# yex33/ReSpaSol

Hardware: AMD Instinct MI355X
Metric: CSR SpMV GFLOP/s + achieved HBM GB/s (fp64 vs fp32), SuiteSparse set, 1/2/4/8 GPU (higher is better)
Workload: dtype f64; 1 GPU; big-set CSR SpMV fp64, 15 matrices per step; matrices=15, nnz_stored_total=268386865, parallelism=1 GPU, launch=rsp_spmv_batch (1 launch(es) of <= 32 matrices per step part): whole step

## Files before the change

include/rsp.h:

```cpp
#ifndef RSP_H
#define RSP_H

#include <stddef.h>
#include <stdint.h>

#ifdef __cplusplus
extern "C" {
#endif

#define RSP_VERSION_MAJOR 0
#define RSP_VERSION_MINOR 1

typedef enum {
    RSP_STATUS_SUCCESS = 0,
    RSP_STATUS_NOT_INITIALIZED = 1,
    RSP_STATUS_ALLOC_FAILED = 2,
    RSP_STATUS_INVALID_VALUE = 3,
    RSP_STATUS_ARCH_MISMATCH = 4,
    RSP_STATUS_EXECUTION_FAILED = 6,
    RSP_STATUS_INTERNAL_ERROR = 7,
    RSP_STATUS_MATRIX_TYPE_NOT_SUPPORTED = 8,
    RSP_STATUS_ZERO_PIVOT = 9,
    RSP_STATUS_NOT_SUPPORTED = 10
} rsp_status_t;

typedef enum { RSP_R_64F = 0, RSP_R_32F = 1 } rsp_datatype_t;

typedef enum { RSP_OPERATION_NON_TRANSPOSE = 0, RSP_OPERATION_TRANSPOSE = 1 } rsp_operation_t;

typedef struct rsp_context *rsp_handle_t;
typedef struct rsp_spmat *rsp_spmat_t;
typedef struct rsp_ilu0_info *rsp_ilu0_info_t;
typedef struct rsp_spmv_batch *rsp_spmv_batch_t;


rsp_status_t rsp_create(rsp_handle_t *handle);
rsp_status_t rsp_destroy(rsp_handle_t handle);
rsp_status_t rsp_set_stream(rsp_handle_t handle, void *stream);
rsp_status_t rsp_get_stream(rsp_handle_t handle, void **stream);
rsp_status_t rsp_set_ftz(rsp_handle_t handle, int enable);
rsp_status_t rsp_get_ftz(rsp_handle_t handle, int *enable);
const char *rsp_get_error_string(rsp_status_t status);
int rsp_get_version(void);


rsp_status_t rsp_create_csr(rsp_spmat_t *mat, int64_t rows, int64_t cols, int64_t nnz,
                            void *d_row_offsets, void *d_col_ind, void *d_values,
                            rsp_datatype_t value_type);
rsp_status_t rsp_csr_set_values(rsp_spmat_t mat, void *d_values, rsp_datatype_t value_type);
rsp_status_t rsp_destroy_spmat(rsp_spmat_t mat);


rsp_status_t rsp_spmv_buffer_size(rsp_handle_t handle, rsp_operation_t op, const void *alpha,
                                  rsp_spmat_t mat, const void *beta, rsp_datatype_t compute_type,
                                  size_t *buffer_size);
rsp_status_t rsp_spmv_preprocess(rsp_handle_t handle, rsp_operation_t op, const void *alpha,
                                 rsp_spmat_t mat, const void *d_x, const void *beta, void *d_y,
                                 rsp_datatype_t compute_type, void *d_buffer);
rsp_status_t rsp_spmv(rsp_handle_t handle, rsp_operation_t op, const void *alpha, rsp_spmat_t mat,
                      const void *d_x, const void *beta, void *d_y, rsp_datatype_t compute_type,
                      void *d_buffer);


rsp_status_t rsp_create_ilu0_info(rsp_ilu0_info_t *info);
rsp_status_t rsp_destroy_ilu0_info(rsp_ilu0_info_t info);

rsp_status_t rsp_ilu0_buffer_size(rsp_handle_t handle, int n, int nnz, rsp_datatype_t value_type,
                                  rsp_ilu0_info_t info, size_t *buffer_size);

rsp_status_t rsp_ilu0_analysis(rsp_handle_t handle, int n, int nnz, const int *d_row_offsets,
                               const int *d_col_ind, rsp_ilu0_info_t info);

rsp_status_t rsp_trsv_analysis(rsp_handle_t handle, rsp_operation_t op, rsp_ilu0_info_t info);

rsp_status_t rsp_ilu0_zero_pivot(rsp_handle_t handle, rsp_ilu0_info_t info, int *position);

#define RSP_TRSV_L 0
#define RSP_TRSV_LT 1
#define RSP_TRSV_U 2
rsp_status_t rsp_trsv_zero_pivot(rsp_handle_t handle, rsp_ilu0_info_t info, int which, int *position);

rsp_status_t rsp_ilu0_factor(rsp_handle_t handle, rsp_ilu0_info_t info, rsp_datatype_t value_type,
                             void *d_values);

rsp_status_t rsp_trsv_lower_unit(rsp_handle_t handle, rsp_operation_t op, const void *alpha,
                                 rsp_ilu0_info_t info, rsp_datatype_t value_type,
                                 const void *d_values, const void *d_x, void *d_y);

rsp_status_t rsp_trsv_upper(rsp_handle_t handle, const void *alpha, rsp_ilu0_info_t info,
                            rsp_datatype_t value_type, const void *d_values, const void *d_x,
                            void *d_y);


typedef struct rsp_bicgstab *rsp_bicgstab_t;
typedef enum { RSP_SOLVE_CONVERGED = 0, RSP_SOLVE_MAX_ITERS = 1, RSP_SOLVE_BREAKDOWN = 2 } rsp_solve_reason_t;

rsp_status_t rsp_bicgstab_create(rsp_handle_t handle, rsp_spmat_t A, rsp_ilu0_info_t info,
                                 rsp_datatype_t precond_type, const void *d_factor, rsp_bicgstab_t *s);
rsp_status_t rsp_bicgstab_solve(rsp_handle_t handle, rsp_bicgstab_t s, const void *d_b, void *d_x,
                                double rtol, int max_iters, int check_every,
                                int *iters, double *relres, rsp_solve_reason_t *reason);
rsp_status_t rsp_bicgstab_history(rsp_bicgstab_t s, int cap, double *relres, int *count);
rsp_status_t rsp_bicgstab_destroy(rsp_bicgstab_t s);
rsp_status_t rsp_dot(rsp_handle_t handle, rsp_datatype_t value_type, int64_t n, const void *d_x,
                     const void *d_y, double *result);

#define RSP_GMRES_MAX_RESTART 64
typedef struct rsp_gmres *rsp_gmres_t;
rsp_status_t rsp_gmres_create(rsp_handle_t handle, rsp_spmat_t A, rsp_ilu0_info_t info,
                              rsp_datatype_t precond_type, const void *d_factor, int restart,
                              rsp_gmres_t *s);
rsp_status_t rsp_gmres_solve(rsp_handle_t handle, rsp_gmres_t s, const void *d_b, void *d_x, double rtol,
                             int max_iters, int check_every, int *iters, double *relres,
                             rsp_solve_reason_t *reason);
rsp_status_t rsp_gmres_history(rsp_gmres_t s, int cap, double *relres, int *count);
rsp_status_t rsp_gmres_destroy(rsp_gmres_t s);
rsp_status_t rsp_orthogonalize(rsp_handle_t handle, rsp_datatype_t value_type, int64_t n, int k,
                               const void *d_V, int64_t ldv, void *d_w, double *h);
rsp_status_t rsp_gmres_lsq_host(int k, int ldh, const double *H, double beta, double *y, double *est);


rsp_status_t rsp_gather(rsp_handle_t handle, rsp_datatype_t value_type, int64_t n,
                        const int64_t *d_idx, const void *d_src, void *d_dst);
rsp_status_t rsp_scatter(rsp_handle_t handle, rsp_datatype_t value_type, int64_t n,
                         const int64_t *d_idx, const void *d_src, void *d_dst);

rsp_status_t rsp_csr2csc(rsp_handle_t handle, int64_t rows, int64_t cols, int64_t nnz,
                         const int *d_row_offsets, const int *d_col_ind, const void *d_values,
                         rsp_datatype_t value_type, int *d_csc_col_offsets, int *d_csc_row_ind,
                         void *d_csc_values);

rsp_status_t rsp_spmv_plan_info(rsp_spmat_t mat, int64_t *tiles, int64_t *entries_16bit);

rsp_status_t rsp_spmat_set_local_cols(rsp_spmat_t mat, int64_t ncols_local);
rsp_status_t rsp_spmv_part(rsp_handle_t handle, const void *alpha, rsp_spmat_t mat,
                           const void *d_x, const void *beta, void *d_y,
                           rsp_datatype_t compute_type, void *d_buffer, int part);

rsp_status_t rsp_spmv_batch_create(rsp_handle_t handle, int count, const rsp_spmat_t *mats,
                                   const void *const *d_x, void *const *d_y,
                                   void *const *d_buffers, rsp_datatype_t compute_type,
                                   int part, rsp_spmv_batch_t *batch);
rsp_status_t rsp_spmv_batch_run(rsp_handle_t handle, rsp_spmv_batch_t batch, const void *alpha,
                                const void *beta);
rsp_status_t rsp_spmv_batch_destroy(rsp_spmv_batch_t batch);
rsp_status_t rsp_spmv_batch_info(rsp_spmv_batch_t batch, int64_t *tiles, int64_t *entries_16bit);

rsp_status_t rsp_ilu0_levels(rsp_ilu0_info_t info, int *levels_lower, int *levels_upper);
rsp_status_t rsp_ilu0_solve_blocks(rsp_ilu0_info_t info, int *blocks_lower, int *blocks_upper);

rsp_status_t rsp_ilu0_analysis_host(int n, const int *row_offsets, const int *col_ind,
                                    int *levels_lower, int *levels_upper, uint64_t *digest,
                                    double *phase_ms);
rsp_status_t rsp_spmv_plan_host(int m, const int *row_offsets, const int *col_ind, int64_t nnz,
                                rsp_datatype_t compute_type, int64_t *tiles, int64_t *entries_16bit,
                                int64_t *entries_staged);
rsp_status_t rsp_spmv_transpose_permute(rsp_handle_t handle, rsp_spmat_t mat);
rsp_status_t rsp_csr_transpose_host(int64_t rows, int64_t cols, const int *row_offsets, const int *col_ind,
                                    int *t_row_offsets, int *t_col_ind, int *perm);
rsp_status_t rsp_spmv_plan_stats(int m, const int *row_offsets, const int *col_ind, int64_t nnz,
                                 rsp_datatype_t compute_type, int64_t stats[8]);
rsp_status_t rsp_ilu0_plan_digest(rsp_ilu0_info_t info, uint64_t *digest);

#ifdef __cplusplus
}
#endif

#endif
```

respasol_amd/_lib.py:

```python
from __future__ import annotations

import ctypes as C
import os

_HERE = os.path.dirname(os.path.abspath(__file__))
LIB_DIR = os.path.join(_HERE, "lib")
BIN_DIR = os.path.join(_HERE, "bin")


class RspError(RuntimeError):

    def __init__(self, status: int, where: str):
        self.status = int(status)
        super().__init__(f"{where}: {STATUS_NAMES.get(self.status, 'RSP_STATUS_UNKNOWN')} ({self.status})")


STATUS_SUCCESS = 0
STATUS_NOT_INITIALIZED = 1
STATUS_ALLOC_FAILED = 2
STATUS_INVALID_VALUE = 3
STATUS_ARCH_MISMATCH = 4
STATUS_EXECUTION_FAILED = 6
STATUS_INTERNAL_ERROR = 7
STATUS_MATRIX_TYPE_NOT_SUPPORTED = 8
STATUS_ZERO_PIVOT = 9
STATUS_NOT_SUPPORTED = 10
STATUS_NAMES = {
    0: "RSP_STATUS_SUCCESS", 1: "RSP_STATUS_NOT_INITIALIZED", 2: "RSP_STATUS_ALLOC_FAILED",
    3: "RSP_STATUS_INVALID_VALUE", 4: "RSP_STATUS_ARCH_MISMATCH", 6: "RSP_STATUS_EXECUTION_FAILED",
    7: "RSP_STATUS_INTERNAL_ERROR", 8: "RSP_STATUS_MATRIX_TYPE_NOT_SUPPORTED",
    9: "RSP_STATUS_ZERO_PIVOT", 10: "RSP_STATUS_NOT_SUPPORTED",
}

R_64F = 0
R_32F = 1
OP_N = 0
OP_T = 1

SOLVE_CONVERGED = 0
SOLVE_MAX_ITERS = 1
SOLVE_BREAKDOWN = 2
KRY_CHUNK = 2048
KRY_MAX_GRID = 1024
GMRES_MAX_RESTART = 64

MM_FULL_SYMMETRIC = 0x1
MM_QUIET = 0x2
MM_SERIAL = 0x4
SURR_FTZ_STRESS = 0x1


class CSRStruct(C.Structure):

    _fields_ = [("isSymmetric", C.c_int), ("m", C.c_int), ("n", C.c_int), ("nnz", C.c_int),
                ("rowptr", C.POINTER(C.c_int)), ("colidx", C.POINTER(C.c_int)),
                ("values", C.POINTER(C.c_double))]


class COOStruct(C.Structure):

    _fields_ = [("isSymmetric", C.c_int), ("m", C.c_int), ("n", C.c_int), ("nnz", C.c_int),
                ("Colidx", C.POINTER(C.c_int)), ("Rowidx", C.POINTER(C.c_int)),
                ("values", C.POINTER(C.c_double))]


vp = C.c_void_p
ip = C.POINTER(C.c_int)
i64 = C.c_int64
i32 = C.c_int

RSP_PROTOS = {
    "rsp_create": (i32, [C.POINTER(vp)]),
    "rsp_destroy": (i32, [vp]),
    "rsp_set_stream": (i32, [vp, vp]),
    "rsp_get_stream": (i32, [vp, C.POINTER(vp)]),
    "rsp_set_ftz": (i32, [vp, i32]),
    "rsp_get_ftz": (i32, [vp, ip]),
    "rsp_get_error_string": (C.c_char_p, [i32]),
    "rsp_get_version": (i32, []),
    "rsp_create_csr": (i32, [C.POINTER(vp), i64, i64, i64, vp, vp, vp, i32]),
    "rsp_csr_set_values": (i32, [vp, vp, i32]),
    "rsp_destroy_spmat": (i32, [vp]),
    "rsp_spmv_buffer_size": (i32, [vp, i32, vp, vp, vp, i32, C.POINTER(C.c_size_t)]),
    "rsp_spmv_preprocess": (i32, [vp, i32, vp, vp, vp, vp, vp, i32, vp]),
    "rsp_spmv": (i32, [vp, i32, vp, vp, vp, vp, vp, i32, vp]),
    "rsp_create_ilu0_info": (i32, [C.POINTER(vp)]),
    "rsp_destroy_ilu0_info": (i32, [vp]),
    "rsp_ilu0_buffer_size": (i32, [vp, i32, i32, i32, vp, C.POINTER(C.c_size_t)]),
    "rsp_ilu0_analysis": (i32, [vp, i32, i32, vp, vp, vp]),
    "rsp_ilu0_zero_pivot": (i32, [vp, vp, ip]),
    "rsp_trsv_zero_pivot": (i32, [vp, vp, i32, ip]),
    "rsp_ilu0_factor": (i32, [vp, vp, i32, vp]),
    "rsp_trsv_lower_unit": (i32, [vp, i32, vp, vp, i32, vp, vp, vp]),
    "rsp_trsv_upper": (i32, [vp, vp, vp, i32, vp, vp, vp]),
    "rsp_ilu0_levels": (i32, [vp, ip, ip]),
    "rsp_ilu0_solve_blocks": (i32, [vp, ip, ip]),
    "rsp_trsv_analysis": (i32, [vp, i32, vp]),
    "rsp_bicgstab_create": (i32, [vp, vp, vp, i32, vp, C.POINTER(vp)]),
    "rsp_bicgstab_solve": (i32, [vp, vp, vp, vp, C.c_double, i32, i32, ip, C.POINTER(C.c_double), ip]),
    "rsp_bicgstab_history": (i32, [vp, i32, C.POINTER(C.c_double), ip]),
    "rsp_bicgstab_destroy": (i32, [vp]),
    "rsp_dot": (i32, [vp, i32, i64, vp, vp, C.POINTER(C.c_double)]),
    "rsp_gmres_create": (i32, [vp, vp, vp, i32, vp, i32, C.POINTER(vp)]),
    "rsp_gmres_solve": (i32, [vp, vp, vp, vp, C.c_double, i32, i32, ip, C.POINTER(C.c_double), ip]),
    "rsp_gmres_history": (i32, [vp, i32, C.POINTER(C.c_double), ip]),
    "rsp_gmres_destroy": (i32, [vp]),
    "rsp_orthogonalize": (i32, [vp, i32, i64, i32, vp, i64, vp, C.POINTER(C.c_double)]),
    "rsp_gmres_lsq_host": (i32, [i32, i32, C.POINTER(C.c_double), C.c_double, C.POINTER(C.c_double),
                                 C.POINTER(C.c_double)]),
    "rsp_gather": (i32, [vp, i32, i64, vp, vp, vp]),
    "rsp_scatter": (i32, [vp, i32, i64, vp, vp, vp]),
    "rsp_spmat_set_local_cols": (i32, [vp, i64]),
    "rsp_spmv_part": (i32, [vp, vp, vp, vp, vp, vp, i32, vp, i32]),
    "rsp_spmv_batch_create": (i32, [vp, i32, vp, vp, vp, vp, i32, i32, vp]),
    "rsp_spmv_batch_run": (i32, [vp, vp, vp, vp]),
    "rsp_spmv_batch_destroy": (i32, [vp]),
    "rsp_spmv_batch_info": (i32, [vp, vp, vp]),
    "rsp_spmv_plan_info": (i32, [vp, vp, vp]),
    "rsp_ilu0_analysis_host": (i32, [i32, vp, vp, vp, vp, vp, vp]),
    "rsp_spmv_plan_host": (i32, [i32, vp, vp, C.c_int64, i32, vp, vp, vp]),
    "rsp_spmv_plan_stats": (i32, [i32, vp, vp, C.c_int64, i32, vp]),
    "rsp_ilu0_plan_digest": (i32, [vp, vp]),
    "rsp_csr2csc": (i32, [vp, i64, i64, i64, vp, vp, vp, i32, vp, vp, vp]),
    "rsp_csr_transpose_host": (i32, [i64, i64, vp, vp, vp, vp, vp]),
    "rsp_spmv_transpose_permute": (i32, [vp, vp]),
}

HOST_PROTOS = {
    "loadMatrixMarket": (i32, [C.c_char_p, C.POINTER(CSRStruct), i32, i32]),
    "loadCooMatrix": (i32, [C.c_char_p, C.POINTER(COOStruct), i32, i32]),
    "rsp_mm_load": (i32, [C.c_char_p, C.POINTER(CSRStruct), i32, i32, i32]),
    "rsp_mm_load_buffer": (i32, [C.c_char_p, C.c_size_t, C.POINTER(CSRStruct), i32, i32, i32]),
    "rsp_row_qsort": (None, [ip, C.POINTER(C.c_double), i32, i32]),
    "rsp_csr_free": (None, [C.POINTER(CSRStruct)]),
    "rsp_coo_free": (None, [C.POINTER(COOStruct)]),
    "rsp_csr_save": (i32, [C.c_char_p, C.POINTER(CSRStruct)]),
    "rsp_csr_load": (i32, [C.c_char_p, C.POINTER(CSRStruct)]),
    "rsp_dlarnv": (i32, [i32, ip, i64, C.POINTER(C.c_double)]),
    "rsp_set_cpu_ftz": (None, [i32]),
    "rsp_surrogate_count": (i32, []),
    "rsp_surrogate_name": (C.c_char_p, [i32]),
    "rsp_surrogate_info": (i32, [C.c_char_p, ip, C.POINTER(i64), ip, ip, ip]),
    "rsp_surrogate_rowlens": (i32, [C.c_char_p, C.c_double, i32, i32, i32, ip]),
    "rsp_surrogate_rows": (i32, [C.c_char_p, C.c_double, ip]),
    "rsp_surrogate_fill": (i32, [C.c_char_p, C.c_double, i32, i32, i32, ip, ip, C.POINTER(C.c_double)]),
    "rsp_surrogate_csr": (i32, [C.c_char_p, C.c_double, i32, C.POINTER(CSRStruct)]),
    "rsp_partition_rows": (i32, [ip, i32, i32, ip]),
    "rsp_padded_chunk": (i32, [ip, i32]),
    "rsp_remap_cols_padded": (i32, [i64, ip, ip, i32, i32, ip]),
    "rsp_host_spmv_f64": (None, [i32, ip, ip, vp, vp, vp]),
    "rsp_host_spmv_f32": (None, [i32, ip, ip, vp, vp, vp]),
}


def _load(name: str, protos: dict, path: str | None = None, probe: bool = False) -> C.CDLL:
    path = path or os.path.join(LIB_DIR, name)
    if not os.path.exists(path):
        raise ImportError(
            f"{path} is missing: build the HIP/C libraries first "
            f"(python -c 'import __graft_entry__ as g; g.build()' or make -C respasol_amd/csrc)")
    lib = C.CDLL(path, mode=C.RTLD_GLOBAL)
    for fname, (res, args) in protos.items():
        if probe and not hasattr(lib, fname):
            continue
        fn = getattr(lib, fname)
        fn.restype = res
        fn.argtypes = args
    return lib


host = _load("librsp_host.so", HOST_PROTOS)
_RSP_PATH = os.environ.get("RSP_PROBE_LIB") or os.path.join(LIB_DIR, "librsp.so")
rsp = (None if os.environ.get("RSP_HOST_ONLY") == "1"
       else _load("librsp.so", RSP_PROTOS, _RSP_PATH, probe=bool(os.environ.get("RSP_PROBE_LIB"))))


def check(status: int, where: str) -> None:
    if status != STATUS_SUCCESS:
        raise RspError(status, where)


def loaded_paths() -> list[str]:
    return [os.path.join(LIB_DIR, "librsp_host.so"), _RSP_PATH]
```

respasol_amd/csrc/rsp_api.cpp:

```cpp

#include "rsp_internal.h"

#include <atomic>

using namespace rsp_api;

using rsp::SpmvBlock;
using rsp::SpmvLongRow;
using rsp_plan::PlanOptions;
using rsp_plan::TilePlan;

namespace {
std::atomic<unsigned long long> g_plan_next{1};
unsigned long long plan_new_gen() { return g_plan_next.fetch_add(1); }
}


static int64_t spmv_resident_tiles(rsp_handle_t h, rsp_datatype_t t) {
    return (int64_t)rsp_k::spmv_tiles_per_cu((int)elem_size(t)) * h->num_cus;
}

static PlanOptions handle_plan_options(rsp_handle_t h, rsp_datatype_t t, int64_t local_cols, int64_t spread) {
    const int e = (int)elem_size(t), v = h->spmv_variant;
    PlanOptions o = rsp_plan::plan_options(t);
    o.spread = spread;
    o.local_cols = local_cols;
    o.row_align = (v & 64) ? 128 / e : (v & 128) ? 64 / e : 1;
    o.use_c16 = !(v & 32);
    o.use_stage = !(v & rsp::kSpmvVariantNoStage);
    return o;
}

static rsp_status_t download_pattern(rsp_handle_t h, rsp_spmat_t mat, rsp_an::hvec<int> &rp,
                                     rsp_an::hvec<int> &ci) {
    const int m = (int)mat->rows;
    rp.assign((size_t)m + 1, 0);
    ci.clear();
    if (m > 0) {
        RSP_CHECK_HIP(hipMemcpyAsync(rp.data(), mat->rowptr, ((size_t)m + 1) * sizeof(int),
                                     hipMemcpyDeviceToHost, h->stream));
        RSP_CHECK_HIP(hipStreamSynchronize(h->stream));
    }
    if (m > 0 && rp[0] != 0) return RSP_STATUS_INVALID_VALUE;
    for (int i = 0; i < m; i++)
        if (rp[i + 1] < rp[i]) return RSP_STATUS_INVALID_VALUE;
    if (m > 0 && (int64_t)rp[(size_t)m] > mat->nnz) return RSP_STATUS_INVALID_VALUE;
    if (m > 0 && rp[(size_t)m] > 0) {
        if (!mat->colidx) return RSP_STATUS_INVALID_VALUE;
        ci.resize((size_t)rp[(size_t)m]);
        RSP_CHECK_HIP(hipMemcpyAsync(ci.data(), mat->colidx, ci.size() * sizeof(int),
                                     hipMemcpyDeviceToHost, h->stream));
        RSP_CHECK_HIP(hipStreamSynchronize(h->stream));
        const int ncols = (int)mat->cols;
        for (int c : ci)
            if ((unsigned)c >= (unsigned)ncols) return RSP_STATUS_INVALID_VALUE;
    }
    return RSP_STATUS_SUCCESS;
}

rsp_status_t rsp_api::spmv_plan(rsp_handle_t h, rsp_spmat_t mat, rsp_datatype_t compute_type) {
    const int m = (int)mat->rows;
    rsp_an::hvec<int> rp, ci;
    rsp_status_t st = download_pattern(h, mat, rp, ci);
    if (st != RSP_STATUS_SUCCESS) return st;
    const bool spread = (h->spmv_variant & 512) != 0;
    TilePlan p;
    rsp_plan::make_tile_plan(rp.data(), ci.data(), m, mat->nnz,
                             handle_plan_options(h, compute_type, mat->local_cols,
                                                 spread ? spmv_resident_tiles(h, compute_type) : 0),
                             p);
    const size_t elem = elem_size(compute_type);
    const rsp_plan::SpmvLayout lay = rsp_plan::spmv_layout({p.blocks.size(), p.longrows.size(), (size_t)p.nslots},
                                                           elem, (int64_t)p.c16.size(), p.runs.size());
    mat->planned = 0;
    if (lay.bytes > mat->plan_cap || !mat->d_plan) {
        if (mat->d_plan) {
            int cur = 0;
            (void)hipGetDevice(&cur);
            (void)hipSetDevice(mat->plan_device);
            (void)hipFree(mat->d_plan);
            (void)hipSetDevice(cur);
            mat->d_plan = nullptr;
            mat->plan_cap = 0;
        }
        RSP_CHECK_HIP(hipMalloc(&mat->d_plan, std::max<size_t>(lay.bytes, 256)));
        mat->plan_cap = std::max<size_t>(lay.bytes, 256);
        RSP_CHECK_HIP(hipGetDevice(&mat->plan_device));
    }
    char *buf = (char *)mat->d_plan;
    auto upload = [&](size_t off, const void *src, size_t bytes) {
        return bytes == 0 ? hipSuccess : hipMemcpyAsync(buf + off, src, bytes, hipMemcpyHostToDevice, h->stream);
    };
    RSP_CHECK_HIP(upload(0, p.blocks.data(), p.blocks.size() * sizeof(SpmvBlock)));
    RSP_CHECK_HIP(upload(lay.off_cbase, p.cbase.data(), p.cbase.size() * sizeof(int)));
    RSP_CHECK_HIP(upload(lay.off_poff, p.poff.data(), p.poff.size() * sizeof(int)));
    RSP_CHECK_HIP(upload(lay.off_cidx, p.c16.data(), p.c16.size() * sizeof(uint16_t)));
    RSP_CHECK_HIP(upload(lay.off_runs, p.runs.data(), p.runs.size() * sizeof(int)));
    RSP_CHECK_HIP(upload(lay.off_long, p.longrows.data(), p.longrows.size() * sizeof(SpmvLongRow)));
    if (p.nslots > 0)
        RSP_CHECK_HIP(hipMemsetAsync(buf + lay.off_part, 0, (size_t)p.nslots * 2 * elem, h->stream));
    RSP_CHECK_HIP(hipStreamSynchronize(h->stream));
    mat->planned = 1;
    mat->plan_type = compute_type;
    mat->nblocks = (int)p.blocks.size();
    mat->nint = p.nint;
    mat->plan_gen = plan_new_gen();
    mat->nlong = (int)p.longrows.size();
    mat->nslots = p.nslots;
    mat->nnz_s = m > 0 ? rp[(size_t)m] : 0;
    mat->lay = lay;
    mat->nnz_c16 = p.nnz_c16;
    mat->nnz_staged = p.nnz_staged;
    return RSP_STATUS_SUCCESS;
}


struct HostTranspose {
    rsp_an::hvec<int> rowptr, colidx, perm;
    int64_t nnz = 0;
};

static rsp_status_t transpose_pattern(rsp_handle_t h, rsp_spmat_t mat, HostTranspose &t) {
    rsp_an::hvec<int> rp, ci;
    RSP_TRY(download_pattern(h, mat, rp, ci));
    t.nnz = mat->rows > 0 ? rp[(size_t)mat->rows] : 0;
    if (mat->cols > INT_MAX - 1) return RSP_STATUS_INVALID_VALUE;
    t.rowptr.assign((size_t)mat->cols + 1, 0);
    t.colidx.assign((size_t)t.nnz, 0);
    t.perm.assign((size_t)t.nnz, 0);
    return rsp_tr::csr_transpose(mat->rows, mat->cols, rp.data(), ci.data(), t.rowptr.data(), t.colidx.data(),
                                 t.perm.data());
}

static hipError_t upload_ints(rsp_handle_t h, void *dst, const rsp_an::hvec<int> &src) {
    return src.empty() ? hipSuccess
                       : hipMemcpyAsync(dst, src.data(), src.size() * sizeof(int), hipMemcpyHostToDevice, h->stream);
}

static rsp_status_t tside_build(rsp_handle_t h, rsp_spmat_t mat) {
    HostTranspose ht;
    RSP_TRY(transpose_pattern(h, mat, ht));
    std::unique_ptr<rsp_spmat_tside> t(new rsp_spmat_tside());
    RSP_CHECK_HIP(hipGetDevice(&t->device));
    const size_t off_ci = align256(ht.rowptr.size() * sizeof(int));
    const size_t off_perm = off_ci + align256(ht.colidx.size() * sizeof(int));
    const size_t bytes = off_perm + std::max<size_t>(align256(ht.perm.size() * sizeof(int)), 256);
    RSP_CHECK_HIP(hipMalloc(&t->pattern.p, bytes));
    RSP_CHECK_HIP(hipMalloc(&t->vt.p, std::max<size_t>((size_t)ht.nnz * elem_size(mat->type), 256)));
    char *buf = (char *)t->pattern.p;
    RSP_CHECK_HIP(upload_ints(h, buf, ht.rowptr));
    RSP_CHECK_HIP(upload_ints(h, buf + off_ci, ht.colidx));
    RSP_CHECK_HIP(upload_ints(h, buf + off_perm, ht.perm));
    RSP_CHECK_HIP(hipStreamSynchronize(h->stream));
    t->perm = (int *)(buf + off_perm);
    rsp_spmat &c = t->child;
    c.rows = mat->cols;
    c.cols = mat->rows;
    c.nnz = ht.nnz;
    c.rowptr = (int *)buf;
    c.colidx = (int *)(buf + off_ci);
    c.vals = t->vt.p;
    c.type = mat->type;
    c.local_cols = -1;
    RSP_TRY(rsp_api::spmv_plan(h, &c, c.type));
    rsp_k::warm_transpose();
    delete mat->tside;
    mat->tside = t.release();
    return RSP_STATUS_SUCCESS;
}

static rsp_status_t tside_ready(rsp_handle_t h, rsp_spmat_t mat) {
    if (!mat->tside) return tside_build(h, mat);
    rsp_spmat_tside *t = mat->tside;
    if (t->child.type != mat->type) {
        DevMem v;
        RSP_CHECK_HIP(hipMalloc(&v.p, std::max<size_t>((size_t)t->child.nnz * elem_size(mat->type), 256)));
        t->vt = std::move(v);
        t->child.vals = t->vt.p;
        t->child.type = mat->type;
        t->child.planned = 0;
    }
    return RSP_STATUS_SUCCESS;
}

static rsp_status_t spmv_run_transposed(rsp_handle_t h, const void *alpha, rsp_spmat_t mat, const void *d_x,
                                        const void *beta, void *d_y, rsp_datatype_t compute_type, void *d_buffer) {
    if (compute_type != mat->type) return RSP_STATUS_INVALID_VALUE;
    if ((mat->rows > 0 && !d_x) || (mat->cols > 0 && !d_y)) return RSP_STATUS_INVALID_VALUE;
    RSP_TRY(tside_ready(h, mat));
    rsp_spmat_tside *t = mat->tside;
    if (t->child.nnz > 0 && !mat->vals) return RSP_STATUS_INVALID_VALUE;
    if (rsp_k::permute_values((int)elem_size(compute_type), t->child.nnz, t->perm, mat->vals, t->vt.p, h->num_cus,
                              h->stream) != hipSuccess)
        return RSP_STATUS_EXECUTION_FAILED;
    return rsp_api::spmv_run(h, RSP_OPERATION_NON_TRANSPOSE, alpha, &t->child, d_x, beta, d_y, compute_type,
                             d_buffer, 0);
}

rsp_status_t rsp_api::spmv_run(rsp_handle_t h, rsp_operation_t op, const void *alpha, rsp_spmat_t mat,
                               const void *d_x, const void *beta, void *d_y,
                               rsp_datatype_t compute_type, void *d_buffer, int part) {
    if (!h) return RSP_STATUS_NOT_INITIALIZED;
    if (!mat || !alpha || !beta) return RSP_STATUS_INVALID_VALUE;
    if (op == RSP_OPERATION_TRANSPOSE && part == 0)
        return spmv_run_transposed(h, alpha, mat, d_x, beta, d_y, compute_type, d_buffer);
    if (op != RSP_OPERATION_NON_TRANSPOSE) return RSP_STATUS_NOT_SUPPORTED;
    if (compute_type != mat->type) return RSP_STATUS_INVALID_VALUE;
    if (mat->rows > 0 && (!d_y || (mat->cols > 0 && !d_x))) return RSP_STATUS_INVALID_VALUE;
    (void)d_buffer;
    if (!mat->planned || mat->plan_type != compute_type) {
        rsp_status_t st = spmv_plan(h, mat, compute_type);
        if (st != RSP_STATUS_SUCCESS) return st;
    }
    char *plan = (char *)mat->d_plan;
    rsp::SpmvArgs a;
    a.m = (int)mat->rows;
    a.rowptr = mat->rowptr;
    a.colidx = mat->colidx;
    a.vals = mat->vals;
    a.x = d_x;
    a.y = d_y;
    a.blocks = (const SpmvBlock *)plan;
    a.nblocks = mat->nblocks;
    a.cbases = (const int *)(plan + mat->lay.off_cbase);
    a.poffs = (const int *)(plan + mat->lay.off_poff);
    a.cidx = (const unsigned short *)(plan + mat->lay.off_cidx);
    a.runs = (const int *)(plan + mat->lay.off_runs);
    a.cmax = mat->cols > 0 ? (int)(mat->cols - 1) : 0;
    a.longrows = (const SpmvLongRow *)(plan + mat->lay.off_long);
    a.nlong = mat->nlong;
    a.partials = plan + mat->lay.off_part;
    if (compute_type == RSP_R_64F) {
        a.alpha = *(const double *)alpha;
        a.beta = *(const double *)beta;
    } else {
        a.alpha = *(const float *)alpha;
        a.beta = *(const float *)beta;
    }
    if (part != 0) {
        if (a.beta != 0.0) return RSP_STATUS_INVALID_VALUE;
        if (part == 1) {
            a.nblocks = mat->nint;
            a.nlong = 0;
        } else {
            a.blocks += mat->nint;
            a.cbases += mat->nint;
            a.poffs += mat->nint;
            a.nblocks = mat->nblocks - mat->nint;
        }
    }
    a.vector_ok = ((((uintptr_t)mat->colidx) | ((uintptr_t)mat->vals)) & 15) == 0;
    a.nnz = mat->nnz_s;
    a.variant = h->spmv_variant;
    hipError_t e;
    if (compute_type == RSP_R_64F)
        e = rsp_k::spmv_f64(a, h->stream);
    else
        e = h->ftz ? rsp_k_ftz::spmv_f32(a, h->stream) : rsp_k::spmv_f32(a, h->stream);
    return e == hipSuccess ? RSP_STATUS_SUCCESS : RSP_STATUS_EXECUTION_FAILED;
}


struct rsp_spmv_batch {
    rsp_datatype_t type;
    int part;
    rsp_an::hvec<rsp_spmat_t> mats;
    rsp_an::hvec<unsigned long long> plan_gen;
    rsp_an::hvec<rsp::SpmvBatchArgs> launches;
    void *d_mem = nullptr;
    int64_t tiles = 0, entries_16bit = 0;
    ~rsp_spmv_batch() {
        if (d_mem) (void)hipFree(d_mem);
    }
};

static rsp_status_t spmv_batch_create(rsp_handle_t h, int count, const rsp_spmat_t *mats,
                                      const void *const *d_x, void *const *d_y,
                                      void *const *d_buffers, rsp_datatype_t compute_type,
                                      int part, rsp_spmv_batch_t *batch) {
    if (!h) return RSP_STATUS_NOT_INITIALIZED;
    (void)d_buffers;
    if (!batch || count < 0 || (count > 0 && (!mats || !d_x || !d_y)))
        return RSP_STATUS_INVALID_VALUE;
    if (part < 0 || part > 2) return RSP_STATUS_INVALID_VALUE;
    if (compute_type != RSP_R_64F && compute_type != RSP_R_32F) return RSP_STATUS_INVALID_VALUE;
    *batch = nullptr;
    for (int j = 0; j < count; j++) {
        rsp_spmat_t A = mats[j];
        if (!A) return RSP_STATUS_INVALID_VALUE;
        if (A->type != compute_type) return RSP_STATUS_INVALID_VALUE;
        if (A->rows > 0 && (!d_y[j] || (A->cols > 0 && !d_x[j]))) return RSP_STATUS_INVALID_VALUE;
        if (!A->planned || A->plan_type != compute_type) {
            rsp_status_t st = spmv_plan(h, A, compute_type);
            if (st != RSP_STATUS_SUCCESS) return st;
        }
    }
    std::unique_ptr<rsp_spmv_batch> b(new rsp_spmv_batch());
    b->type = compute_type;
    b->part = part;
    const int64_t R = spmv_resident_tiles(h, compute_type);
    const bool spread_ok = !(h->spmv_variant & 16);
    rsp_an::hvec<TilePlan> plans((size_t)count);
    struct Region { size_t off, len; };
    struct Span {
        int first, count, nt, nl;
        rsp_an::hvec<Region> reg;
        enum { kEntries, kTiles, kCbases, kPoffs, kLongRows, kC16, kRuns, kPartials };
        const Region &at(int kind, int q) const { return reg[kind < kC16 ? kind : kC16 + (kind - kC16) * count + q]; }
    };
    rsp_an::hvec<Span> spans;
    size_t bytes = 0;
    auto tile_range = [part](const TilePlan &p, int *t0, int *t1) {
        *t0 = part == 2 ? p.nint : 0;
        *t1 = part == 1 ? p.nint : (int)p.blocks.size();
    };
    for (int first = 0; first < count; first += rsp::kSpmvBatchMax) {
        Span sp{first, std::min(rsp::kSpmvBatchMax, count - first), 0, 0, {}};
        rsp_an::hvec<rsp_an::hvec<int>> rps((size_t)sp.count), cis((size_t)sp.count);
        auto plan_members = [&](int64_t spread_all, int64_t nnz_all) {
            sp.nt = 0;
            for (int q = 0; q < sp.count; q++) {
                rsp_spmat_t A = mats[first + q];
                const int64_t nnz_q = A->rows > 0 ? rps[q][(size_t)A->rows] : 0;
                const int64_t share =
                    spread_all > 0 ? std::max<int64_t>(1, spread_all * nnz_q / std::max<int64_t>(1, nnz_all)) : 0;
                TilePlan &p = plans[first + q];
                rsp_plan::make_tile_plan(rps[q].data(), cis[q].data(), (int)A->rows, A->nnz,
                                         handle_plan_options(h, compute_type, A->local_cols, share), p);
                int t0, t1;
                tile_range(p, &t0, &t1);
                sp.nt += t1 - t0;
            }
        };
        int64_t nnz_all = 0;
        for (int q = 0; q < sp.count; q++) {
            rsp_spmat_t A = mats[first + q];
            rsp_status_t st = download_pattern(h, A, rps[q], cis[q]);
            if (st != RSP_STATUS_SUCCESS) return st;
            nnz_all += A->rows > 0 ? rps[q][(size_t)A->rows] : 0;
        }
        plan_members(0, nnz_all);
        if (spread_ok && sp.nt < R) plan_members(R, nnz_all);
        for (int q = 0; q < sp.count; q++) {
            const TilePlan &p = plans[first + q];
            rsp_spmat_t A = mats[first + q];
            if ((int)p.longrows.size() != A->nlong || p.nslots != A->nslots)
                return RSP_STATUS_INTERNAL_ERROR;
            sp.nl += part == 1 ? 0 : (int)p.longrows.size();
        }
        sp.reg = {{0, (size_t)sp.count * sizeof(rsp::SpmvBatchEntry)},
                  {0, (size_t)sp.nt * sizeof(SpmvBlock)},
                  {0, (size_t)sp.nt * sizeof(int)},
                  {0, (size_t)sp.nt * sizeof(int)},
                  {0, (size_t)sp.nl * sizeof(SpmvLongRow)}};
        for (int q = 0; q < sp.count; q++) sp.reg.push_back({0, plans[first + q].c16.size() * sizeof(uint16_t)});
        for (int q = 0; q < sp.count; q++) sp.reg.push_back({0, plans[first + q].runs.size() * sizeof(int)});
        for (int q = 0; q < sp.count; q++)
            sp.reg.push_back({0, (size_t)plans[first + q].nslots * 2 * elem_size(compute_type)});
        for (Region &r : sp.reg) {
            r.off = bytes;
            bytes += (r.len + 15) & ~(size_t)15;
        }
        spans.push_back(sp);
    }
    {
        size_t end = 0;
        for (const Span &sp : spans)
            for (const Region &r : sp.reg) {
                if (r.off < end || r.off + r.len > bytes) return RSP_STATUS_INTERNAL_ERROR;
                end = r.off + r.len;
            }
    }
    if (bytes > 0) RSP_CHECK_HIP(hipMalloc(&b->d_mem, bytes));
    rsp_an::hvec<unsigned char> host(bytes);
    bool fits = true;
    for (const Span &sp : spans) {
        auto dev = [&](int kind, int q = 0) { return (char *)b->d_mem + sp.at(kind, q).off; };
        auto put = [&](int kind, int q, size_t at, const void *src, size_t n) {
            const Region &r = sp.at(kind, q);
            if (at + n > r.len)
                fits = false;
            else if (n > 0)
                memcpy(host.data() + r.off + at, src, n);
        };
        rsp::SpmvBatchArgs a{};
        a.entries = (const rsp::SpmvBatchEntry *)dev(Span::kEntries);
        a.tiles = (const SpmvBlock *)dev(Span::kTiles);
        a.cbases = (const int *)dev(Span::kCbases);
        a.poffs = (const int *)dev(Span::kPoffs);
        a.longrows = (const SpmvLongRow *)dev(Span::kLongRows);
        a.count = sp.count;
        for (int q = 0; q <= rsp::kSpmvBatchMax; q++)
            a.tiles_at.begin[q] = a.longs_at.begin[q] = INT_MAX;
        size_t nt = 0, nl = 0;
        for (int q = 0; q < sp.count; q++) {
            rsp_spmat_t A = mats[sp.first + q];
            const TilePlan &p = plans[sp.first + q];
            int t0, t1;
            tile_range(p, &t0, &t1);
            const size_t ntq = (size_t)(t1 - t0), nlq = part == 1 ? 0 : p.longrows.size();
            rsp::SpmvBatchEntry e{};
            e.rowptr = A->rowptr;
            e.colidx = A->colidx;
            e.vals = A->vals;
            e.x = d_x[sp.first + q];
            e.y = d_y[sp.first + q];
            e.partials = (void *)dev(Span::kPartials, q);
            e.cidx = (const unsigned short *)dev(Span::kC16, q);
            e.runs = (const int *)dev(Span::kRuns, q);
            e.cmax = A->cols > 0 ? (int)(A->cols - 1) : 0;
            e.nnz = A->nnz_s;
            e.vector_ok = ((((uintptr_t)A->colidx) | ((uintptr_t)A->vals)) & 15) == 0;
            put(Span::kEntries, 0, (size_t)q * sizeof(e), &e, sizeof(e));
            a.tiles_at.begin[q] = (int)nt;
            a.longs_at.begin[q] = (int)nl;
            for (int t = t0; t < t1; t++)
                if (p.cbase[(size_t)t] != rsp_plan::kCbaseInt32)
                    b->entries_16bit += p.blocks[(size_t)t].k1 - p.blocks[(size_t)t].k0;
            b->tiles += (int64_t)ntq;
            put(Span::kTiles, 0, nt * sizeof(SpmvBlock), p.blocks.data() + t0, ntq * sizeof(SpmvBlock));
            put(Span::kCbases, 0, nt * sizeof(int), p.cbase.data() + t0, ntq * sizeof(int));
            put(Span::kPoffs, 0, nt * sizeof(int), p.poff.data() + t0, ntq * sizeof(int));
            put(Span::kLongRows, 0, nl * sizeof(SpmvLongRow), p.longrows.data(), nlq * sizeof(SpmvLongRow));
            put(Span::kC16, q, 0, p.c16.data(), p.c16.size() * sizeof(uint16_t));
            put(Span::kRuns, q, 0, p.runs.data(), p.runs.size() * sizeof(int));
            nt += ntq;
            nl += nlq;
        }
        a.tiles_at.begin[sp.count] = (int)nt;
        a.longs_at.begin[sp.count] = (int)nl;
        b->launches.push_back(a);
    }
    if (!fits) return RSP_STATUS_INTERNAL_ERROR;
    if (bytes > 0) {
        RSP_CHECK_HIP(hipMemcpyAsync(b->d_mem, host.data(), bytes, hipMemcpyHostToDevice, h->stream));
        RSP_CHECK_HIP(hipStreamSynchronize(h->stream));
    }
    for (int j = 0; j < count; j++) {
        b->mats.push_back(mats[j]);
        b->plan_gen.push_back(mats[j]->plan_gen);
    }
    *batch = b.release();
    return RSP_STATUS_SUCCESS;
}

extern "C" {

int rsp_get_version(void) { return RSP_VERSION_MAJOR * 1000 + RSP_VERSION_MINOR; }

const char *rsp_get_error_string(rsp_status_t s) {
    switch (s) {
        case RSP_STATUS_SUCCESS: return "RSP_STATUS_SUCCESS";
        case RSP_STATUS_NOT_INITIALIZED: return "RSP_STATUS_NOT_INITIALIZED";
        case RSP_STATUS_ALLOC_FAILED: return "RSP_STATUS_ALLOC_FAILED";
        case RSP_STATUS_INVALID_VALUE: return "RSP_STATUS_INVALID_VALUE";
        case RSP_STATUS_ARCH_MISMATCH: return "RSP_STATUS_ARCH_MISMATCH";
        case RSP_STATUS_EXECUTION_FAILED: return "RSP_STATUS_EXECUTION_FAILED";
        case RSP_STATUS_INTERNAL_ERROR: return "RSP_STATUS_INTERNAL_ERROR";
        case RSP_STATUS_MATRIX_TYPE_NOT_SUPPORTED: return "RSP_STATUS_MATRIX_TYPE_NOT_SUPPORTED";
        case RSP_STATUS_ZERO_PIVOT: return "RSP_STATUS_ZERO_PIVOT";
        case RSP_STATUS_NOT_SUPPORTED: return "RSP_STATUS_NOT_SUPPORTED";
    }
    return "RSP_STATUS_UNKNOWN";
}

rsp_status_t rsp_create(rsp_handle_t *handle) {
    if (!handle) return RSP_STATUS_INVALID_VALUE;
    *handle = nullptr;
    int dev = 0;
    if (hipGetDevice(&dev) != hipSuccess) return RSP_STATUS_NOT_INITIALIZED;
    hipDeviceProp_t prop;
    if (hipGetDeviceProperties(&prop, dev) != hipSuccess) return RSP_STATUS_NOT_INITIALIZED;
    if (strncmp(prop.gcnArchName, "gfx950", 6) != 0) return RSP_STATUS_ARCH_MISMATCH;
    rsp_context *c = new (std::nothrow) rsp_context;
    if (!c) return RSP_STATUS_ALLOC_FAILED;
    c->device = dev;
    c->stream = nullptr;
    c->ftz = 0;
    const char *v = getenv("RSP_SPMV_VARIANT");
    c->spmv_variant = v ? atoi(v) : 0;
    c->num_cus = prop.multiProcessorCount > 0 ? prop.multiProcessorCount : 256;
    rsp_k::warm_spmv();
    rsp_k_ftz::warm_spmv();
    rsp_k::warm_ilu();
    rsp_k_ftz::warm_ilu();
    rsp_k::warm_analysis();
    rsp_k::warm_krylov();
    rsp_k_ftz::warm_krylov();
    c->d_ftrace = nullptr;
    c->d_strace = nullptr;
    c->d_dot = nullptr;
    c->h_dot = nullptr;
    c->d_gm = nullptr;
    c->h_gm = nullptr;
    *handle = c;
    return RSP_STATUS_SUCCESS;
}

rsp_status_t rsp_destroy(rsp_handle_t h) {
    if (!h) return RSP_STATUS_NOT_INITIALIZED;
    if (h->d_ftrace || h->d_strace || h->d_dot || h->h_dot || h->d_gm || h->h_gm) {
        int cur = 0;
        (void)hipGetDevice(&cur);
        (void)hipSetDevice(h->device);
        if (h->d_ftrace) (void)hipFree(h->d_ftrace);
        if (h->d_strace) (void)hipFree(h->d_strace);
        if (h->d_dot) (void)hipFree(h->d_dot);
        if (h->h_dot) (void)hipHostFree(h->h_dot);
        if (h->d_gm) (void)hipFree(h->d_gm);
        if (h->h_gm) (void)hipHostFree(h->h_gm);
        (void)hipSetDevice(cur);
    }
    delete h;
    return RSP_STATUS_SUCCESS;
}

rsp_status_t rsp_set_stream(rsp_handle_t h, void *stream) {
    if (!h) return RSP_STATUS_NOT_INITIALIZED;
    h->stream = (hipStream_t)stream;
    return RSP_STATUS_SUCCESS;
}

rsp_status_t rsp_get_stream(rsp_handle_t h, void **stream) {
    if (!h) return RSP_STATUS_NOT_INITIALIZED;
    if (!stream) return RSP_STATUS_INVALID_VALUE;
    *stream = (void *)h->stream;
    return RSP_STATUS_SUCCESS;
}

rsp_status_t rsp_set_ftz(rsp_handle_t h, int enable) {
    if (!h) return RSP_STATUS_NOT_INITIALIZED;
    h->ftz = enable ? 1 : 0;
    return RSP_STATUS_SUCCESS;
}

rsp_status_t rsp_get_ftz(rsp_handle_t h, int *enable) {
    if (!h) return RSP_STATUS_NOT_INITIALIZED;
    if (!enable) return RSP_STATUS_INVALID_VALUE;
    *enable = h->ftz;
    return RSP_STATUS_SUCCESS;
}


rsp_status_t rsp_create_csr(rsp_spmat_t *mat, int64_t rows, int64_t cols, int64_t nnz,
                            void *d_row_offsets, void *d_col_ind, void *d_values,
                            rsp_datatype_t value_type) {
    if (!mat) return RSP_STATUS_INVALID_VALUE;
    *mat = nullptr;
    if (rows < 0 || cols < 0 || nnz < 0 || rows > INT_MAX - 1 || cols > INT_MAX || nnz > INT_MAX)
        return RSP_STATUS_INVALID_VALUE;
    if (value_type != RSP_R_64F && value_type != RSP_R_32F) return RSP_STATUS_INVALID_VALUE;
    if (!d_row_offsets && rows > 0) return RSP_STATUS_INVALID_VALUE;
    if ((!d_col_ind || !d_values) && nnz > 0) return RSP_STATUS_INVALID_VALUE;
    rsp_spmat *a = new (std::nothrow) rsp_spmat;
    if (!a) return RSP_STATUS_ALLOC_FAILED;
    memset(a, 0, sizeof(*a));
    a->rows = rows;
    a->cols = cols;
    a->nnz = nnz;
    a->rowptr = (int *)d_row_offsets;
    a->colidx = (int *)d_col_ind;
    a->vals = d_values;
    a->type = value_type;
    a->planned = 0;
    a->d_plan = nullptr;
    a->local_cols = -1;
    *mat = a;
    return RSP_STATUS_SUCCESS;
}

rsp_status_t rsp_spmat_set_local_cols(rsp_spmat_t mat, int64_t ncols_local) {
    if (!mat || ncols_local < 0 || ncols_local > mat->cols) return RSP_STATUS_INVALID_VALUE;
    mat->local_cols = ncols_local;
    mat->planned = 0;
    return RSP_STATUS_SUCCESS;
}

rsp_status_t rsp_csr_set_values(rsp_spmat_t mat, void *d_values, rsp_datatype_t value_type) {
    if (!mat) return RSP_STATUS_INVALID_VALUE;
    if (value_type != RSP_R_64F && value_type != RSP_R_32F) return RSP_STATUS_INVALID_VALUE;
    if (d_values != mat->vals) mat->plan_gen = plan_new_gen();
    mat->vals = d_values;
    if (value_type != mat->type) mat->planned = 0;
    mat->type = value_type;
    return RSP_STATUS_SUCCESS;
}

rsp_status_t rsp_destroy_spmat(rsp_spmat_t mat) {
    if (!mat) return RSP_STATUS_INVALID_VALUE;
    if (mat->d_plan) {
        int cur = 0;
        (void)hipGetDevice(&cur);
        (void)hipSetDevice(mat->plan_device);
        (void)hipFree(mat->d_plan);
        (void)hipSetDevice(cur);
    }
    delete mat->tside;
    delete mat;
    return RSP_STATUS_SUCCESS;
}


rsp_status_t rsp_spmv_buffer_size(rsp_handle_t h, rsp_operation_t op, const void *alpha,
                                  rsp_spmat_t mat, const void *beta, rsp_datatype_t compute_type,
                                  size_t *buffer_size) {
    (void)alpha;
    (void)beta;
    return guarded([&] {
        if (!h) return RSP_STATUS_NOT_INITIALIZED;
        if (!mat || !buffer_size) return RSP_STATUS_INVALID_VALUE;
        if (op == RSP_OPERATION_TRANSPOSE) {
            if (compute_type != mat->type) return RSP_STATUS_INVALID_VALUE;
            RSP_TRY(tside_ready(h, mat));
            rsp_spmat *c = &mat->tside->child;
            if (!c->planned || c->plan_type != compute_type) RSP_TRY(spmv_plan(h, c, compute_type));
            *buffer_size = 0;
            return RSP_STATUS_SUCCESS;
        }
        if (op != RSP_OPERATION_NON_TRANSPOSE) return RSP_STATUS_NOT_SUPPORTED;
        if (compute_type != mat->type) return RSP_STATUS_INVALID_VALUE;
        if (!mat->planned || mat->plan_type != compute_type) RSP_TRY(spmv_plan(h, mat, compute_type));
        *buffer_size = 0;
        return RSP_STATUS_SUCCESS;
    });
}

rsp_status_t rsp_spmv_preprocess(rsp_handle_t h, rsp_operation_t op, const void *alpha,
                                 rsp_spmat_t mat, const void *d_x, const void *beta, void *d_y,
                                 rsp_datatype_t compute_type, void *d_buffer) {
    (void)alpha;
    (void)beta;
    (void)d_x;
    (void)d_y;
    (void)d_buffer;
    return guarded([&] {
        if (!h) return RSP_STATUS_NOT_INITIALIZED;
        if (!mat) return RSP_STATUS_INVALID_VALUE;
        if (op != RSP_OPERATION_NON_TRANSPOSE && op != RSP_OPERATION_TRANSPOSE) return RSP_STATUS_NOT_SUPPORTED;
        if (compute_type != mat->type) return RSP_STATUS_INVALID_VALUE;
        return op == RSP_OPERATION_TRANSPOSE ? tside_build(h, mat) : spmv_plan(h, mat, compute_type);
    });
}

rsp_status_t rsp_spmv_plan_info(rsp_spmat_t mat, int64_t *tiles, int64_t *entries_16bit) {
    if (!mat || !tiles || !entries_16bit) return RSP_STATUS_INVALID_VALUE;
    if (!mat->planned) return RSP_STATUS_NOT_INITIALIZED;
    *tiles = mat->nblocks;
    *entries_16bit = mat->nnz_c16;
    return RSP_STATUS_SUCCESS;
}

rsp_status_t rsp_spmv(rsp_handle_t h, rsp_operation_t op, const void *alpha, rsp_spmat_t mat,
                      const void *d_x, const void *beta, void *d_y, rsp_datatype_t compute_type,
                      void *d_buffer) {
    return guarded([&] { return spmv_run(h, op, alpha, mat, d_x, beta, d_y, compute_type, d_buffer, 0); });
}

rsp_status_t rsp_spmv_part(rsp_handle_t h, const void *alpha, rsp_spmat_t mat, const void *d_x,
                           const void *beta, void *d_y, rsp_datatype_t compute_type,
                           void *d_buffer, int part) {
    return guarded([&] {
        if (part < 0 || part > 2) return RSP_STATUS_INVALID_VALUE;
        return spmv_run(h, RSP_OPERATION_NON_TRANSPOSE, alpha, mat, d_x, beta, d_y, compute_type,
                        d_buffer, part);
    });
}


rsp_status_t rsp_spmv_batch_create(rsp_handle_t h, int count, const rsp_spmat_t *mats,
                                   const void *const *d_x, void *const *d_y,
                                   void *const *d_buffers, rsp_datatype_t compute_type,
                                   int part, rsp_spmv_batch_t *batch) {
    return guarded([&] { return spmv_batch_create(h, count, mats, d_x, d_y, d_buffers, compute_type, part, batch); });
}

rsp_status_t rsp_spmv_batch_run(rsp_handle_t h, rsp_spmv_batch_t b, const void *alpha,
                                const void *beta) {
    if (!h) return RSP_STATUS_NOT_INITIALIZED;
    if (!b || !alpha || !beta) return RSP_STATUS_INVALID_VALUE;
    for (size_t j = 0; j < b->mats.size(); j++) {
        const rsp_spmat_t A = b->mats[j];
        if (!A->planned || A->plan_gen != b->plan_gen[j]) return RSP_STATUS_INVALID_VALUE;
    }
    const double av = b->type == RSP_R_64F ? *(const double *)alpha : *(const float *)alpha;
    const double bv = b->type == RSP_R_64F ? *(const double *)beta : *(const float *)beta;
    if (b->part != 0 && bv != 0.0) return RSP_STATUS_INVALID_VALUE;
    for (rsp::SpmvBatchArgs a : b->launches) {
        a.alpha = av;
        a.beta = bv;
        a.variant = h->spmv_variant;
        hipError_t e;
        if (b->type == RSP_R_64F)
            e = rsp_k::spmv_batch_f64(a, h->stream);
        else
            e = h->ftz ? rsp_k_ftz::spmv_batch_f32(a, h->stream) : rsp_k::spmv_batch_f32(a, h->stream);
        if (e != hipSuccess) return RSP_STATUS_EXECUTION_FAILED;
    }
    return RSP_STATUS_SUCCESS;
}

rsp_status_t rsp_spmv_batch_info(rsp_spmv_batch_t b, int64_t *tiles, int64_t *entries_16bit) {
    if (!b || !tiles || !entries_16bit) return RSP_STATUS_INVALID_VALUE;
    *tiles = b->tiles;
    *entries_16bit = b->entries_16bit;
    return RSP_STATUS_SUCCESS;
}

rsp_status_t rsp_spmv_batch_destroy(rsp_spmv_batch_t b) {
    if (!b) return RSP_STATUS_INVALID_VALUE;
    delete b;
    return RSP_STATUS_SUCCESS;
}

rsp_status_t rsp_gather(rsp_handle_t h, rsp_datatype_t value_type, int64_t n, const int64_t *d_idx,
                        const void *d_src, void *d_dst) {
    if (!h) return RSP_STATUS_NOT_INITIALIZED;
    if (value_type != RSP_R_64F && value_type != RSP_R_32F) return RSP_STATUS_INVALID_VALUE;
    if (n < 0 || (n > 0 && (!d_idx || !d_src || !d_dst))) return RSP_STATUS_INVALID_VALUE;
    hipError_t e = rsp_k::gather(value_type == RSP_R_64F ? 8 : 4, n, d_idx, d_src, d_dst, h->stream);
    return e == hipSuccess ? RSP_STATUS_SUCCESS : RSP_STATUS_EXECUTION_FAILED;
}

rsp_status_t rsp_scatter(rsp_handle_t h, rsp_datatype_t value_type, int64_t n, const int64_t *d_idx,
                         const void *d_src, void *d_dst) {
    if (!h) return RSP_STATUS_NOT_INITIALIZED;
    if (value_type != RSP_R_64F && value_type != RSP_R_32F) return RSP_STATUS_INVALID_VALUE;
    if (n < 0 || (n > 0 && (!d_idx || !d_src || !d_dst))) return RSP_STATUS_INVALID_VALUE;
    hipError_t e = rsp_k::scatter(value_type == RSP_R_64F ? 8 : 4, n, d_idx, d_src, d_dst, h->stream);
    return e == hipSuccess ? RSP_STATUS_SUCCESS : RSP_STATUS_EXECUTION_FAILED;
}

rsp_status_t rsp_spmv_transpose_permute(rsp_handle_t h, rsp_spmat_t mat) {
    if (!h) return RSP_STATUS_NOT_INITIALIZED;
    if (!mat) return RSP_STATUS_INVALID_VALUE;
    const rsp_spmat_tside *t = mat->tside;
    if (!t || t->child.type != mat->type) return RSP_STATUS_NOT_INITIALIZED;
    if (t->child.nnz > 0 && !mat->vals) return RSP_STATUS_INVALID_VALUE;
    const hipError_t e = rsp_k::permute_values((int)elem_size(mat->type), t->child.nnz, t->perm, mat->vals, t->vt.p,
                                               h->num_cus, h->stream);
    return e == hipSuccess ? RSP_STATUS_SUCCESS : RSP_STATUS_EXECUTION_FAILED;
}

rsp_status_t rsp_csr2csc(rsp_handle_t h, int64_t rows, int64_t cols, int64_t nnz, const int *d_row_offsets,
                         const int *d_col_ind, const void *d_values, rsp_datatype_t value_type,
                         int *d_csc_col_offsets, int *d_csc_row_ind, void *d_csc_values) {
    return guarded([&] {
        if (!h) return RSP_STATUS_NOT_INITIALIZED;
        if (rows < 0 || cols < 0 || nnz < 0 || rows > INT_MAX - 1 || cols > INT_MAX - 1 || nnz > INT_MAX)
            return RSP_STATUS_INVALID_VALUE;
        if (value_type != RSP_R_64F && value_type != RSP_R_32F) return RSP_STATUS_INVALID_VALUE;
        if ((!d_row_offsets && rows > 0) || !d_csc_col_offsets) return RSP_STATUS_INVALID_VALUE;
        const bool symbolic = !d_values && !d_csc_values;
        rsp_spmat a;
        memset(&a, 0, sizeof(a));
        a.rows = rows;
        a.cols = cols;
        a.nnz = nnz;
        a.rowptr = const_cast<int *>(d_row_offsets);
        a.colidx = const_cast<int *>(d_col_ind);
        HostTranspose ht;
        RSP_TRY(transpose_pattern(h, &a, ht));
        if (ht.nnz > 0 && (!d_csc_row_ind || (!symbolic && (!d_values || !d_csc_values))))
            return RSP_STATUS_INVALID_VALUE;
        DevMem perm;
        RSP_CHECK_HIP(upload_ints(h, d_csc_col_offsets, ht.rowptr));
        RSP_CHECK_HIP(upload_ints(h, d_csc_row_ind, ht.colidx));
        if (!symbolic && ht.nnz > 0) {
            RSP_CHECK_HIP(hipMalloc(&perm.p, (size_t)ht.nnz * sizeof(int)));
            RSP_CHECK_HIP(upload_ints(h, perm.p, ht.perm));
            if (rsp_k::permute_values((int)elem_size(value_type), ht.nnz, (const int *)perm.p, d_values,
                                      d_csc_values, h->num_cus, h->stream) != hipSuccess)
                return RSP_STATUS_EXECUTION_FAILED;
        }
        RSP_CHECK_HIP(hipStreamSynchronize(h->stream));
        return RSP_STATUS_SUCCESS;
    });
}

rsp_status_t rsp_spmv_plan_host(int m, const int *row_offsets, const int *col_ind, int64_t nnz,
                                rsp_datatype_t compute_type, int64_t *tiles, int64_t *entries_16bit,
                                int64_t *entries_staged) {
    return guarded([&] {
        if (m < 0 || (m > 0 && (!row_offsets || !col_ind)) || !tiles || !entries_16bit || !entries_staged)
            return RSP_STATUS_INVALID_VALUE;
        if (compute_type != RSP_R_64F && compute_type != RSP_R_32F) return RSP_STATUS_NOT_SUPPORTED;
        const PlanOptions o = rsp_plan::plan_options(compute_type);
        TilePlan p;
        rsp_plan::make_tile_plan(row_offsets, col_ind, m, nnz, o, p);
        if (!rsp_plan::plan_verify(row_offsets, col_ind, m, o, p)) return RSP_STATUS_INTERNAL_ERROR;
        *tiles = (int64_t)p.blocks.size();
        *entries_16bit = p.nnz_c16;
        *entries_staged = p.nnz_staged;
        return RSP_STATUS_SUCCESS;
    });
}

rsp_status_t rsp_spmv_plan_stats(int m, const int *row_offsets, const int *col_ind, int64_t nnz,
                                 rsp_datatype_t compute_type, int64_t stats[8]) {
    return guarded([&] {
        if (m < 0 || (m > 0 && (!row_offsets || !col_ind)) || !stats) return RSP_STATUS_INVALID_VALUE;
        if (compute_type != RSP_R_64F && compute_type != RSP_R_32F) return RSP_STATUS_NOT_SUPPORTED;
        TilePlan p;
        rsp_plan::make_tile_plan(row_offsets, col_ind, m, nnz, rsp_plan::plan_options(compute_type), p);
        rsp_plan::plan_stats(p, compute_type, stats);
        return RSP_STATUS_SUCCESS;
    });
}

}
```

respasol_amd/csrc/rsp_internal.h:

```cpp
#pragma once

#include "rsp.h"

#include <hip/hip_runtime.h>
#include <limits.h>
#include <math.h>
#include <stdio.h>
#include <stdlib.h>
#include <string.h>

#include <algorithm>
#include <cmath>
#include <memory>
#include <new>
#include <vector>

#include "rsp_kernels.h"
#include "ilu_analysis.h"
#include "spmv_plan.h"
#include "csr_transpose.h"

struct rsp_context {
    int device;
    hipStream_t stream;
    int ftz;
    int spmv_variant;
    int num_cus;
    unsigned long long *d_ftrace;
    unsigned long long *d_strace;
    double *d_dot;
    double *h_dot;
    double *d_gm;
    double *h_gm;
};

struct rsp_spmat_tside;
struct rsp_spmat {
    int64_t rows, cols, nnz;
    int *rowptr;
    int *colidx;
    void *vals;
    rsp_datatype_t type;
    int planned;
    int plan_device;
    void *d_plan;
    size_t plan_cap;
    rsp_datatype_t plan_type;
    int nblocks, nlong, nslots;
    int nnz_s;
    rsp_plan::SpmvLayout lay;
    int64_t nnz_c16;
    int64_t nnz_staged;
    int64_t local_cols;
    int nint;
    unsigned long long plan_gen;
    rsp_spmat_tside *tside;
};

struct DevMem {
    void *p = nullptr;
    DevMem() = default;
    DevMem(DevMem &&o) noexcept : p(o.p) { o.p = nullptr; }
    DevMem &operator=(DevMem &&o) noexcept {
        std::swap(p, o.p);
        return *this;
    }
    ~DevMem() {
        if (p) (void)hipFree(p);
    }
};

struct rsp_spmat_tside {
    int device = 0;
    DevMem pattern;
    DevMem vt;
    int *perm = nullptr;
    rsp_spmat child{};
    rsp_spmat_tside() = default;
    rsp_spmat_tside(const rsp_spmat_tside &) = delete;
    rsp_spmat_tside &operator=(const rsp_spmat_tside &) = delete;
    ~rsp_spmat_tside() {
        int cur = 0;
        (void)hipGetDevice(&cur);
        (void)hipSetDevice(device);
        if (child.d_plan) (void)hipFree(child.d_plan);
        pattern = DevMem();
        vt = DevMem();
        (void)hipSetDevice(cur);
    }
};

struct rsp_ilu0_info {
    int analysed = 0, factored = 0;
    int n = 0, nnz_s = 0;
    int structural_zero = -1;
    rsp_handle_t han = nullptr;
    long long n_updates = 0;
    rsp::IluArgs fac{};
    int *d_zero = nullptr;
    unsigned long long claim_host = 0;
    int *d_fdone = nullptr;
    unsigned *d_tk = nullptr;
    unsigned long long tk_seq = 0;
    unsigned flow_epoch = 0;
    int fac_gen = 0;
    int solve_gen[3] = {0, 0, 0};
    struct Dag {
        rsp::LevelPlan plan{};
        rsp_an::hvec<int> ptr;
        int nterms = 0;
        rsp_an::hvec<int> nshort;
        rsp_an::hvec<int> nwave;
        rsp_an::hvec<int> sbase;
        rsp_an::hvec<rsp::LevelSeg> segs;
        int batch = 8;
        int group = 4;
    } L, LT, U, F;
    struct BlkDag {
        bool on = false;
        rsp::BlkArgs args{};
        rsp_an::hvec<rsp::BlkSeg> segs;
    } Lb, LTb;
    bool fac_one = false;
    const Dag &fdag() const { return fac_one ? F : L; }
    rsp_an::hvec<rsp::LevelSeg> fac_segs;
    int fac_batch = 8;
    rsp_an::hvec<rsp::FacFlowRun> fruns;
    rsp_an::hvec<rsp::FacSlotLevel> fslev;
    void *d_sval = nullptr, *d_sx = nullptr, *d_sdg = nullptr;
    void *d_usval = nullptr;
    DevMem arena;
    DevMem arena_sym;
    DevMem arena_pairs;
    DevMem arena_s;
    DevMem arena_u;
    DevMem fslots;
    unsigned long long digest = 0;
    std::unique_ptr<rsp_an::IluHostPlan> host;
    rsp_an::hvec<int> host_rp, host_ci;
    std::unique_ptr<rsp_an::Task> solves_task;
    bool solves_ready = false;
    bool dev_terms = true;
    DevMem fbackup;
    size_t fbackup_bytes = 0;
    long long call_seq = 0;
    struct FacCall {
        long long seq = 0;
        int valid = 0;
        int ftz = 0;
        rsp_datatype_t type = RSP_R_64F;
        void *vals = nullptr;
    } last_fac;
    struct SolveCall {
        long long seq = 0;
        int valid = 0;
        int ftz = 0;
        rsp_operation_t op = RSP_OPERATION_NON_TRANSPOSE;
        double alpha = 1.0;
        rsp_datatype_t type = RSP_R_64F;
        const void *vals = nullptr, *x = nullptr;
        void *y = nullptr;
    } last_solve[3];

    void reset() {
        solves_task.reset();
        *this = rsp_ilu0_info();
    }
};

#define RSP_CHECK_HIP(call)                                                     \
    do {                                                                        \
        hipError_t e_ = (call);                                                 \
        if (e_ != hipSuccess)                                                   \
            return e_ == hipErrorOutOfMemory ? RSP_STATUS_ALLOC_FAILED          \
                                             : RSP_STATUS_EXECUTION_FAILED;     \
    } while (0)

#define RSP_TRY(call)                                   \
    do {                                                \
        const rsp_status_t st_ = (call);                \
        if (st_ != RSP_STATUS_SUCCESS) return st_;      \
    } while (0)

namespace rsp_api {

using rsp_an::env_int;

template <typename F, typename C>
rsp_status_t guarded(F body, C cleanup) {
    try {
        return body();
    } catch (const std::bad_alloc &) {
        cleanup();
        return RSP_STATUS_ALLOC_FAILED;
    } catch (...) {
        cleanup();
        return RSP_STATUS_INTERNAL_ERROR;
    }
}
template <typename F>
rsp_status_t guarded(F body) {
    return guarded(body, [] {});
}

inline size_t align256(size_t x) { return (x + 255) & ~(size_t)255; }
inline size_t elem_size(rsp_datatype_t t) { return t == RSP_R_64F ? 8 : 4; }

rsp_status_t spmv_plan(rsp_handle_t h, rsp_spmat_t mat, rsp_datatype_t compute_type);
rsp_status_t spmv_run(rsp_handle_t h, rsp_operation_t op, const void *alpha, rsp_spmat_t mat, const void *d_x,
                      const void *beta, void *d_y, rsp_datatype_t compute_type, void *d_buffer, int part);

rsp_status_t ilu_solves_ready(rsp_handle_t h, rsp_ilu0_info *f);
rsp_status_t ilu_plan_u(rsp_handle_t h, rsp_ilu0_info *f);

rsp_status_t rsp_trsv_lower_unit_impl(rsp_handle_t h, rsp_operation_t op, const void *alpha, rsp_ilu0_info *f,
                                      rsp_datatype_t value_type, const void *d_values, const void *d_x, void *d_y,
                                      bool flow_ok);
rsp_status_t rsp_trsv_upper_impl(rsp_handle_t h, const void *alpha, rsp_ilu0_info *f, rsp_datatype_t value_type,
                                 const void *d_values, const void *d_x, void *d_y, bool flow_ok);

}
```

respasol_amd/csrc/rsp_kernels.h:

```cpp
#pragma once

#include <hip/hip_runtime.h>
#include <stdint.h>

namespace rsp {

struct alignas(16) SpmvBlock {
    int r0, r1, k0, k1;
};

struct alignas(16) SpmvLongRow {
    int row, first, nchunks, pad;
};

#ifndef RSP_SPMV_THREADS
#define RSP_SPMV_THREADS 256
#endif
constexpr int kSpmvThreads = RSP_SPMV_THREADS;
#ifndef RSP_SPMV_ITER
#define RSP_SPMV_ITER 4
#endif
constexpr int kSpmvIter = RSP_SPMV_ITER;
#ifndef RSP_SPMV_MAXROWS
#define RSP_SPMV_MAXROWS 512
#endif
constexpr int kSpmvMaxRows = RSP_SPMV_MAXROWS;
constexpr int kSpmvLongRow = 256;
constexpr int kSpmvHeavyMax = 128;
constexpr int kSpmvWholeRow = -2147483647 - 1;
template <typename T>
struct SpmvTile {
    static constexpr int kVec = 16 / sizeof(T);
    static constexpr int kSlots = kSpmvThreads * kSpmvIter * kVec;
    static constexpr int kMaxNnz = kSlots - (kVec - 1);
    static constexpr int kChunk = kSpmvThreads * 4 * kVec - (kVec - 1);
    static_assert(kChunk <= kMaxNnz, "a chunk must fit one tile");
    static constexpr int kMaxRows = sizeof(T) == 8 ? kSpmvMaxRows : 2 * kSpmvMaxRows;
    static constexpr int kStageSlots = sizeof(T) == 8 ? 1536 : 2048;
    static constexpr bool kStageList = sizeof(T) == 8;
};
static_assert(SpmvTile<float>::kMaxNnz / 33 < kSpmvHeavyMax && SpmvTile<double>::kMaxNnz / 33 < kSpmvHeavyMax,
              "every > 32-entry row of a tile fits the heavy-row list");
constexpr int kStageRuns = 254;

struct SpmvArgs {
    int m;
    const int *rowptr;
    const int *colidx;
    const void *vals;
    const void *x;
    void *y;
    const SpmvBlock *blocks;
    int nblocks;
    const int *cbases;
    const unsigned short *cidx;
    const int *runs;
    const int *poffs;
    int cmax;
    const SpmvLongRow *longrows;
    int nlong;
    void *partials;
    double alpha, beta;
    int nnz;
    int vector_ok;
    int variant;
};

constexpr int kSpmvBatchMax = 32;
struct alignas(16) SpmvBatchEntry {
    const int *rowptr;
    const int *colidx;
    const void *vals;
    const void *x;
    void *y;
    void *partials;
    const unsigned short *cidx;
    const int *runs;
    int nnz;
    int vector_ok;
    int cmax;
};
struct SpmvBatchTable {
    int begin[kSpmvBatchMax + 1];
};
struct SpmvBatchArgs {
    const SpmvBatchEntry *entries;
    const SpmvBlock *tiles;
    const int *cbases;
    const int *poffs;
    const SpmvLongRow *longrows;
    int count;
    SpmvBatchTable tiles_at, longs_at;
    double alpha, beta;
    int variant;
};
constexpr int kSpmvVariantFixup = 256;
constexpr int kSpmvVariantNoStage = 1024;

struct LevelSeg {
    int lb, le, thin, c0, c1;
    int nth;
};
struct alignas(16) RowTask {
    int i, t0, t1, d;
};
struct alignas(16) LevelChunk {
    int l0, l1;
    int x0, x1;
    int k0, k1;
    int st0, st1;
};
struct alignas(16) FlowItem {
    int x0, n, t0, gate;
};
struct alignas(16) ThinRowPlan {
    int g, out, i, d;
};
struct alignas(8) StagedTerm {
    int slot, j;
};

struct LevelPlan {
    const int *rows;
    const int *ptr_dev;
    const int *ptr_host;
    int nlev;
    const LevelSeg *segs;
    int nseg;
    int batch;
    int group;
    const RowTask *tasks;
    const int *tpos;
    const int *src;
    const LevelChunk *chunks;
    const ThinRowPlan *trow;
    const int *sid;
    const StagedTerm *stg;
    const FlowItem *fitems;
    int has_flow;
    int nterms;
    const int *nshort;
    const int *nshort_host;
    const int *nwave_host;
    const int *sbase_host;
};
constexpr int kLongTerms = 64;
constexpr int kHubTerms = 256;
constexpr int kFatLongTerms = 8;
constexpr int kFatLongDefault = 3;
constexpr int kYWin = 4096;
constexpr int kChunkRows = 1024;
constexpr int kChunkTerms = 4096;
constexpr int kThinThreads = 1024;
constexpr int kGroup = 4;
constexpr int kPadSrc = -(kYWin + 1);
constexpr int kIluWaves = 4;
constexpr int kFacRow = 256;
constexpr int kFacPairs = 1024;
constexpr int kThinSolveRows = 512;
constexpr int kThinSolveTerms = 2048;
constexpr int kThinFactorRows = 1024;
constexpr int kRndItems = 2048;
constexpr int kRndPairs = 4096;
constexpr int kRndStaged = 4096;
constexpr int kRndRounds = 2048;
constexpr int kRndLevelItems = 1 << 15;
constexpr int kRndFlowItems = 1024;
constexpr int kRndItemPairs = 1024;
constexpr int kRndLevelStart = 1 << 15;
struct alignas(16) RndChunk {
    int i0, i1, p0, p1, s0, s1, r0, r1;
};
struct alignas(16) RndItem {
    int pos, u, d, zr;
};

struct alignas(16) FacRow {
    int i, rs, di, re, q0, q1, hasdiag, pad;
};

struct FacSlotLevel {
    long long off;
    int stride, rm, qm, pad;
};
__host__ __device__ constexpr int fac_pairs_at(int rm) { return (8 + 2 * rm + 1) & ~1; }

struct alignas(16) FacFlowItem {
    long long off;
    int rmqm, gate;
};
struct FacFlowRun {
    int lb, le, c0, c1;
};

struct FlowCtl {
    int *status;
    int gen;
    unsigned long long ticks;
    unsigned long long *claim;
    unsigned long long *claim_host;
    int mode;
    unsigned *tickets;
    unsigned long long *tk_seq;
    int *done;
    int grid_x;
    unsigned epoch;
};
constexpr int kFlowClaims = 1;
constexpr int kFlowTickets = 2;
constexpr int kFlowTicketCtrs = 8;
constexpr int kFlowOwnMax = 1024;
constexpr int kFlowStealUs = 50;


struct IluArgs {
    int n;
    const int *rowptr;
    const int *colidx;
    const int *dpos;
    const int *hasdiag;
    void *vals;
    int *zero_pivot;
    const int *upd_ptr;
    const int *upd_l;
    const int *upd_u;
    const int *lord;
    const int *lend;
    const int *udiv;
    const FacRow *frow;
    const int *fslots;
    const FacSlotLevel *fslev;
    int fat_slots;
    int fat_lds;
    LevelPlan plan;
    const RndChunk *rchunks;
    const RndItem *ritems;
    const int *rpairs, *rstaged, *rrounds;
    unsigned long long *trace;
    int trace_cap;
    int defer_rounds;
    int narrow_waves;
    const FacFlowItem *fitems;
    const FacFlowRun *fruns;
    int nfruns;
    const int *lev;
    void *forig;
    int gen;
    int flow, flow_grid, flow_sleep;
    int flow_cus;
    FlowCtl fc;
    int fac_one;
};

constexpr int kBlkRows = 64, kBlkYMax = 32, kBlkNear = 12, kBlkNearWin = 1 << 30, kBlkWin = 16384;
constexpr int kBlkLongCap = 64 * kBlkNear;
constexpr int kBlkPre = 6;
constexpr int kBlkLdsMax = 160 * 1024;
struct alignas(16) BlkDesc {
    int p0, np, kind, kn;
    int eoff, ne, doff, nd;
    int loff, nlev, pad[2];
};
struct alignas(16) BlkRow {
    int off, nx, ny, nfar;
};
struct BlkSeg {
    int b0, b1, p0, p1;
};
struct BlkArgs {
    int n, nb;
    const int *order;
    const BlkDesc *desc;
    const BlkRow *rows;
    const int *ref;
    const int *vpos;
    const unsigned *eord;
    const int *lptr;
    const int *rptr;
    const unsigned *rit;
    const BlkSeg *segs;
    int nseg;
    int lds_elems;
    int lds_words;
    const void *vals, *x;
    void *y;
    double alpha;
    void *ev, *yp;
    void *rc;
};

struct TrsvArgs {
    int n;
    const int *rowptr;
    const int *colidx;
    const int *dpos;
    const int *hasdiag;
    const void *vals;
    const void *x;
    void *y;
    double alpha;
    LevelPlan plan;
    void *sval;
    void *sx;
    void *sdg;
    unsigned long long *trace;
    int trace_cap;
    int trace_clk;
    int wave_lds;
    int narrow_waves;
    int narrow_split;
    int narrow_pairs;
    int loaders;
    int flow;
    int flow_grid;
    int flow_cus;
    FlowCtl fc;
    int flow_sleep;
};


constexpr int kKryThreads = 256;
constexpr int kKryChunk = 2048;
constexpr int kKryMaxGrid = 1024;
struct KryGrid {
    int grid;
    long long chunk;
};
inline KryGrid kry_grid(long long n) {
    KryGrid g;
    const long long span = (long long)kKryChunk * kKryMaxGrid;
    g.chunk = (long long)kKryChunk * (n > span ? (n + span - 1) / span : 1);
    g.grid = n > 0 ? (int)((n + g.chunk - 1) / g.chunk) : 1;
    return g;
}
enum {
    kKryRho0 = 0,
    kKryRho1 = 1,
    kKryAlpha = 2,
    kKryOmega = 3,
    kKryFlag = 4,
    kKryFlagIt = 5,
    kKryScalars = 16
};
enum { kKryPartRR = 0, kKryPartBB, kKryPartRhR, kKryPartRhV, kKryPartTS, kKryPartTT, kKryDots };
enum { kKryBreakRho = 1, kKryBreakOmega = 2, kKryBreakRhV = 3, kKryBreakTT = 4 };
constexpr size_t kKryBlockDoubles = kKryScalars + (size_t)kKryDots * kKryMaxGrid;
enum KryOp {
    kKryInit,
    kKryPUpdate,
    kKryDotRhV,
    kKrySUpdate,
    kKryDotTS,
    kKryXUpdate,
    kKryWiden,
    kKryZero,
    kKryDot
};
enum { kKryF64 = 0, kKryF32 = 1, kKryF64Copy32 = 2 };
struct KryArgs {
    long long n;
    double *blk;
    int it;
    const void *b;
    const void *c;
    void *x, *r, *rhat, *p, *v, *s, *t;
    const void *phat, *shat;
    void *copy32;
};
inline double kry_combine_host(const double *part, int g) {
    double v[kKryThreads];
    for (int t = 0; t < kKryThreads; t++) {
        v[t] = 0.0;
        for (int i = t; i < g; i += kKryThreads) v[t] += part[i];
    }
    double w[kKryThreads / 64];
    for (int k = 0; k < kKryThreads / 64; k++) {
        double *l = v + 64 * k;
        for (int off = 32; off > 0; off >>= 1)
            for (int i = 0; i < off; i++) l[i] += l[i + off];
        w[k] = l[0];
    }
    return ((w[0] + w[1]) + w[2]) + w[3];
}

constexpr int kGmMax = 64;
constexpr int kGmLd = kGmMax + 1;
enum {
    kGmStop = 0,
    kGmDone = 1,
    kGmBeta = 2,
    kGmBn = 3,
    kGmFlag = kKryFlag,
    kGmFlagIt = kKryFlagIt,
    kGmScalars = 16,
    kGmEst = kGmScalars,
    kGmHead = kGmEst + kGmMax,
    kGmR = kGmHead,
    kGmCs = kGmR + kGmLd * kGmMax,
    kGmSn = kGmCs + kGmMax,
    kGmG = kGmSn + kGmMax,
    kGmY = kGmG + kGmLd,
    kGmH1 = kGmY + kGmMax,
    kGmH2 = kGmH1 + kGmLd,
    kGmSmall = (kGmH2 + kGmLd + 15) / 16 * 16
};
enum {
    kGmPartRR = 0,
    kGmPartBB = 1,
    kGmPartNrm = 2,
    kGmPartD1 = 3,
    kGmPartD2 = kGmPartD1 + kGmLd,
    kGmDots = kGmPartD2 + kGmLd
};
enum { kGmBreakH = 1, kGmBreakDiag = 2, kGmBreakNorm = 3, kGmBreakY = 4 };
constexpr size_t kGmBlockDoubles = kGmSmall + (size_t)kGmDots * kKryMaxGrid;
enum GmOp {
    kGmResid,
    kGmNormalise,
    kGmMultiDot,
    kGmUpdate1,
    kGmUpdate2,
    kGmCombine
};
struct GmArgs {
    long long n;
    double *blk;
    int j;
    int first;
    const void *b;
    void *x;
    void *V;
    long long ldv;
    const void *Z;
    long long ldz;
    void *w;
    void *copy32;
};

#if defined(__HIPCC__)
#define RSP_HD __host__ __device__
#else
#define RSP_HD
#endif
RSP_HD inline int gmres_lsq(double *col, int j, double *cs, double *sn, double *g, const double *R, int ldr,
                            int k, double *y) {
    if (col) {
        for (int i = 0; i <= j + 1; i++)
            if (!(col[i] - col[i] == 0.0)) return kGmBreakH;
        for (int i = 0; i < j; i++) {
            const double a = col[i], b = col[i + 1];
            col[i] = cs[i] * a + sn[i] * b;
            col[i + 1] = cs[i] * b - sn[i] * a;
        }
        const double a = col[j], b = col[j + 1];
        const double aa = a < 0.0 ? -a : a, ab = b < 0.0 ? -b : b;
        const double s = aa > ab ? aa : ab;
        if (s == 0.0) return kGmBreakDiag;
        const double as = a / s, bs = b / s;
        const double r = s * sqrt(as * as + bs * bs);
        if (r == 0.0 || !(r - r == 0.0)) return kGmBreakDiag;
        const double c = a / r, t = b / r;
        cs[j] = c;
        sn[j] = t;
        col[j] = r;
        col[j + 1] = 0.0;
        const double gj = g[j];
        g[j] = c * gj;
        g[j + 1] = -(t * gj);
    }
    if (y) {
        for (int i = k - 1; i >= 0; i--) {
            double v = g[i];
            for (int l = i + 1; l < k; l++) v -= R[i + (size_t)l * ldr] * y[l];
            y[i] = v / R[i + (size_t)i * ldr];
        }
    }
    return 0;
}
}

#define RSP_DECLARE_KERNEL_API(NS)                                                              \
    namespace NS {                                                                              \
    hipError_t spmv_f32(const rsp::SpmvArgs &a, hipStream_t s);                                 \
    hipError_t spmv_batch_f32(const rsp::SpmvBatchArgs &a, hipStream_t s);                      \
    hipError_t ilu0_factor_f32(const rsp::IluArgs &a, hipStream_t s);                           \
    hipError_t trsv_lower_n_f32(const rsp::TrsvArgs &a, hipStream_t s);                         \
    hipError_t trsv_lower_t_f32(const rsp::TrsvArgs &a, hipStream_t s);                         \
    hipError_t trsv_upper_f32(const rsp::TrsvArgs &a, hipStream_t s);                           \
    hipError_t trsv_blocks_f32(const rsp::BlkArgs &a, hipStream_t s);                           \
    void warm_spmv();                                                                           \
    void warm_ilu();                                                                            \
    hipError_t krylov(rsp::KryOp op, int type, const rsp::KryArgs &a, hipStream_t s);           \
    hipError_t gmres(rsp::GmOp op, int type, const rsp::GmArgs &a, hipStream_t s);              \
    void warm_krylov();                                                                         \
    }

RSP_DECLARE_KERNEL_API(rsp_k)
RSP_DECLARE_KERNEL_API(rsp_k_ftz)

namespace rsp_k {
hipError_t gather(int elem_bytes, int64_t n, const int64_t *idx, const void *src, void *dst,
                  hipStream_t s);
hipError_t scatter(int elem_bytes, int64_t n, const int64_t *idx, const void *src, void *dst,
                   hipStream_t s);
hipError_t spmv_f64(const rsp::SpmvArgs &a, hipStream_t s);
hipError_t spmv_batch_f64(const rsp::SpmvBatchArgs &a, hipStream_t s);
int spmv_tiles_per_cu(int elem_bytes);
hipError_t permute_values(int elem_bytes, int64_t nnz, const int *perm, const void *v, void *vt, int num_cus,
                          hipStream_t s);
void warm_transpose();
void warm_analysis();
hipError_t ilu0_factor_f64(const rsp::IluArgs &a, hipStream_t s);
hipError_t trsv_lower_n_f64(const rsp::TrsvArgs &a, hipStream_t s);
hipError_t trsv_lower_t_f64(const rsp::TrsvArgs &a, hipStream_t s);
hipError_t trsv_upper_f64(const rsp::TrsvArgs &a, hipStream_t s);
hipError_t trsv_blocks_f64(const rsp::BlkArgs &a, hipStream_t s);
hipError_t ilu0_build_slots(const rsp::IluArgs &a, const int4 *desc, const long long *offs, int nrows,
                            int *slots, hipStream_t s);
hipError_t ilu_an_rows(int n, const int *rp, const int *ci, int *dpos, int *hasdiag, int *flags, hipStream_t s);
hipError_t ilu_an_count(const int *const rows_c[3], const int n_c[3], int cap0, const int *rp, const int *ci,
                        const int *dpos, const int *hasdiag, int *cnt, int *gcur, hipStream_t s);
hipError_t ilu_an_scan(const int *cnt, int *ptr, int count, void *temp, size_t *temp_bytes, hipStream_t s);
hipError_t ilu_an_gather_pairs(const int *rows, int nrows, const int *rp, const int *ptr, const int *cbase,
                               const int *upd_l, const int *upd_u, int *out_l, int *out_u, hipStream_t s);
hipError_t ilu_an_fill(const int *const rows_c[3], const int n_c[3], int cap0, const int *rp, const int *ci,
                       const int *dpos, const int *hasdiag, const int *ptr, int *gcur, int *upd_l, int *upd_u,
                       hipStream_t s);
hipError_t ilu_an_stages(int n, int maxlen, const int *rp, const int *ci, const int *dpos, const int *hasdiag,
                         const int *ptr, const int *upd_l, int *stage, int *lord, int *lend, int *udiv,
                         int *scratch, const int *wrows, int nwrows, hipStream_t s);
struct SolveTermsArgs {
    int kind, n, nx, total, nch, group;
    const rsp::RowTask *tasks;
    const int *ptr;
    const int *rp, *ci, *dpos;
    const int *ltp, *lts, *ltc;
    const int *lpos;
    const int *ne;
    rsp::LevelChunk *chunks;
    const int *cbase;
    int *tpos, *src, *sid;
    rsp::ThinRowPlan *trow;
    rsp::StagedTerm *stg;
    int *slot_of, *nst, *nst_ptr;
    void *scan;
};
hipError_t ilu_an_solve_terms(const SolveTermsArgs &a, hipStream_t s);
}
```

respasol_amd/csrc/spmv.hip:

```cpp

#include <hip/hip_runtime.h>

#include <type_traits>

#include "rsp_kernels.h"
#include "spmv_pack.h"

#ifndef RSP_KNS
#define RSP_KNS rsp_k
#endif

#ifndef RSP_NT_Y
#define RSP_NT_Y -1
#endif

namespace RSP_KNS {

using rsp::kSpmvThreads;
using rsp::kSpmvHeavyMax;
using rsp::SpmvArgs;
using rsp::SpmvBlock;
using rsp::SpmvLongRow;
using rsp::SpmvTile;
using rsp::kSpmvBatchMax;
using rsp::SpmvBatchArgs;
using rsp::SpmvBatchEntry;
using rsp::SpmvBatchTable;

template <typename T, int N>
struct VecT;
template <>
struct VecT<double, 2> {
    typedef double __attribute__((ext_vector_type(2))) V;
    typedef int __attribute__((ext_vector_type(2))) I;
    typedef unsigned short __attribute__((ext_vector_type(2))) H;
};
template <>
struct VecT<float, 4> {
    typedef float __attribute__((ext_vector_type(4))) V;
    typedef int __attribute__((ext_vector_type(4))) I;
    typedef unsigned short __attribute__((ext_vector_type(4))) H;
};

__device__ __forceinline__ int xcd_swizzle(int bid, int nwg) {
    const int q = nwg >> 3, r = nwg & 7;
    const int xcd = bid & 7, idx = bid >> 3;
    const int start = xcd < r ? xcd * (q + 1) : r * (q + 1) + (xcd - r) * q;
    return start + idx;
}

template <bool NT, typename P>
__device__ __forceinline__ P ld(const P *p) {
    if constexpr (NT)
        return __builtin_nontemporal_load(p);
    else
        return *p;
}

template <typename T, bool NT, bool C16 = false, int NTH = kSpmvThreads,
          int IT = SpmvTile<T>::kSlots / (kSpmvThreads * (16 / sizeof(T)))>
__device__ __forceinline__ void stream_products(const int *__restrict__ colidx,
                                                const unsigned short *__restrict__ cidx, int cbase,
                                                int cmax, const T *__restrict__ vals,
                                                const T *__restrict__ x, int kb, int k1,
                                                T *__restrict__ lds) {
    constexpr int VW = 16 / sizeof(T);
    typedef typename VecT<T, VW>::V V;
    typedef typename VecT<T, VW>::I I;
    typedef typename VecT<T, VW>::H H;
    const int tid = threadIdx.x;
    const int last = (k1 - 1) & ~(VW - 1);
    I ci[IT];
    H ch[IT];
#pragma unroll
    for (int it = 0; it < IT; ++it) {
        const int e = min(kb + (it * NTH + tid) * VW, last);
        if constexpr (C16)
            ch[it] = ld<NT>(reinterpret_cast<const H *>(cidx + e));
        else
            ci[it] = ld<NT>(reinterpret_cast<const I *>(colidx + e));
    }
    V vv[IT];
#pragma unroll
    for (int it = 0; it < IT; ++it) {
        const int e = min(kb + (it * NTH + tid) * VW, last);
        vv[it] = ld<NT>(reinterpret_cast<const V *>(vals + e));
    }
    __builtin_amdgcn_sched_barrier(0);
    T xv[IT][VW];
#pragma unroll
    for (int it = 0; it < IT; ++it)
#pragma unroll
        for (int j = 0; j < VW; ++j) {
            int c;
            if constexpr (C16)
                c = min(cbase + (int)ch[it][j], cmax);
            else
                c = ci[it][j];
            xv[it][j] = x[c];
        }
    __builtin_amdgcn_sched_barrier(0);
#pragma unroll
    for (int it = 0; it < IT; ++it) {
        V p;
#pragma unroll
        for (int j = 0; j < VW; ++j) p[j] = vv[it][j] * xv[it][j];
        *reinterpret_cast<V *>(lds + (it * NTH + tid) * VW) = p;
    }
}

__device__ __forceinline__ void lds_barrier() {
    __builtin_amdgcn_fence(__ATOMIC_RELEASE, "workgroup", "local");
    __builtin_amdgcn_s_barrier();
    __builtin_amdgcn_fence(__ATOMIC_ACQUIRE, "workgroup", "local");
}

template <typename T, bool NT, int PKM, int NTH = kSpmvThreads,
          int IT = SpmvTile<T>::kSlots / (kSpmvThreads * (16 / sizeof(T)))>
__device__ __forceinline__ void stream_products_staged(const unsigned short *__restrict__ cidx,
                                                       const unsigned int *__restrict__ pk, int2 rd,
                                                       int nr, const int (&lsl)[SpmvTile<T>::kStageSlots / NTH],
                                                       const T *__restrict__ vals,
                                                       const T *__restrict__ x, int kb, int k1,
                                                       T *__restrict__ lds) {
    constexpr int VW = 16 / sizeof(T);
    constexpr int SMAX = SpmvTile<T>::kStageSlots / NTH;
    typedef typename VecT<T, VW>::V V;
    const int tid = threadIdx.x;
    const int last = (k1 - 1) & ~(VW - 1);
    constexpr int NW = rsp_pack::words_per_thread(IT * VW);
    constexpr int HW = VW / 2;
    static_assert(NW <= IT * HW, "the packed words fit the unpacked ones' registers");
    const bool pkd = PKM == 2 ? pk != nullptr : PKM == 1;
    unsigned int iw[PKM == 1 ? NW : IT * HW];
    V vv[IT];
    if (pkd) {
        const unsigned int *w = pk + tid * NW;
#pragma unroll
        for (int q = 0; q < NW; ++q) iw[q] = ld<NT>(w + q);
    } else {
#pragma unroll
        for (int it = 0; it < IT; ++it) {
            const int e = min(kb + (it * NTH + tid) * VW, last);
            const unsigned int *w = reinterpret_cast<const unsigned int *>(cidx + e);
#pragma unroll
            for (int q = 0; q < HW; ++q) iw[it * HW + q] = ld<NT>(w + q);
        }
    }
#pragma unroll
    for (int it = 0; it < IT; ++it) {
        const int e = min(kb + (it * NTH + tid) * VW, last);
        vv[it] = ld<NT>(reinterpret_cast<const V *>(vals + e));
    }
    __builtin_amdgcn_sched_barrier(0);
    const __amdgpu_buffer_rsrc_t xr =
        __builtin_amdgcn_make_buffer_rsrc((void *)x, (short)0, 0x7ffffffc, 0x00020000);
    auto xload = [&](int col) {
        if constexpr (sizeof(T) == 8)
            return __builtin_bit_cast(T, __builtin_amdgcn_raw_buffer_load_b64(xr, col * 8, 0, 0));
        else
            return __builtin_bit_cast(T, __builtin_amdgcn_raw_buffer_load_b32(xr, col * 4, 0, 0));
    };
    T xs[SMAX];
    int U;
    if (SpmvTile<T>::kStageList && nr == 255) {
        U = rd.y;
#pragma unroll
        for (int k = 0; k < SMAX; ++k)
            if (k * NTH < U) xs[k] = xload(rd.x + lsl[k]);
    } else {
        int2 *tab = reinterpret_cast<int2 *>(lds + SpmvTile<T>::kSlots) - (nr + 1);
        if (tid <= nr) tab[tid] = rd;
        lds_barrier();
        U = tab[nr].y;
        int us[SMAX], lo[SMAX];
#pragma unroll
        for (int k = 0; k < SMAX; ++k) {
            us[k] = min(k * NTH + tid, U - 1);
            lo[k] = 0;
        }
        for (int n = nr; n > 1;) {
            const int h = n >> 1;
#pragma unroll
            for (int k = 0; k < SMAX; ++k)
                if (tab[lo[k] + h].y <= us[k]) lo[k] += h;
            n -= h;
        }
#pragma unroll
        for (int k = 0; k < SMAX; ++k)
            if (k * NTH < U) {
                const int2 r = tab[lo[k]];
                xs[k] = xload(r.x + (us[k] - r.y));
            }
    }
#pragma unroll
    for (int k = 0; k < SMAX; ++k)
        if (k * NTH < U && k * NTH + tid < U) lds[k * NTH + tid] = xs[k];
    lds_barrier();
    T xv[IT][VW];
    if (pkd) {
#pragma unroll
        for (int it = 0; it < IT; ++it)
#pragma unroll
            for (int j = 0; j < VW; ++j) xv[it][j] = lds[min((int)rsp_pack::get_field(iw, it * VW + j), U - 1)];
    } else {
#pragma unroll
        for (int it = 0; it < IT; ++it)
#pragma unroll
            for (int j = 0; j < VW; ++j)
                xv[it][j] = lds[min((int)((iw[(it * VW + j) >> 1] >> (16 * (j & 1))) & 0xffffu), U - 1)];
    }
    lds_barrier();
#pragma unroll
    for (int it = 0; it < IT; ++it) {
        V p;
#pragma unroll
        for (int j = 0; j < VW; ++j) p[j] = vv[it][j] * xv[it][j];
        *reinterpret_cast<V *>(lds + (it * NTH + tid) * VW) = p;
    }
}

template <typename T, int NTH = kSpmvThreads>
__device__ __forceinline__ void stream_products_scalar(const int *__restrict__ colidx,
                                                       const T *__restrict__ vals,
                                                       const T *__restrict__ x, int k0, int kb,
                                                       int k1, T *lds) {
    for (int e = kb + (int)threadIdx.x; e < k1; e += NTH)
        if (e >= k0) lds[e - kb] = vals[e] * x[colidx[e]];
}

template <typename T, int L, int NTH, typename Sink>
__device__ __forceinline__ void reduce_rows(const T *lds, const unsigned short *rp_lds, int nrows, int kb,
                                            int heavy, int *hl, int *hn, Sink sink) {
    constexpr int NA = 8 / L;
    constexpr int NG = NTH / L;
    const int tid = threadIdx.x;
    const int g = tid / L, lane = tid & (L - 1);
    for (int rr = g; rr - g < nrows; rr += NG) {
        bool active = rr < nrows;
        T acc[NA];
#pragma unroll
        for (int t = 0; t < NA; ++t) acc[t] = T(0);
        if (active) {
            const int a0 = rp_lds[rr] - kb, a1 = rp_lds[rr + 1] - kb, last = a1 - 1;
            if (heavy > 0 && a1 - a0 > heavy) {
                active = false;
                if (lane == 0) hl[atomicAdd(hn, 1)] = rr;
            } else {
                for (int base = a0 + lane; base < a1; base += 8) {
                    T v[NA];
#pragma unroll
                    for (int t = 0; t < NA; ++t) v[t] = lds[min(base + t * L, last)];
#pragma unroll
                    for (int t = 0; t < NA; ++t)
                        acc[t] = base + t * L < a1 ? acc[t] + v[t] : acc[t];
                }
            }
        }
#pragma unroll
        for (int h = NA / 2; h >= 1; h >>= 1)
#pragma unroll
            for (int t = 0; t < h; ++t) acc[t] = acc[t] + acc[t + h];
        T s = acc[0];
#pragma unroll
        for (int off = L / 2; off >= 1; off >>= 1) s = s + __shfl_xor(s, off, 64);
        if (active && lane == 0) sink(rr, s);
    }
}

template <typename T, int NTH, typename Sink>
__device__ __forceinline__ void reduce_heavy_rows(const T *lds, const unsigned short *rp_lds, int kb,
                                                  const int *hl, int hn, Sink sink) {
    constexpr int NG = NTH / 8;
    const int tid = threadIdx.x;
    const int g = tid >> 3, lane = tid & 7;
    for (int h = g; h - g < hn; h += NG) {
        const bool active = h < hn;
        T acc = T(0);
        const int rr = active ? hl[h] : 0;
        if (active) {
            const int a1 = rp_lds[rr + 1] - kb, last = a1 - 1;
            for (int base = rp_lds[rr] - kb + lane; base < a1; base += 32) {
                T v[4];
#pragma unroll
                for (int t = 0; t < 4; ++t) v[t] = lds[min(base + 8 * t, last)];
#pragma unroll
                for (int t = 0; t < 4; ++t) acc = base + 8 * t < a1 ? acc + v[t] : acc;
            }
        }
#pragma unroll
        for (int off = 4; off >= 1; off >>= 1) acc = acc + __shfl_xor(acc, off, 64);
        if (active && lane == 0) sink(rr, acc);
    }
}

template <typename T, int NTH = kSpmvThreads, typename Sink>
__device__ __forceinline__ void reduce_tile_rows(const T *lds, const unsigned short *rp_lds, int nrows,
                                                 int nnzt, int kb, int *hl, int *hn, Sink sink) {
    int L = 1;
    while (L < 8 && 2 * L * nrows <= NTH && 8 * L * nrows <= nnzt) L <<= 1;
    switch (L) {
        case 1: reduce_rows<T, 1, NTH>(lds, rp_lds, nrows, kb, 32, hl, hn, sink); break;
        case 2: reduce_rows<T, 2, NTH>(lds, rp_lds, nrows, kb, 64, hl, hn, sink); break;
        case 4: reduce_rows<T, 4, NTH>(lds, rp_lds, nrows, kb, 128, hl, hn, sink); break;
        default: reduce_rows<T, 8, NTH>(lds, rp_lds, nrows, kb, 0, hl, hn, sink); return;
    }
    lds_barrier();
    const int n = *hn;
    if (n > 0) reduce_heavy_rows<T, NTH>(lds, rp_lds, kb, hl, n, sink);
}

template <typename T>
__device__ __forceinline__ T reduce_long(const T *lds, int a, int e, T *wsum) {
    const int tid = threadIdx.x;
    T s = T(0);
    for (int k = a + tid; k < e; k += kSpmvThreads) s += lds[k];
#pragma unroll
    for (int off = 32; off >= 1; off >>= 1) s = s + __shfl_xor(s, off, 64);
    if ((tid & 63) == 0) wsum[tid >> 6] = s;
    lds_barrier();
    return (wsum[0] + wsum[1]) + (wsum[2] + wsum[3]);
}

#ifdef RSP_SPMV_PROBE_LOADS
#include "spmv_probe.h"
#endif

#if defined(__HIP_DEVICE_COMPILE__) && !defined(__gfx950__) && !defined(__gfx942__)
#error "longrow_arrive's relaxed hand-off is only valid on gfx942 / gfx950"
#endif
template <typename T>
__device__ __forceinline__ void longrow_arrive(const SpmvBlock blk, const int *__restrict__ rowptr,
                                               T *partials, T *__restrict__ y, T t, T alpha, T beta,
                                               bool beta_nz) {
    typedef typename std::conditional<sizeof(T) == 8, unsigned long long, unsigned int>::type U;
    constexpr int C = SpmvTile<T>::kChunk;
    const int lane = threadIdx.x & 63;
    const int slot = -(blk.r1 + 1);
    const int rs = rowptr[blk.r0], re = rowptr[blk.r0 + 1];
    const int first = slot - (blk.k0 - rs) / C;
    const int n = (re - rs + C - 1) / C;
    typedef __attribute__((address_space(1))) U GU;
    typedef __attribute__((address_space(1))) unsigned int GI;
    GU *pv = (GU *)reinterpret_cast<U *>(partials);
    GI *ticket = (GI *)reinterpret_cast<unsigned int *>(partials + 2 * first + 1);
    unsigned int arrived = 0;
    if (lane == 0) {
        __hip_atomic_store(pv + 2 * slot, __builtin_bit_cast(U, t), __ATOMIC_RELAXED, __HIP_MEMORY_SCOPE_AGENT);
        asm volatile("s_waitcnt vmcnt(0)" ::: "memory");
        arrived = __hip_atomic_fetch_add(ticket, 1u, __ATOMIC_RELAXED, __HIP_MEMORY_SCOPE_AGENT);
    }
    arrived = (unsigned int)__builtin_amdgcn_readfirstlane((int)arrived);
    if (arrived != (unsigned int)(n - 1)) return;
    T s = T(0);
    for (int c0 = 0; c0 < n; c0 += 64) {
        const T p = c0 + lane < n ? __builtin_bit_cast(T, __hip_atomic_load(pv + 2 * (first + c0 + lane),
                                                                            __ATOMIC_RELAXED, __HIP_MEMORY_SCOPE_AGENT))
                                  : T(0);
        const int cn = min(64, n - c0);
        for (int c = 0; c < cn; ++c) s += __shfl(p, c, 64);
    }
    if (lane == 0) {
        T out = alpha * s;
        if (beta_nz) out += beta * y[blk.r0];
        y[blk.r0] = out;
        __hip_atomic_store(ticket, 0u, __ATOMIC_RELAXED, __HIP_MEMORY_SCOPE_AGENT);
    }
}

template <typename T, bool NT, bool BETA>
__device__ __forceinline__ void spmv_tile(
    const SpmvBlock blk, const int *__restrict__ rowptr, const int *__restrict__ colidx,
    const unsigned short *__restrict__ cidx, const int *__restrict__ runs, int cbase, int poff, int cmax,
    const T *__restrict__ vals, const T *__restrict__ x, T *__restrict__ y,
    T *partials, T alpha, T beta, int beta_nonzero, int nnz, int vector_ok, T *lds,
    T *wsum, unsigned short *rp_lds, int *hl, int fuse) {
    constexpr int VW = 16 / sizeof(T);
    constexpr int RPQ = (SpmvTile<T>::kMaxRows + kSpmvThreads) / kSpmvThreads;
    constexpr int RPW = (SpmvTile<T>::kMaxRows / 2 + kSpmvThreads) / kSpmvThreads;
    static_assert(RPW <= RPQ, "the packed row words fit the row offsets' registers");
    const int tid = threadIdx.x;
    const int k0 = blk.k0, k1 = blk.k1;
    const bool staged = cbase <= -2;
    constexpr int SMAX = SpmvTile<T>::kStageSlots / kSpmvThreads;
    int2 rd = make_int2(0, 0);
    int nr = 0;
    int lsl[SMAX];
    if (staged) {
        const int code = -2 - cbase;
        nr = code & 255;
        if (SpmvTile<T>::kStageList && nr == 255) {
            rd = reinterpret_cast<const int2 *>(runs)[code >> 8];
            const unsigned short *lst = reinterpret_cast<const unsigned short *>(runs + 2 * (code >> 8) + 2);
#pragma unroll
            for (int k = 0; k < SMAX; ++k)
                if (k * kSpmvThreads < rd.y) lsl[k] = lst[min(k * kSpmvThreads + tid, rd.y - 1)];
        } else if (tid <= nr) {
            rd = reinterpret_cast<const int2 *>(runs)[(code >> 8) + tid];
        }
    }
    const int nrows = blk.r1 - blk.r0;
    const int nrows_ld = nrows > 0 ? nrows : 0;
    const bool vec = vector_ok && k1 > k0 && k1 <= (nnz & ~(VW - 1));
    const int kb = vec ? (k0 & ~(VW - 1)) : k0;
    const unsigned int *rec =
        vec && staged && poff >= 0 ? reinterpret_cast<const unsigned int *>(runs) + (poff >> 1) : nullptr;
    const bool prow = rec && (poff & 1);
    const int nrw = (nrows_ld + 2) >> 1;
    const int *rsrc = prow ? reinterpret_cast<const int *>(rec) +
                                 kSpmvThreads * rsp_pack::words_per_thread(SpmvTile<T>::kSlots / kSpmvThreads)
                           : rowptr + blk.r0;
    const int rlim = prow ? nrw - 1 : nrows_ld;
    int rpv[RPQ];
#pragma unroll
    for (int q = 0; q < RPQ; ++q)
        rpv[q] = rsrc[min(tid + q * kSpmvThreads, rlim)];
#ifdef RSP_SPMV_PROBE_LOADS
    if (vec) {
        probe_tile_loads<T, NT>(colidx, vals, y, blk, kb, k1, rpv[0]);
        return;
    }
#endif
    if (vec && cbase >= 0)
        stream_products<T, NT, true>(colidx, cidx, cbase, cmax, vals, x, kb, k1, lds);
    else if (vec && staged && sizeof(T) == 4)
        stream_products_staged<T, NT, 2>(cidx, rec, rd, nr, lsl, vals, x, kb, k1, lds);
    else if (vec && rec)
        stream_products_staged<T, NT, 1>(cidx, rec, rd, nr, lsl, vals, x, kb, k1, lds);
    else if (vec && staged)
        stream_products_staged<T, NT, 0>(cidx, rec, rd, nr, lsl, vals, x, kb, k1, lds);
    else if (vec)
        stream_products<T, NT>(colidx, cidx, 0, 0, vals, x, kb, k1, lds);
    else
        stream_products_scalar<T>(colidx, vals, x, k0, kb, k1, lds);
    if (prow) {
#pragma unroll
        for (int q = 0; q < RPW; ++q) {
            const int i = tid + q * kSpmvThreads;
            if (i < nrw) reinterpret_cast<unsigned int *>(rp_lds)[i] = (unsigned int)rpv[q];
        }
    } else {
#pragma unroll
        for (int q = 0; q < RPQ; ++q) {
            const int i = tid + q * kSpmvThreads;
            if (i <= nrows) rp_lds[i] = (unsigned short)(rpv[q] - kb);
        }
    }
    if (tid == 0) hl[0] = 0;
    lds_barrier();

    if (blk.r1 < 0) {
        const T t = reduce_long(lds, k0 - kb, k1 - kb, wsum);
        if (blk.r1 != rsp::kSpmvWholeRow && fuse) {
            if (tid < 64) longrow_arrive<T>(blk, rowptr, partials, y, t, alpha, beta, BETA);
        } else if (tid == 0) {
            if (blk.r1 == rsp::kSpmvWholeRow) {
                T out = alpha * t;
                if (BETA) out += beta * y[blk.r0];
                y[blk.r0] = out;
            } else {
                partials[2 * -(blk.r1 + 1)] = t;
            }
        }
        return;
    }

    const int r0 = blk.r0;
    reduce_tile_rows<T>(lds, rp_lds, nrows, k1 - k0, 0, hl + 1, hl, [&](int rr, T sum) {
        T out = alpha * sum;
        if (BETA) out += beta * y[r0 + rr];
        constexpr bool kNtY = RSP_NT_Y > 0 || (RSP_NT_Y < 0 && sizeof(T) == 8);
        if constexpr (kNtY)
            __builtin_nontemporal_store(out, y + r0 + rr);
        else
            y[r0 + rr] = out;
    });
}

template <typename T, bool NT, bool BETA>
__global__ __launch_bounds__(kSpmvThreads) void spmv_tiles(
    const int *__restrict__ rowptr, const int *__restrict__ colidx, const T *__restrict__ vals,
    const T *__restrict__ x, T *__restrict__ y, const SpmvBlock *__restrict__ blocks, int nblocks,
    const int *__restrict__ cbases, const int *__restrict__ poffs, const unsigned short *__restrict__ cidx,
    const int *__restrict__ runs, int cmax, T *partials, T alpha, T beta, int beta_nonzero, int nnz,
    int vector_ok, int fuse) {
    __shared__ __attribute__((aligned(16))) T lds[SpmvTile<T>::kSlots];
    __shared__ T wsum[kSpmvThreads / 64];
    __shared__ int hl[1 + kSpmvHeavyMax];
    __shared__ __attribute__((aligned(4))) unsigned short rp_lds[SpmvTile<T>::kMaxRows + 2];
    const int b = xcd_swizzle(blockIdx.x, nblocks);
    spmv_tile<T, NT, BETA>(blocks[b], rowptr, colidx, cidx, runs, cbases[b], poffs[b], cmax, vals, x, y,
                           partials, alpha, beta, beta_nonzero, nnz, vector_ok, lds, wsum, rp_lds, hl,
                           fuse);
}

template <typename T>
__device__ __forceinline__ void fixup_row(const SpmvLongRow r, const T *__restrict__ partials,
                                          T *__restrict__ y, T alpha, T beta, int beta_nonzero) {
    const int lane = threadIdx.x;
    const T yv = (beta_nonzero && lane == 0) ? y[r.row] : T(0);
    T s = T(0);
    for (int c0 = 0; c0 < r.nchunks; c0 += 64) {
        const T p = c0 + lane < r.nchunks ? partials[2 * (r.first + c0 + lane)] : T(0);
        const int cn = min(64, r.nchunks - c0);
        for (int c = 0; c < cn; ++c) s += __shfl(p, c, 64);
    }
    if (lane == 0) {
        T out = alpha * s;
        if (beta_nonzero) out += beta * yv;
        y[r.row] = out;
    }
}

template <typename T>
__global__ __launch_bounds__(64) void spmv_longrow_fixup(const SpmvLongRow *__restrict__ lr,
                                                          int nlong, const T *__restrict__ partials,
                                                          T *__restrict__ y, T alpha, T beta,
                                                          int beta_nonzero) {
    fixup_row<T>(lr[blockIdx.x], partials, y, alpha, beta, beta_nonzero);
}

template <typename T, bool NT, bool BETA, bool SWZ>
__global__ __launch_bounds__(kSpmvThreads) void spmv_tiles_batch(
    const SpmvBatchEntry *__restrict__ entries, const SpmvBlock *__restrict__ tiles,
    const int *__restrict__ cbases, const int *__restrict__ poffs, SpmvBatchTable at, T alpha, T beta,
    int fuse) {
    __shared__ __attribute__((aligned(16))) T lds[SpmvTile<T>::kSlots];
    __shared__ T wsum[kSpmvThreads / 64];
    __shared__ int hl[1 + kSpmvHeavyMax];
    __shared__ __attribute__((aligned(4))) unsigned short rp_lds[SpmvTile<T>::kMaxRows + 2];
    const int b = blockIdx.x;
    int j = 0, lo = 0, hi = at.begin[1];
#pragma unroll
    for (int q = 1; q < kSpmvBatchMax; ++q)
        if (b >= at.begin[q]) {
            j = q;
            lo = at.begin[q];
            hi = at.begin[q + 1];
        }
    const int t = lo + (SWZ ? xcd_swizzle(b - lo, hi - lo) : b - lo);
    const SpmvBatchEntry e = entries[j];
    spmv_tile<T, NT, BETA>(tiles[t], e.rowptr, e.colidx, e.cidx, e.runs, cbases[t], poffs[t], e.cmax,
                           (const T *)e.vals, (const T *)e.x,
                           (T *)e.y, (T *)e.partials, alpha, beta, BETA, e.nnz, e.vector_ok, lds,
                           wsum, rp_lds, hl, fuse);
}

template <typename T>
__global__ __launch_bounds__(64) void spmv_longrow_fixup_batch(
    const SpmvBatchEntry *__restrict__ entries, const SpmvLongRow *__restrict__ lr,
    SpmvBatchTable at, T alpha, T beta, int beta_nonzero) {
    const int i = blockIdx.x;
    int j = 0;
#pragma unroll
    for (int q = 1; q < kSpmvBatchMax; ++q)
        if (i >= at.begin[q]) j = q;
    const SpmvBatchEntry e = entries[j];
    fixup_row<T>(lr[i], (const T *)e.partials, (T *)e.y, alpha, beta, beta_nonzero);
}

template <typename T>
static hipError_t launch_spmv_batch(const SpmvBatchArgs &a, hipStream_t s) {
    const T alpha = (T)a.alpha, beta = (T)a.beta;
    const int bnz = a.beta != 0.0;
    const int ntiles = a.tiles_at.begin[a.count];
    const int fuse = !(a.variant & rsp::kSpmvVariantFixup);
    if (ntiles > 0) {
        const bool nt = !(a.variant & 1), swz = !(a.variant & 8);
        auto kern = bnz ? (nt ? (swz ? spmv_tiles_batch<T, true, true, true>
                                     : spmv_tiles_batch<T, true, true, false>)
                              : (swz ? spmv_tiles_batch<T, false, true, true>
                                     : spmv_tiles_batch<T, false, true, false>))
                        : (nt ? (swz ? spmv_tiles_batch<T, true, false, true>
                                     : spmv_tiles_batch<T, true, false, false>)
                              : (swz ? spmv_tiles_batch<T, false, false, true>
                                     : spmv_tiles_batch<T, false, false, false>));
        hipLaunchKernelGGL(kern, dim3(ntiles), dim3(kSpmvThreads), 0, s, a.entries, a.tiles,
                           a.cbases, a.poffs, a.tiles_at, alpha, beta, fuse);
        const hipError_t e = hipGetLastError();
        if (e != hipSuccess) return e;
    }
    const int nlong = a.longs_at.begin[a.count];
    if (nlong > 0 && !fuse) {
        SpmvBatchTable lt = a.longs_at;
        lt.begin[kSpmvBatchMax] = nlong;
        hipLaunchKernelGGL((spmv_longrow_fixup_batch<T>), dim3(nlong), dim3(64), 0, s,
                           a.entries, a.longrows, lt, alpha, beta, bnz);
        return hipGetLastError();
    }
    return hipSuccess;
}

hipError_t spmv_batch_f32(const SpmvBatchArgs &a, hipStream_t s) {
    return launch_spmv_batch<float>(a, s);
}

template <typename T>
static hipError_t launch_spmv(const SpmvArgs &a, hipStream_t s) {
    if (a.nblocks <= 0) return hipSuccess;
    const T alpha = (T)a.alpha, beta = (T)a.beta;
    const int bnz = a.beta != 0.0;
    const int fuse = !(a.variant & rsp::kSpmvVariantFixup);
    auto kern = (a.variant & 1) ? (bnz ? spmv_tiles<T, false, true> : spmv_tiles<T, false, false>)
                                : (bnz ? spmv_tiles<T, true, true> : spmv_tiles<T, true, false>);
    hipLaunchKernelGGL(kern, dim3(a.nblocks), dim3(kSpmvThreads), 0, s, a.rowptr, a.colidx,
                       (const T *)a.vals, (const T *)a.x, (T *)a.y, a.blocks, a.nblocks, a.cbases,
                       a.poffs, a.cidx, a.runs, a.cmax, (T *)a.partials, alpha, beta, bnz, a.nnz, a.vector_ok, fuse);
    hipError_t e = hipGetLastError();
    if (e != hipSuccess) return e;
    if (a.nlong > 0 && !fuse) {
        hipLaunchKernelGGL((spmv_longrow_fixup<T>), dim3(a.nlong), dim3(64), 0, s,
                           a.longrows, a.nlong, (const T *)a.partials, (T *)a.y, alpha, beta, bnz);
        e = hipGetLastError();
    }
    return e;
}

hipError_t spmv_f32(const SpmvArgs &a, hipStream_t s) { return launch_spmv<float>(a, s); }
void warm_spmv() {
    hipFuncAttributes at;
    (void)hipFuncGetAttributes(&at, reinterpret_cast<const void *>(spmv_tiles<float, true, false>));
    int o = 0;
    (void)hipOccupancyMaxActiveBlocksPerMultiprocessor(&o, spmv_tiles<float, true, false>, kSpmvThreads, 0);
}

#ifndef RSP_FTZ_BUILD
int spmv_tiles_per_cu(int elem_bytes) {
    int o = 0;
    const hipError_t e =
        elem_bytes == 8
            ? hipOccupancyMaxActiveBlocksPerMultiprocessor(&o, spmv_tiles<double, true, false>, kSpmvThreads, 0)
            : hipOccupancyMaxActiveBlocksPerMultiprocessor(&o, spmv_tiles<float, true, false>, kSpmvThreads, 0);
    return (e == hipSuccess && o > 0) ? o : 1;
}

template <typename E>
__global__ __launch_bounds__(256) void gather_kernel(const int64_t *__restrict__ idx,
                                                     const E *__restrict__ src, E *__restrict__ dst,
                                                     int64_t n) {
    const int64_t stride = (int64_t)gridDim.x * 256;
    for (int64_t i = (int64_t)blockIdx.x * 256 + threadIdx.x; i < n; i += stride) dst[i] = src[idx[i]];
}

template <typename E>
__global__ __launch_bounds__(256) void scatter_kernel(const int64_t *__restrict__ idx,
                                                      const E *__restrict__ src, E *__restrict__ dst,
                                                      int64_t n) {
    const int64_t stride = (int64_t)gridDim.x * 256;
    for (int64_t i = (int64_t)blockIdx.x * 256 + threadIdx.x; i < n; i += stride) dst[idx[i]] = src[i];
}

hipError_t scatter(int elem_bytes, int64_t n, const int64_t *idx, const void *src, void *dst,
                   hipStream_t s) {
    if (n <= 0) return hipSuccess;
    const int64_t want = (n + 255) / 256;
    const int grid = (int)(want < 2048 ? want : 2048);
    if (elem_bytes == 8)
        hipLaunchKernelGGL((scatter_kernel<double>), dim3(grid), dim3(256), 0, s, idx,
                           (const double *)src, (double *)dst, n);
    else
        hipLaunchKernelGGL((scatter_kernel<float>), dim3(grid), dim3(256), 0, s, idx,
                           (const float *)src, (float *)dst, n);
    return hipGetLastError();
}

hipError_t gather(int elem_bytes, int64_t n, const int64_t *idx, const void *src, void *dst,
                  hipStream_t s) {
    if (n <= 0) return hipSuccess;
    const int64_t want = (n + 255) / 256;
    const int grid = (int)(want < 2048 ? want : 2048);
    if (elem_bytes == 8)
        hipLaunchKernelGGL((gather_kernel<double>), dim3(grid), dim3(256), 0, s, idx,
                           (const double *)src, (double *)dst, n);
    else
        hipLaunchKernelGGL((gather_kernel<float>), dim3(grid), dim3(256), 0, s, idx,
                           (const float *)src, (float *)dst, n);
    return hipGetLastError();
}

hipError_t spmv_f64(const SpmvArgs &a, hipStream_t s) { return launch_spmv<double>(a, s); }
hipError_t spmv_batch_f64(const SpmvBatchArgs &a, hipStream_t s) {
    return launch_spmv_batch<double>(a, s);
}
#endif

}
```

respasol_amd/csrc/spmv_plan.cpp:

```cpp

#include "spmv_plan.h"
#include "spmv_pack.h"

#include <algorithm>
#include <atomic>
#include <vector>

namespace rsp_plan {

using rsp::SpmvTile;

namespace {

size_t align256(size_t x) { return (x + 255) & ~(size_t)255; }

struct TileGeom {
    int cap, chunk, maxrows;
    int ucap;
    bool list;
    int vw, iw;
    int xelem;
};
template <typename T>
TileGeom geom_of() {
    using S = SpmvTile<T>;
    return {S::kMaxNnz, S::kChunk, S::kMaxRows, S::kStageSlots, S::kStageList, S::kVec,
            rsp_pack::index_words(rsp::kSpmvThreads, rsp::kSpmvIter * S::kVec), (int)sizeof(T)};
}
TileGeom geom(rsp_datatype_t t) { return t == RSP_R_64F ? geom_of<double>() : geom_of<float>(); }

SpmvBounds spmv_bounds(int64_t rows, int64_t nnz, int cap) {
    SpmvBounds b;
    size_t q = (size_t)(nnz / cap) + 1;
    size_t l = (size_t)(nnz / rsp::kSpmvLongRow) + 1;
    b.nlong = q;
    b.nslots = 2 * q + 1;
    b.nblocks = 6 * q + 2 * l + (size_t)(rows / rsp::kSpmvMaxRows) + 8;
    b.nblocks += std::min<size_t>(b.nblocks, 8192);
    return b;
}

}

SpmvLayout spmv_layout(const SpmvBounds &b, size_t elem, int64_t nnz, size_t run_ints) {
    SpmvLayout l;
    l.off_long = align256(b.nblocks * sizeof(SpmvBlock));
    l.off_part = l.off_long + align256(b.nlong * sizeof(SpmvLongRow));
    l.off_cbase = l.off_part + align256(b.nslots * 2 * elem);
    l.off_poff = l.off_cbase + align256(b.nblocks * sizeof(int));
    l.off_cidx = l.off_poff + align256(b.nblocks * sizeof(int));
    l.off_runs = l.off_cidx + align256((size_t)std::max<int64_t>(nnz, 0) * sizeof(uint16_t));
    l.bytes = l.off_runs + align256(run_ints * sizeof(int));
    return l;
}

PlanOptions plan_options(rsp_datatype_t type) {
    using rsp_an::env_int;
    PlanOptions o;
    o.type = type;
    o.stage_list = env_int("RSP_SPMV_STAGE_LIST", 1);
    o.list_cap = env_int("RSP_SPMV_LIST_CAP", o.list_cap);
    o.stage_pct = std::min(std::max(env_int("RSP_SPMV_STAGE_PCT", 80), 0), 100);
    o.pack_mode = std::min(std::max(env_int("RSP_SPMV_PACK", 2), 0), 2);
    return o;
}

RowPlan build_spmv_plan(const int *rp, int m, int cap, int chunk, int maxrows, int row_align) {
    RowPlan out;
    hvec<SpmvBlock> &blocks = out.blocks;
    int slots = 0;
    int r = 0;
    while (r < m) {
        int len = rp[r + 1] - rp[r];
        if (len > rsp::kSpmvLongRow) {
            if (len <= chunk) {
                SpmvBlock b;
                b.r0 = r;
                b.r1 = rsp::kSpmvWholeRow;
                b.k0 = rp[r];
                b.k1 = rp[r + 1];
                blocks.push_back(b);
                r++;
                continue;
            }
            SpmvLongRow lr;
            lr.row = r;
            lr.first = slots;
            lr.nchunks = 0;
            lr.pad = 0;
            for (int k = rp[r]; k < rp[r + 1]; k += chunk) {
                SpmvBlock b;
                b.r0 = r;
                b.r1 = -(slots + 1);
                b.k0 = k;
                b.k1 = std::min(k + chunk, rp[r + 1]);
                blocks.push_back(b);
                slots++;
                lr.nchunks++;
            }
            out.longrows.push_back(lr);
            r++;
            continue;
        }
        int start = r, nnz = 0;
        while (r < m && r - start < maxrows) {
            int l = rp[r + 1] - rp[r];
            if (l > rsp::kSpmvLongRow || (r > start && nnz + l > cap)) break;
            nnz += l;
            r++;
        }
        if (row_align > 1 && r < m && r % row_align != 0) {
            const int ra = r - r % row_align;
            if (ra > start && (int64_t)(rp[ra] - rp[start]) * 4 >= (int64_t)(rp[r] - rp[start]) * 3) r = ra;
        }
        SpmvBlock b;
        b.r0 = start;
        b.r1 = r;
        b.k0 = rp[start];
        b.k1 = rp[r];
        blocks.push_back(b);
    }
    out.nslots = slots;
    return out;
}

namespace {

RowPlan pack_rows(const int *rp, int m, int cap, const TileGeom &g, const PlanOptions &o) {
    return build_spmv_plan(rp, m, cap, g.chunk, g.maxrows, o.row_align);
}

void respread(const int *rp, int m, int64_t nnz_bound, const TileGeom &g, const PlanOptions &o, RowPlan &p) {
    const SpmvBounds bb = spmv_bounds(m, std::max<int64_t>(nnz_bound, 0), g.chunk);
    const int64_t nnz_s = rp[(size_t)m];
    int c = (int)std::max<int64_t>(64, std::min<int64_t>(g.cap, (nnz_s + o.spread - 1) / o.spread));
    for (int tries = 0; tries < 32 && c < g.cap; tries++) {
        RowPlan p2 = pack_rows(rp, m, c, g, o);
        if ((int64_t)p2.blocks.size() <= o.spread && p2.blocks.size() <= bb.nblocks) {
            p = std::move(p2);
            break;
        }
        c += std::max(8, c / 16);
    }
}

int distinct_cols(const int *ci, int k0, int k1, std::vector<int> &cols) {
    cols.assign(ci + k0, ci + k1);
    std::sort(cols.begin(), cols.end());
    cols.erase(std::unique(cols.begin(), cols.end()), cols.end());
    int R = 1;
    for (size_t u = 1; u < cols.size(); u++) R += cols[u] != cols[u - 1] + 1;
    return R;
}

bool list_tiles_ok(const TileGeom &g, const PlanOptions &o) {
    return o.use_stage && o.use_c16 && g.list && o.stage_list != 0;
}

void list_repack(const int *rp, const int *ci, int m, const TileGeom &g, const PlanOptions &o, RowPlan &p) {
    int64_t band = 0, all = 0;
    std::vector<int> cols;
    const size_t step = std::max<size_t>(1, p.blocks.size() / 64);
    for (size_t t = 0; t < p.blocks.size(); t += step) {
        const SpmvBlock &bk = p.blocks[t];
        if (bk.r1 < 0 || bk.k1 <= bk.k0) continue;
        const int R = distinct_cols(ci, bk.k0, bk.k1, cols);
        all += bk.k1 - bk.k0;
        if (cols.back() - cols.front() <= 65535 && R > rsp::kStageRuns && (int)cols.size() > g.ucap)
            band += bk.k1 - bk.k0;
    }
    if (2 * band > all) p = pack_rows(rp, m, std::min(g.cap, std::min(std::max(o.list_cap, 64), g.ucap)), g, o);
}

bool interior_tile(const SpmvBlock &b, const int *ci, int64_t local_cols) {
    if (b.r1 < 0) return false;
    for (int k = b.k0; k < b.k1; k++)
        if (ci[(size_t)k] >= local_cols) return false;
    return true;
}
int partition_interior(const int *ci, int64_t local_cols, hvec<SpmvBlock> &blocks) {
    auto mid = std::stable_partition(blocks.begin(), blocks.end(),
                                     [&](const SpmvBlock &b) { return interior_tile(b, ci, local_cols); });
    return (int)(mid - blocks.begin());
}

enum class TileKind { Int32, Gather16, Runs, List };
TileKind classify_tile(const SpmvBlock &bk, const int *ci, const TileGeom &g, const PlanOptions &o,
                       std::vector<int> &cols, int *lo_out, int *R_out) {
    int lo = ci[(size_t)bk.k0], hi = lo;
    for (int k = bk.k0 + 1; k < bk.k1; k++) {
        lo = std::min(lo, ci[(size_t)k]);
        hi = std::max(hi, ci[(size_t)k]);
    }
    *lo_out = lo;
    if (hi - lo > 65535) return TileKind::Int32;
    const bool x_in_rsrc = ((int64_t)hi + 1) * g.xelem <= (int64_t)0x7ffffffc;
    if (!o.use_stage || bk.r1 < 0 || !x_in_rsrc) return TileKind::Gather16;
    const int len = bk.k1 - bk.k0;
    const int R = *R_out = distinct_cols(ci, bk.k0, bk.k1, cols);
    const int U = (int)cols.size();
    if (U <= g.ucap && R <= rsp::kStageRuns && 100LL * U <= (long long)o.stage_pct * len) return TileKind::Runs;
    if (list_tiles_ok(g, o) && U <= g.ucap && R > rsp::kStageRuns) return TileKind::List;
    return TileKind::Gather16;
}

void encode_columns(const int *ci, int64_t nnz_s, const TileGeom &g, const PlanOptions &o, TilePlan &p) {
    p.c16.assign((size_t)nnz_s, 0);
    const long long nt = (long long)p.blocks.size();
    std::vector<std::vector<int>> truns(o.use_stage ? (size_t)nt : 0);
    std::vector<char> tlist(o.use_stage ? (size_t)nt : 0, 0);
    std::atomic<int64_t> n16{0}, nst{0};
    rsp_an::parallel_for(nt, 64, [&](long long t0, long long t1) {
        std::vector<int> cols;
        int64_t c16n = 0, stn = 0;
        for (long long t = t0; t < t1; t++) {
            const SpmvBlock &bk = p.blocks[(size_t)t];
            if (bk.k1 <= bk.k0) continue;
            int lo = 0, R = 0;
            const TileKind kind = classify_tile(bk, ci, g, o, cols, &lo, &R);
            if (kind == TileKind::Int32) continue;
            const int len = bk.k1 - bk.k0;
            c16n += len;
            if (kind == TileKind::Gather16) {
                p.cbase[(size_t)t] = lo;
                for (int k = bk.k0; k < bk.k1; k++) p.c16[(size_t)k] = (uint16_t)(ci[(size_t)k] - lo);
                continue;
            }
            const int U = (int)cols.size();
            std::vector<int> &r = truns[(size_t)t];
            tlist[(size_t)t] = kind == TileKind::List;
            if (kind == TileKind::Runs) {
                r.reserve(2 * (size_t)(R + 1));
                for (int u = 0; u < U; u++)
                    if (u == 0 || cols[(size_t)u] != cols[(size_t)u - 1] + 1) {
                        r.push_back(cols[(size_t)u]);
                        r.push_back(u);
                    }
                r.push_back(0);
                r.push_back(U);
            } else {
                r.assign(2 + 2 * (size_t)((U + 3) / 4), 0);
                r[0] = cols[0];
                r[1] = U;
                uint16_t *ofs = reinterpret_cast<uint16_t *>(r.data() + 2);
                for (int u = 0; u < U; u++) ofs[u] = (uint16_t)(cols[(size_t)u] - cols[0]);
            }
            for (int k = bk.k0; k < bk.k1; k++)
                p.c16[(size_t)k] =
                    (uint16_t)(std::lower_bound(cols.begin(), cols.end(), ci[(size_t)k]) - cols.begin());
            stn += len;
        }
        n16 += c16n;
        nst += stn;
    });
    p.nnz_c16 = n16;
    p.nnz_staged = nst;
    for (size_t t = 0; t < truns.size(); t++) {
        const std::vector<int> &r = truns[t];
        if (r.empty()) continue;
        const int64_t off = (int64_t)p.runs.size() / 2;
        if (off >= kStageOffLimit) {
            p.nnz_c16 -= p.blocks[t].k1 - p.blocks[t].k0;
            p.nnz_staged -= p.blocks[t].k1 - p.blocks[t].k0;
            continue;
        }
        p.cbase[t] = stage_encode(off, tlist[t] ? kStageListCode : (int)r.size() / 2 - 1);
        p.runs.insert(p.runs.end(), r.begin(), r.end());
    }
}

void pack_staged_tiles(const int *rp, const TileGeom &g, int mode, TilePlan &p) {
    constexpr int IT = rsp::kSpmvIter, NTH = rsp::kSpmvThreads;
    const int VW = g.vw, IW = g.iw;
    if (mode <= 0) return;
    int64_t end = ((int64_t)p.runs.size() + 3) & ~(int64_t)3;
    for (size_t t = 0; t < p.blocks.size(); t++) {
        const SpmvBlock &b = p.blocks[t];
        if (!staged(p.cbase[t]) || b.r1 < 0 || !rsp_pack::eligible(NTH, IT * VW, b.k1 - b.k0)) continue;
        const int64_t words = IW + (mode >= 2 ? rsp_pack::row_words(b.r1 - b.r0) : 0);
        if (end + words >= kPackWordLimit) break;
        p.poff[t] = pack_encode(end, mode >= 2);
        end = (end + words + 3) & ~(int64_t)3;
        p.tiles_packed++;
        p.nnz_packed += b.k1 - b.k0;
    }
    if (p.tiles_packed == 0) return;
    p.runs.resize((size_t)end + 4, 0);
    rsp_an::parallel_for((long long)p.blocks.size(), 64, [&](long long t0, long long t1) {
        for (long long t = t0; t < t1; t++) {
            if (p.poff[(size_t)t] == kNoPack) continue;
            const SpmvBlock &b = p.blocks[(size_t)t];
            const PackCode pc = pack_decode(p.poff[(size_t)t]);
            uint32_t *rec = reinterpret_cast<uint32_t *>(p.runs.data()) + pc.word;
            rsp_pack::pack_slots(p.c16.data(), b.k0, b.k1, VW, IT, NTH, rec);
            if (pc.rows) rsp_pack::pack_rows(rp, b.r0, b.r1 - b.r0, b.k0 & ~(VW - 1), rec + IW);
        }
    });
}

}

void make_tile_plan(const int *rp, const int *ci, int m, int64_t nnz_bound, const PlanOptions &o, TilePlan &p) {
    const TileGeom g = geom(o.type);
    RowPlan &rows = p;
    rows = pack_rows(rp, m, g.cap, g, o);
    const size_t nb = p.blocks.size();
    if (o.spread > 0 && nb > 0 && (int64_t)nb < o.spread) respread(rp, m, nnz_bound, g, o, rows);
    if (list_tiles_ok(g, o) && p.blocks.size() == nb && nb > 0) list_repack(rp, ci, m, g, o, rows);
    p.nint = o.local_cols >= 0 ? partition_interior(ci, o.local_cols, p.blocks) : 0;
    const int64_t nnz_s = m > 0 ? rp[(size_t)m] : 0;
    p.cbase.assign(p.blocks.size(), kCbaseInt32);
    p.c16.clear();
    p.runs.clear();
    p.poff.assign(p.blocks.size(), kNoPack);
    p.tiles_packed = p.nnz_packed = 0;
    p.nnz_c16 = 0;
    p.nnz_staged = 0;
    if (o.use_c16 && nnz_s > 0 && nnz_s <= nnz_bound) {
        encode_columns(ci, nnz_s, g, o, p);
        if (o.use_stage) pack_staged_tiles(rp, g, o.pack_mode, p);
    }
}

void plan_stats(const TilePlan &p, rsp_datatype_t type, int64_t out[8]) {
    const TileGeom g = geom(type);
    int64_t nstaged = 0, idx = 0, desc = 0, rows16 = 0, rowptr = 0;
    for (size_t t = 0; t < p.blocks.size(); t++) {
        const SpmvBlock &b = p.blocks[t];
        const int cb = p.cbase[t], po = p.poff[t];
        const int64_t len = b.k1 - b.k0, nrows = b.r1 > b.r0 ? b.r1 - b.r0 : 0;
        idx += po != kNoPack ? 4LL * g.iw : cb == kCbaseInt32 ? 4 * len : 2 * len;
        if (staged(cb)) {
            const StageCode sc = stage_decode(cb);
            nstaged++;
            desc += sc.list() ? 8 + 2LL * p.runs[2 * (size_t)sc.off + 1] : 8LL * (sc.nr + 1);
        }
        if (po != kNoPack && pack_decode(po).rows)
            rows16 += 4LL * rsp_pack::row_words((int)nrows);
        else
            rowptr += 4 * (nrows + 1);
    }
    out[0] = (int64_t)p.blocks.size();
    out[1] = p.tiles_packed;
    out[2] = p.nnz_packed;
    out[3] = 24 * (int64_t)p.blocks.size() + idx + desc + rows16;
    out[4] = rowptr;
    out[5] = nstaged;
    out[6] = idx;
    out[7] = rows16;
}

namespace {

bool verify_split(const int *ci, const PlanOptions &o, const TilePlan &p) {
    const size_t nt = p.blocks.size(), nint = (size_t)p.nint;
    if (p.nint < 0 || nint > nt || (o.local_cols < 0 && nint != 0)) return false;
    for (size_t t = 0; t < nt; t++) {
        const SpmvBlock &b = p.blocks[t];
        if (o.local_cols >= 0 && t <= nint && interior_tile(b, ci, o.local_cols) != (t < nint)) return false;
        if (t == 0 || t == nint) continue;
        const SpmvBlock &a = p.blocks[t - 1];
        if (a.r0 > b.r0 || (a.r0 == b.r0 && a.k0 >= b.k0)) return false;
    }
    return true;
}

}

bool plan_verify(const int *rp, const int *ci, int m, const PlanOptions &o, const TilePlan &p) {
    const TileGeom g = geom(o.type);
    const int vw = g.vw, iw = g.iw;
    const int nnz_s = m > 0 ? rp[m] : 0;
    if (p.poff.size() != p.blocks.size() || p.cbase.size() != p.blocks.size()) return false;
    if (!p.c16.empty() && p.c16.size() != (size_t)nnz_s) return false;
    int64_t npk = 0, epk = 0;
    for (size_t t = 0; t < p.blocks.size(); t++) {
        const SpmvBlock &b = p.blocks[t];
        const int cb = p.cbase[t], po = p.poff[t];
        if (b.r0 < 0 || b.r0 >= m || (b.r1 >= 0 && (b.r1 < b.r0 || b.r1 > m))) return false;
        if (b.k0 < 0 || b.k1 < b.k0 || b.k1 > nnz_s) return false;
        if (cb != kCbaseInt32 && p.c16.empty() && b.k1 > b.k0) return false;
        if (!o.use_c16 && cb != kCbaseInt32) return false;
        if (!o.use_stage && (staged(cb) || po != kNoPack)) return false;
        const uint32_t *rec = nullptr;
        if (po != kNoPack) {
            const PackCode pc = pack_decode(po);
            const int nrows = b.r1 - b.r0, kb = b.k0 & ~(vw - 1);
            const size_t words = (size_t)iw + (pc.rows ? rsp_pack::row_words(nrows) : 0);
            if (po < 0 || !staged(cb) || b.r1 < 0 || o.pack_mode == 0 || pc.rows != (o.pack_mode >= 2) ||
                !rsp_pack::eligible(rsp::kSpmvThreads, rsp::kSpmvIter * vw, b.k1 - b.k0) || (pc.word & 3) ||
                pc.word + words > p.runs.size())
                return false;
            rec = reinterpret_cast<const uint32_t *>(p.runs.data()) + pc.word;
            const int nwt = iw / rsp::kSpmvThreads;
            for (int tid = 0; tid < rsp::kSpmvThreads; tid++)
                for (int f = 0; f < rsp::kSpmvIter * vw; f++) {
                    const long long e = (long long)kb + (long long)((f / vw) * rsp::kSpmvThreads + tid) * vw + f % vw;
                    if ((e < b.k0 || e >= b.k1) && rsp_pack::get_field(rec + (size_t)tid * nwt, f) != 0) return false;
                }
            if (pc.rows)
                for (int i = 0; i <= nrows; i++)
                    if (rsp_pack::unpack_row(rec + iw, i) + kb != rp[b.r0 + i]) return false;
            npk++;
            epk += b.k1 - b.k0;
        }
        auto slot_of = [&](int k) {
            return rec ? (int)rsp_pack::unpack_slot(rec, b.k0, k, vw, rsp::kSpmvIter, rsp::kSpmvThreads)
                       : (int)p.c16[(size_t)k];
        };
        if (cb == kCbaseInt32 || b.k1 <= b.k0) continue;
        const StageCode sc = staged(cb) ? stage_decode(cb) : StageCode{0, 0};
        const int off = sc.off, nr = sc.nr;
        const int *r = nullptr;
        const uint16_t *ofs = nullptr;
        int U = 0;
        if (staged(cb) && sc.list()) {
            if (o.type != RSP_R_64F) return false;
            if ((size_t)2 * off + 2 > p.runs.size()) return false;
            r = p.runs.data() + 2 * (size_t)off;
            U = r[1];
            if (U < 1 || U > g.ucap || (size_t)2 * off + 2 + 2 * (size_t)((U + 3) / 4) > p.runs.size()) return false;
            ofs = reinterpret_cast<const uint16_t *>(r + 2);
            for (int u = 1; u < U; u++)
                if (ofs[u] <= ofs[u - 1]) return false;
        } else if (staged(cb)) {
            if (nr < 1 || nr > rsp::kStageRuns || (size_t)2 * (off + nr + 1) > p.runs.size()) return false;
            r = p.runs.data() + 2 * (size_t)off;
            U = r[2 * nr + 1];
            if (r[1] != 0 || U > g.ucap) return false;
            for (int j = 1; j <= nr; j++)
                if (r[2 * j + 1] <= r[2 * j - 1] ||
                    (j < nr && r[2 * j] <= r[2 * j - 2] + (r[2 * j + 1] - r[2 * j - 1]) - 1))
                    return false;
        }
        for (int k = b.k0; k < b.k1; k++) {
            int col;
            if (cb >= 0) {
                col = cb + p.c16[(size_t)k];
            } else {
                const int u = slot_of(k);
                if (u >= U) return false;
                int j = 0;
                while (!ofs && j + 1 < nr && r[2 * (j + 1) + 1] <= u) j++;
                col = ofs ? r[0] + ofs[u] : r[2 * j] + (u - r[2 * j + 1]);
            }
            if (col != ci[k]) return false;
        }
    }
    return npk == p.tiles_packed && epk == p.nnz_packed && verify_split(ci, o, p);
}

uint64_t digest(const TilePlan &p) {
    rsp_an::Fnv f;
    f.vec(p.blocks);
    f.vec(p.longrows);
    f.bytes(&p.nslots, sizeof(p.nslots));
    f.bytes(&p.nint, sizeof(p.nint));
    f.vec(p.cbase);
    f.vec(p.c16);
    f.vec(p.runs);
    f.vec(p.poff);
    for (const int64_t c : {p.nnz_c16, p.nnz_staged, p.tiles_packed, p.nnz_packed}) f.bytes(&c, sizeof(c));
    return f.h;
}

}
```

respasol_amd/csrc/spmv_plan.h:

```cpp
#ifndef RSP_SPMV_PLAN_H
#define RSP_SPMV_PLAN_H

#include <stddef.h>
#include <stdint.h>

#include "rsp.h"
#include "host_pool.h"
#include "rsp_kernels.h"

namespace rsp_plan {

using rsp::SpmvBlock;
using rsp::SpmvLongRow;
using rsp_an::hvec;


constexpr int kCbaseInt32 = -1;
constexpr int kStageListCode = 255;
constexpr int64_t kStageOffLimit = 1LL << 22;
struct StageCode {
    int off, nr;
    bool list() const { return nr == kStageListCode; }
};
inline bool staged(int cbase) { return cbase <= -2; }
inline int stage_encode(int64_t off, int nr) { return -2 - (int)((off << 8) | nr); }
inline StageCode stage_decode(int cbase) { return {(-2 - cbase) >> 8, (-2 - cbase) & 255}; }

constexpr int kNoPack = -1;
constexpr int64_t kPackWordLimit = 1LL << 30;
struct PackCode {
    size_t word;
    int rows;
};
inline int pack_encode(int64_t word, int rows) { return (int)(word << 1) | rows; }
inline PackCode pack_decode(int poff) { return {(size_t)(poff >> 1), poff & 1}; }

struct SpmvBounds {
    size_t nblocks, nlong, nslots;
};

struct SpmvLayout {
    size_t off_long, off_part, off_cbase, off_poff, off_cidx, off_runs, bytes;
};
SpmvLayout spmv_layout(const SpmvBounds &b, size_t elem, int64_t nnz, size_t run_ints = 0);

struct PlanOptions {
    rsp_datatype_t type = RSP_R_64F;
    int64_t spread = 0;
    int64_t local_cols = -1;
    int row_align = 1;
    bool use_c16 = true;
    bool use_stage = true;
    int stage_list = 1;
    int list_cap = 1 << 30;
    int stage_pct = 80;
    int pack_mode = 2;
};
PlanOptions plan_options(rsp_datatype_t type);

struct RowPlan {
    hvec<SpmvBlock> blocks;
    hvec<SpmvLongRow> longrows;
    int nslots = 0;
};
RowPlan build_spmv_plan(const int *rp, int m, int cap, int chunk, int maxrows, int row_align);

struct TilePlan : RowPlan {
    int nint = 0;
    hvec<int> cbase;
    hvec<uint16_t> c16;
    hvec<int> runs;
    hvec<int> poff;
    int64_t nnz_c16 = 0;
    int64_t nnz_staged = 0;
    int64_t tiles_packed = 0, nnz_packed = 0;
};

void make_tile_plan(const int *rp, const int *ci, int m, int64_t nnz_bound, const PlanOptions &o, TilePlan &p);

bool plan_verify(const int *rp, const int *ci, int m, const PlanOptions &o, const TilePlan &p);

void plan_stats(const TilePlan &p, rsp_datatype_t type, int64_t out[8]);

uint64_t digest(const TilePlan &p);

}

#endif
```

respasol_amd/sparse.py:

```python
from __future__ import annotations

import ctypes as C

import numpy as np
import torch

from . import _lib
from ._lib import RspError, check, rsp

_DT = {torch.float64: _lib.R_64F, torch.float32: _lib.R_32F}


def _ptr(t: torch.Tensor | None) -> C.c_void_p:
    return C.c_void_p(t.data_ptr() if t is not None and t.numel() > 0 else 0)


def _scalar(value: float, dtype: torch.dtype):
    return C.c_double(value) if dtype == torch.float64 else C.c_float(value)


class Handle:

    def __init__(self, stream: torch.cuda.Stream | None = None, ftz: bool = False):
        if not torch.cuda.is_available():
            raise RuntimeError("respasol_amd.sparse needs a HIP device (MI355X, gfx950)")
        self._h = C.c_void_p()
        check(rsp.rsp_create(C.byref(self._h)), "rsp_create")
        self.set_stream(stream if stream is not None else torch.cuda.current_stream())
        self.set_ftz(ftz)

    @property
    def ptr(self) -> C.c_void_p:
        return self._h

    def set_stream(self, stream: torch.cuda.Stream) -> None:
        self.stream = stream
        check(rsp.rsp_set_stream(self._h, C.c_void_p(stream.cuda_stream)), "rsp_set_stream")

    def set_ftz(self, on: bool) -> None:
        self.ftz = bool(on)
        check(rsp.rsp_set_ftz(self._h, 1 if on else 0), "rsp_set_ftz")

    def close(self) -> None:
        if self._h:
            rsp.rsp_destroy(self._h)
            self._h = C.c_void_p()

    def __del__(self):
        try:
            self.close()
        except Exception:
            pass


def upload_csr(rowptr: np.ndarray, colidx: np.ndarray, values: np.ndarray,
               dtype: torch.dtype = torch.float64, device: str | torch.device = "cuda"):
    np_dt = np.float64 if dtype == torch.float64 else np.float32
    rp = torch.from_numpy(np.ascontiguousarray(rowptr, np.int32)).to(device)
    ci = torch.from_numpy(np.ascontiguousarray(colidx, np.int32)).to(device)
    va = torch.from_numpy(np.ascontiguousarray(values).astype(np_dt)).to(device)
    return rp, ci, va


class SpMat:

    def __init__(self, handle: Handle, rowptr: torch.Tensor, colidx: torch.Tensor,
                 values: torch.Tensor, n_cols: int, nnz: int | None = None):
        if values.dtype not in _DT:
            raise TypeError("values must be float64 or float32")
        if rowptr.dtype != torch.int32 or colidx.dtype != torch.int32:
            raise TypeError("rowptr/colidx must be int32 (CUSPARSE_INDEX_32I)")
        self.handle = handle
        self.rowptr, self.colidx, self.values = rowptr, colidx, values
        self.m = rowptr.numel() - 1
        self.n = int(n_cols)
        self.dtype = values.dtype
        self.nnz = int(nnz if nnz is not None else colidx.numel())
        self._mat = C.c_void_p()
        check(rsp.rsp_create_csr(C.byref(self._mat), self.m, self.n, self.nnz, _ptr(rowptr),
                                 _ptr(colidx), _ptr(values), _DT[self.dtype]), "rsp_create_csr")
        one, zero = _scalar(1.0, self.dtype), _scalar(0.0, self.dtype)
        size = C.c_size_t()
        check(rsp.rsp_spmv_buffer_size(handle.ptr, _lib.OP_N, C.byref(one), self._mat,
                                       C.byref(zero), _DT[self.dtype], C.byref(size)),
              "rsp_spmv_buffer_size")
        self.buffer = torch.empty(max(int(size.value), 1), dtype=torch.uint8, device=values.device)

    @property
    def nnz_stored(self) -> int:
        return int(self.colidx.numel())

    def spmv(self, x: torch.Tensor, y: torch.Tensor | None = None, alpha: float = 1.0,
             beta: float = 0.0, transpose: bool = False) -> torch.Tensor:
        n_in, n_out = (self.m, self.n) if transpose else (self.n, self.m)
        if x.dtype != self.dtype or x.numel() < n_in:
            raise ValueError("x has the wrong dtype or length")
        if y is None:
            y = torch.empty(n_out, dtype=self.dtype, device=x.device)
        elif transpose and (y.dtype != self.dtype or y.numel() < n_out):
            raise ValueError("y has the wrong dtype or length")
        a, b = _scalar(alpha, self.dtype), _scalar(beta, self.dtype)
        check(rsp.rsp_spmv(self.handle.ptr, _lib.OP_T if transpose else _lib.OP_N, C.byref(a), self._mat,
                           _ptr(x), C.byref(b), _ptr(y), _DT[self.dtype], _ptr(self.buffer)), "rsp_spmv")
        return y

    def preprocess_transpose(self) -> None:
        one, zero = _scalar(1.0, self.dtype), _scalar(0.0, self.dtype)
        check(rsp.rsp_spmv_preprocess(self.handle.ptr, _lib.OP_T, C.byref(one), self._mat, None,
                                      C.byref(zero), None, _DT[self.dtype], _ptr(self.buffer)),
              "rsp_spmv_preprocess")

    def bind(self, x: torch.Tensor, y: torch.Tensor, alpha: float = 1.0, beta: float = 0.0):
        if x.dtype != self.dtype or x.numel() < self.n or y.dtype != self.dtype or y.numel() < self.m:
            raise ValueError("x / y have the wrong dtype or length")
        a, b = _scalar(alpha, self.dtype), _scalar(beta, self.dtype)
        args = (self.handle.ptr, _lib.OP_N, C.byref(a), self._mat, _ptr(x), C.byref(b), _ptr(y),
                _DT[self.dtype], _ptr(self.buffer))
        keep = (a, b, x, y)
        fn = rsp.rsp_spmv

        def call():
            st = fn(*args)
            if st:
                check(st, "rsp_spmv")
        call.keep = keep
        return call

    def set_values(self, values: torch.Tensor) -> None:
        if values.dtype not in _DT:
            raise TypeError("values must be float64 or float32")
        if values.numel() < self.nnz_stored:
            raise ValueError("values is shorter than the pattern")
        check(rsp.rsp_csr_set_values(self._mat, _ptr(values), _DT[values.dtype]), "rsp_csr_set_values")
        self.values = values
        self.dtype = values.dtype

    def set_local_cols(self, ncols_local: int) -> None:
        check(rsp.rsp_spmat_set_local_cols(self._mat, int(ncols_local)), "rsp_spmat_set_local_cols")
        one, zero = _scalar(1.0, self.dtype), _scalar(0.0, self.dtype)
        check(rsp.rsp_spmv_preprocess(self.handle.ptr, _lib.OP_N, C.byref(one), self._mat, None,
                                      C.byref(zero), None, _DT[self.dtype], _ptr(self.buffer)),
              "rsp_spmv_preprocess")

    def plan_info(self) -> dict:
        t, e = C.c_int64(), C.c_int64()
        check(rsp.rsp_spmv_plan_info(self._mat, C.byref(t), C.byref(e)), "rsp_spmv_plan_info")
        return {"tiles": t.value, "entries_16bit": e.value}

    def spmv_part(self, x: torch.Tensor, y: torch.Tensor, part: int, alpha: float = 1.0) -> torch.Tensor:
        if x.dtype != self.dtype or x.numel() < self.n:
            raise ValueError("x has the wrong dtype or length")
        a, b = _scalar(alpha, self.dtype), _scalar(0.0, self.dtype)
        check(rsp.rsp_spmv_part(self.handle.ptr, C.byref(a), self._mat, _ptr(x), C.byref(b), _ptr(y),
                                _DT[self.dtype], _ptr(self.buffer), int(part)), "rsp_spmv_part")
        return y

    def close(self) -> None:
        if self._mat:
            rsp.rsp_destroy_spmat(self._mat)
            self._mat = C.c_void_p()

    def __del__(self):
        try:
            self.close()
        except Exception:
            pass


PLAN_STATS = ("tiles", "packed_tiles", "packed_entries", "schedule_bytes", "rowptr_bytes", "staged_tiles",
              "index_bytes", "packed_rowoff_bytes")


def spmv_plan_stats(rowptr, colidx, fp32: bool = False, nnz: int | None = None) -> dict:
    import numpy as np

    rp = np.ascontiguousarray(rowptr, np.int32)
    ci = np.ascontiguousarray(colidx, np.int32)
    out = (C.c_int64 * len(PLAN_STATS))()
    check(rsp.rsp_spmv_plan_stats(len(rp) - 1, rp.ctypes.data, ci.ctypes.data,
                                  int(nnz if nnz is not None else len(ci)), 1 if fp32 else 0, out),
          "rsp_spmv_plan_stats")
    return dict(zip(PLAN_STATS, (int(v) for v in out)))


class SpmvBatch:

    def __init__(self, handle: Handle, mats: list[SpMat], xs: list[torch.Tensor],
                 ys: list[torch.Tensor], part: int = 0):
        if not (len(mats) == len(xs) == len(ys)):
            raise ValueError("mats, xs and ys must have the same length")
        dt = mats[0].dtype if mats else torch.float64
        for A, x, y in zip(mats, xs, ys):
            if A.dtype != dt or x.dtype != dt or y.dtype != dt:
                raise ValueError("one compute type per batch")
            if x.numel() < A.n or y.numel() < A.m:
                raise ValueError("x or y too short")
        self.handle, self.dtype, self.part = handle, dt, int(part)
        self._keep = (list(mats), list(xs), list(ys))
        n = len(mats)
        arr = C.c_void_p * max(n, 1)
        self._b = C.c_void_p()
        check(rsp.rsp_spmv_batch_create(
            handle.ptr, n, arr(*[A._mat.value for A in mats]), arr(*[x.data_ptr() for x in xs]),
            arr(*[y.data_ptr() for y in ys]), arr(*[A.buffer.data_ptr() for A in mats]),
            _DT[dt], self.part, C.byref(self._b)), "rsp_spmv_batch_create")

    def run(self, alpha: float = 1.0, beta: float = 0.0) -> None:
        a, b = _scalar(alpha, self.dtype), _scalar(beta, self.dtype)
        check(rsp.rsp_spmv_batch_run(self.handle.ptr, self._b, C.byref(a), C.byref(b)),
              "rsp_spmv_batch_run")

    def info(self) -> dict:
        t, e = C.c_int64(), C.c_int64()
        check(rsp.rsp_spmv_batch_info(self._b, C.byref(t), C.byref(e)), "rsp_spmv_batch_info")
        return {"tiles": t.value, "entries_16bit": e.value}

    def close(self) -> None:
        if self._b:
            rsp.rsp_spmv_batch_destroy(self._b)
            self._b = C.c_void_p()

    def __del__(self):
        try:
            self.close()
        except Exception:
            pass


class Ilu0:

    def __init__(self, handle: Handle, rowptr: torch.Tensor, colidx: torch.Tensor,
                 nnz: int | None = None):
        self.handle = handle
        self.rowptr, self.colidx = rowptr, colidx
        self.n = rowptr.numel() - 1
        self.nnz = int(nnz if nnz is not None else colidx.numel())
        self._info = C.c_void_p()
        check(rsp.rsp_create_ilu0_info(C.byref(self._info)), "rsp_create_ilu0_info")

    def analysis(self) -> None:
        check(rsp.rsp_ilu0_analysis(self.handle.ptr, self.n, self.nnz, _ptr(self.rowptr),
                                    _ptr(self.colidx), self._info), "rsp_ilu0_analysis")

    def trsv_analysis(self, transpose: bool = False) -> None:
        op = _lib.OP_T if transpose else _lib.OP_N
        check(rsp.rsp_trsv_analysis(self.handle.ptr, op, self._info), "rsp_trsv_analysis")

    def zero_pivot(self) -> int:
        pos = C.c_int(-1)
        st = rsp.rsp_ilu0_zero_pivot(self.handle.ptr, self._info, C.byref(pos))
        if st == _lib.STATUS_ZERO_PIVOT:
            return pos.value
        check(st, "rsp_ilu0_zero_pivot")
        return -1

    TRSV_L, TRSV_LT, TRSV_U = 0, 1, 2

    def solve_zero_pivot(self, which: int) -> int:
        pos = C.c_int(-1)
        st = rsp.rsp_trsv_zero_pivot(self.handle.ptr, self._info, which, C.byref(pos))
        if st == _lib.STATUS_ZERO_PIVOT:
            return pos.value
        check(st, "rsp_trsv_zero_pivot")
        return -1

    def levels(self) -> tuple[int, int]:
        lo, up = C.c_int(), C.c_int()
        check(rsp.rsp_ilu0_levels(self._info, C.byref(lo), C.byref(up)), "rsp_ilu0_levels")
        return lo.value, up.value

    def solve_blocks(self) -> tuple[int, int]:
        lo, up = C.c_int(), C.c_int()
        check(rsp.rsp_ilu0_solve_blocks(self._info, C.byref(lo), C.byref(up)), "rsp_ilu0_solve_blocks")
        return lo.value, up.value

    def factor(self, values: torch.Tensor) -> None:
        check(rsp.rsp_ilu0_factor(self.handle.ptr, self._info, _DT[values.dtype], _ptr(values)),
              "rsp_ilu0_factor")

    def solve_lower(self, values: torch.Tensor, x: torch.Tensor, y: torch.Tensor | None = None,
                    transpose: bool = False, alpha: float = 1.0) -> torch.Tensor:
        if y is None:
            y = torch.empty_like(x)
        a = _scalar(alpha, values.dtype)
        check(rsp.rsp_trsv_lower_unit(self.handle.ptr, _lib.OP_T if transpose else _lib.OP_N,
                                      C.byref(a), self._info, _DT[values.dtype], _ptr(values),
                                      _ptr(x), _ptr(y)), "rsp_trsv_lower_unit")
        return y

    def solve_upper(self, values: torch.Tensor, x: torch.Tensor, y: torch.Tensor | None = None,
                    alpha: float = 1.0) -> torch.Tensor:
        if y is None:
            y = torch.empty_like(x)
        a = _scalar(alpha, values.dtype)
        check(rsp.rsp_trsv_upper(self.handle.ptr, C.byref(a), self._info, _DT[values.dtype],
                                 _ptr(values), _ptr(x), _ptr(y)), "rsp_trsv_upper")
        return y

    def close(self) -> None:
        if self._info:
            rsp.rsp_destroy_ilu0_info(self._info)
            self._info = C.c_void_p()

    def __del__(self):
        try:
            self.close()
        except Exception:
            pass


class SolveResult:

    __slots__ = ("x", "iters", "relres", "reason", "history")

    def __init__(self, x, iters, relres, reason, history):
        self.x, self.iters, self.relres, self.reason, self.history = x, iters, relres, reason, history

    @property
    def converged(self) -> bool:
        return self.reason == _lib.SOLVE_CONVERGED

    def __repr__(self) -> str:
        return (f"SolveResult(iters={self.iters}, relres={self.relres:.3e}, "
                f"reason={self.reason}, n={self.x.numel()})")


class BiCGStab:

    CONVERGED, MAX_ITERS, BREAKDOWN = _lib.SOLVE_CONVERGED, _lib.SOLVE_MAX_ITERS, _lib.SOLVE_BREAKDOWN

    def __init__(self, handle: Handle, A: SpMat, ilu: Ilu0 | None = None,
                 factor: torch.Tensor | None = None):
        if ilu is not None and factor is None:
            raise ValueError("an ILU(0) preconditioner needs its factored values")
        if factor is not None and factor.dtype not in _DT:
            raise TypeError("factor must be float64 or float32")
        self.handle, self.A, self.ilu, self.factor = handle, A, ilu, factor
        self.dtype = A.dtype
        self._s = C.c_void_p()
        check(rsp.rsp_bicgstab_create(handle.ptr, A._mat, ilu._info if ilu is not None else None,
                                      _DT[factor.dtype] if ilu is not None else _DT[A.dtype],
                                      _ptr(factor) if ilu is not None else None, C.byref(self._s)),
              "rsp_bicgstab_create")

    def solve(self, b: torch.Tensor, x0: torch.Tensor | None = None, rtol: float = 1e-10,
              max_iters: int = 1000, check_every: int = 1) -> SolveResult:
        if b.dtype != self.dtype or b.numel() != self.A.m:
            raise ValueError("b has the wrong dtype or length")
        if x0 is not None and (x0.dtype != self.dtype or x0.numel() != self.A.m):
            raise ValueError("x0 has the wrong dtype or length")
        with torch.cuda.stream(self.handle.stream):
            x = torch.zeros_like(b) if x0 is None else x0.clone()
        iters, reason, rel = C.c_int(), C.c_int(), C.c_double()
        check(rsp.rsp_bicgstab_solve(self.handle.ptr, self._s, _ptr(b), _ptr(x), float(rtol),
                                     int(max_iters), int(check_every), C.byref(iters), C.byref(rel),
                                     C.byref(reason)), "rsp_bicgstab_solve")
        count = C.c_int()
        check(rsp.rsp_bicgstab_history(self._s, 0, None, C.byref(count)), "rsp_bicgstab_history")
        hist = (C.c_double * max(count.value, 1))()
        check(rsp.rsp_bicgstab_history(self._s, count.value, hist, C.byref(count)), "rsp_bicgstab_history")
        return SolveResult(x, iters.value, rel.value, reason.value, list(hist[:count.value]))

    def close(self) -> None:
        if self._s:
            rsp.rsp_bicgstab_destroy(self._s)
            self._s = C.c_void_p()

    def __del__(self):
        try:
            self.close()
        except Exception:
            pass


class GMRES:

    CONVERGED, MAX_ITERS, BREAKDOWN = _lib.SOLVE_CONVERGED, _lib.SOLVE_MAX_ITERS, _lib.SOLVE_BREAKDOWN

    def __init__(self, handle: Handle, A: SpMat, ilu: Ilu0 | None = None,
                 factor: torch.Tensor | None = None, restart: int = 30):
        if ilu is not None and factor is None:
            raise ValueError("an ILU(0) preconditioner needs its factored values")
        if factor is not None and factor.dtype not in _DT:
            raise TypeError("factor must be float64 or float32")
        self.handle, self.A, self.ilu, self.factor = handle, A, ilu, factor
        self.dtype = A.dtype
        self.restart = int(restart)
        self._s = C.c_void_p()
        check(rsp.rsp_gmres_create(handle.ptr, A._mat, ilu._info if ilu is not None else None,
                                   _DT[factor.dtype] if ilu is not None else _DT[A.dtype],
                                   _ptr(factor) if ilu is not None else None, self.restart,
                                   C.byref(self._s)), "rsp_gmres_create")

    def solve(self, b: torch.Tensor, x0: torch.Tensor | None = None, rtol: float = 1e-10,
              max_iters: int = 1000, check_every: int = 1) -> SolveResult:
        if b.dtype != self.dtype or b.numel() != self.A.m:
            raise ValueError("b has the wrong dtype or length")
        if x0 is not None and (x0.dtype != self.dtype or x0.numel() != self.A.m):
            raise ValueError("x0 has the wrong dtype or length")
        with torch.cuda.stream(self.handle.stream):
            x = torch.zeros_like(b) if x0 is None else x0.clone()
        iters, reason, rel = C.c_int(), C.c_int(), C.c_double()
        check(rsp.rsp_gmres_solve(self.handle.ptr, self._s, _ptr(b), _ptr(x), float(rtol), int(max_iters),
                                  int(check_every), C.byref(iters), C.byref(rel), C.byref(reason)),
              "rsp_gmres_solve")
        count = C.c_int()
        check(rsp.rsp_gmres_history(self._s, 0, None, C.byref(count)), "rsp_gmres_history")
        hist = (C.c_double * max(count.value, 1))()
        check(rsp.rsp_gmres_history(self._s, count.value, hist, C.byref(count)), "rsp_gmres_history")
        return SolveResult(x, iters.value, rel.value, reason.value, list(hist[:count.value]))

    def close(self) -> None:
        if self._s:
            rsp.rsp_gmres_destroy(self._s)
            self._s = C.c_void_p()

    def __del__(self):
        try:
            self.close()
        except Exception:
            pass


def dot(handle: Handle, x: torch.Tensor, y: torch.Tensor) -> float:
    if x.dtype != y.dtype or x.dtype not in _DT or x.numel() != y.numel():
        raise ValueError("dot: x and y must share dtype (float64 / float32) and length")
    r = C.c_double()
    check(rsp.rsp_dot(handle.ptr, _DT[x.dtype], x.numel(), C.c_void_p(x.data_ptr()),
                      C.c_void_p(y.data_ptr()), C.byref(r)), "rsp_dot")
    return r.value


def orthogonalize(handle: Handle, V: torch.Tensor, w: torch.Tensor) -> np.ndarray:
    if V.dim() != 2 or w.dim() != 1 or V.dtype != w.dtype or V.dtype not in _DT or V.shape[1] != w.numel():
        raise ValueError("orthogonalize: V must be (k, n) and w (n,), one dtype (float64 / float32)")
    if V.shape[1] > 1 and V.stride(1) != 1:
        raise ValueError("orthogonalize: the rows of V must have unit stride")
    k, n = V.shape
    ldv = V.stride(0) if k > 1 else max(n, 1)
    h = np.zeros(k + 1)
    check(rsp.rsp_orthogonalize(handle.ptr, _DT[V.dtype], n, k, C.c_void_p(V.data_ptr()), ldv,
                                C.c_void_p(w.data_ptr()), h.ctypes.data_as(C.POINTER(C.c_double))),
          "rsp_orthogonalize")
    return h


def gather(handle: Handle, idx: torch.Tensor, src: torch.Tensor, dst: torch.Tensor) -> None:
    if idx.dtype != torch.int64 or src.dtype != dst.dtype or dst.numel() < idx.numel():
        raise ValueError("gather: bad arguments")
    check(rsp.rsp_gather(handle.ptr, _DT[src.dtype], idx.numel(), _ptr(idx), _ptr(src), _ptr(dst)),
          "rsp_gather")


def scatter(handle: Handle, idx: torch.Tensor, src: torch.Tensor, dst: torch.Tensor) -> None:
    if idx.dtype != torch.int64 or src.dtype != dst.dtype or src.numel() < idx.numel():
        raise ValueError("scatter: bad arguments")
    check(rsp.rsp_scatter(handle.ptr, _DT[src.dtype], idx.numel(), _ptr(idx), _ptr(src), _ptr(dst)),
          "rsp_scatter")


def csr2csc(handle: Handle, rowptr: torch.Tensor, colidx: torch.Tensor, values: torch.Tensor | None,
            n_cols: int):
    if rowptr.dtype != torch.int32 or colidx.dtype != torch.int32:
        raise TypeError("rowptr/colidx must be int32 (CUSPARSE_INDEX_32I)")
    if values is not None and values.dtype not in _DT:
        raise TypeError("values must be float64 or float32")
    m = rowptr.numel() - 1
    nnz = int(rowptr[-1].item()) if m > 0 else 0
    if nnz > colidx.numel() or (values is not None and nnz > values.numel()):
        raise ValueError("colidx / values are shorter than the pattern")
    t_rp = torch.empty(int(n_cols) + 1, dtype=torch.int32, device=rowptr.device)
    t_ci = torch.empty(nnz, dtype=torch.int32, device=rowptr.device)
    t_va = None if values is None else torch.empty(nnz, dtype=values.dtype, device=rowptr.device)
    check(rsp.rsp_csr2csc(handle.ptr, m, int(n_cols), colidx.numel(), _ptr(rowptr), _ptr(colidx), _ptr(values),
                          _DT[values.dtype] if values is not None else _lib.R_64F, _ptr(t_rp), _ptr(t_ci),
                          _ptr(t_va)), "rsp_csr2csc")
    return t_rp, t_ci, t_va


def csr_transpose_host(rowptr, colidx, n_cols: int):
    rp = np.ascontiguousarray(rowptr, np.int32)
    ci = np.ascontiguousarray(colidx, np.int32)
    m = len(rp) - 1
    nnz = max(int(rp[-1]), 0) if m > 0 else 0
    if nnz > len(ci):
        raise ValueError("colidx is shorter than the pattern")
    t_rp = np.zeros(int(n_cols) + 1, np.int32)
    t_ci, perm = np.zeros(nnz, np.int32), np.zeros(nnz, np.int32)
    check(rsp.rsp_csr_transpose_host(m, int(n_cols), rp.ctypes.data, ci.ctypes.data, t_rp.ctypes.data,
                                     t_ci.ctypes.data, perm.ctypes.data), "rsp_csr_transpose_host")
    return t_rp, t_ci, perm


__all__ = ["Handle", "SpMat", "Ilu0", "BiCGStab", "GMRES", "SolveResult", "dot", "orthogonalize", "upload_csr",
           "gather", "scatter", "csr2csc", "csr_transpose_host", "RspError"]
```

Before: 1033 GFLOP/s.

## Add wide 1024-thread list-staged SpMV tiles for scattered fp64 matrices

Adds a second tile geometry (1024 threads, larger LDS stage and row caps) for fp64 matrices whose tiles are mostly scattered list-staged columns. The planner repacks such matrices into wide tiles, and the batch launcher groups those tiles into separate wide tables so each runs with the larger block. This aims to raise the reuse of staged x columns and cut per-tile overhead for scattered matrices. The cost is higher LDS and register use per block, lower occupancy, and more complex planning and spread decisions in the batch.

```diff
diff --git a/include/rsp.h b/include/rsp.h
--- a/include/rsp.h
+++ b/include/rsp.h
@@ -160,6 +160,11 @@
                                     int *t_row_offsets, int *t_col_ind, int *perm);
 rsp_status_t rsp_spmv_plan_stats(int m, const int *row_offsets, const int *col_ind, int64_t nnz,
                                  rsp_datatype_t compute_type, int64_t stats[8]);
+rsp_status_t rsp_spmv_plan_wide_info(rsp_spmat_t mat, int64_t *wide_tiles, int64_t *wide_entries);
+rsp_status_t rsp_spmv_batch_wide_info(rsp_spmv_batch_t batch, int64_t *wide_tiles, int64_t *wide_entries);
+rsp_status_t rsp_spmv_plan_wide_stats(int m, const int *row_offsets, const int *col_ind, int64_t nnz,
+                                      rsp_datatype_t compute_type, int64_t *wide_tiles, int64_t *wide_entries,
+                                      uint64_t *digest);
 rsp_status_t rsp_ilu0_plan_digest(rsp_ilu0_info_t info, uint64_t *digest);
 
 #ifdef __cplusplus
diff --git a/respasol_amd/_lib.py b/respasol_amd/_lib.py
--- a/respasol_amd/_lib.py
+++ b/respasol_amd/_lib.py
@@ -120,6 +120,9 @@
     "rsp_ilu0_analysis_host": (i32, [i32, vp, vp, vp, vp, vp, vp]),
     "rsp_spmv_plan_host": (i32, [i32, vp, vp, C.c_int64, i32, vp, vp, vp]),
     "rsp_spmv_plan_stats": (i32, [i32, vp, vp, C.c_int64, i32, vp]),
+    "rsp_spmv_plan_wide_info": (i32, [vp, vp, vp]),
+    "rsp_spmv_batch_wide_info": (i32, [vp, vp, vp]),
+    "rsp_spmv_plan_wide_stats": (i32, [i32, vp, vp, C.c_int64, i32, vp, vp, vp]),
     "rsp_ilu0_plan_digest": (i32, [vp, vp]),
     "rsp_csr2csc": (i32, [vp, i64, i64, i64, vp, vp, vp, i32, vp, vp, vp]),
     "rsp_csr_transpose_host": (i32, [i64, i64, vp, vp, vp, vp, vp]),
diff --git a/respasol_amd/csrc/rsp_api.cpp b/respasol_amd/csrc/rsp_api.cpp
--- a/respasol_amd/csrc/rsp_api.cpp
+++ b/respasol_amd/csrc/rsp_api.cpp
@@ -20,9 +20,11 @@
     return (int64_t)rsp_k::spmv_tiles_per_cu((int)elem_size(t)) * h->num_cus;
 }
 
-static PlanOptions handle_plan_options(rsp_handle_t h, rsp_datatype_t t, int64_t local_cols, int64_t spread) {
+static PlanOptions handle_plan_options(rsp_handle_t h, rsp_datatype_t t, int64_t local_cols, int64_t spread,
+                                       bool in_batch = false) {
     const int e = (int)elem_size(t), v = h->spmv_variant;
     PlanOptions o = rsp_plan::plan_options(t);
+    o.wide_min_tiles = in_batch ? 0 : 2 * (int64_t)h->num_cus;
     o.spread = spread;
     o.local_cols = local_cols;
     o.row_align = (v & 64) ? 128 / e : (v & 128) ? 64 / e : 1;
@@ -111,6 +113,7 @@
     mat->lay = lay;
     mat->nnz_c16 = p.nnz_c16;
     mat->nnz_staged = p.nnz_staged;
+    mat->wide = p.wide;
     return RSP_STATUS_SUCCESS;
 }
 
@@ -252,6 +255,7 @@
     a.vector_ok = ((((uintptr_t)mat->colidx) | ((uintptr_t)mat->vals)) & 15) == 0;
     a.nnz = mat->nnz_s;
     a.variant = h->spmv_variant;
+    a.wide = mat->wide;
     hipError_t e;
     if (compute_type == RSP_R_64F)
         e = rsp_k::spmv_f64(a, h->stream);
@@ -269,6 +273,7 @@
     rsp_an::hvec<rsp::SpmvBatchArgs> launches;
     void *d_mem = nullptr;
     int64_t tiles = 0, entries_16bit = 0;
+    int64_t tiles_wide = 0, entries_wide = 0;
     ~rsp_spmv_batch() {
         if (d_mem) (void)hipFree(d_mem);
     }
@@ -317,19 +322,24 @@
     for (int first = 0; first < count; first += rsp::kSpmvBatchMax) {
         Span sp{first, std::min(rsp::kSpmvBatchMax, count - first), 0, 0, {}};
         rsp_an::hvec<rsp_an::hvec<int>> rps((size_t)sp.count), cis((size_t)sp.count);
+        int64_t slots = 0;
         auto plan_members = [&](int64_t spread_all, int64_t nnz_all) {
             sp.nt = 0;
+            slots = 0;
             for (int q = 0; q < sp.count; q++) {
                 rsp_spmat_t A = mats[first + q];
                 const int64_t nnz_q = A->rows > 0 ? rps[q][(size_t)A->rows] : 0;
                 const int64_t share =
                     spread_all > 0 ? std::max<int64_t>(1, spread_all * nnz_q / std::max<int64_t>(1, nnz_all)) : 0;
                 TilePlan &p = plans[first + q];
-                rsp_plan::make_tile_plan(rps[q].data(), cis[q].data(), (int)A->rows, A->nnz,
-                                         handle_plan_options(h, compute_type, A->local_cols, share), p);
+                PlanOptions o = handle_plan_options(h, compute_type, A->local_cols, share, true);
+                if (o.wide < 2) o.wide = 0;
+                if (!(spread_all > 0 && p.wide))
+                    rsp_plan::make_tile_plan(rps[q].data(), cis[q].data(), (int)A->rows, A->nnz, o, p);
                 int t0, t1;
                 tile_range(p, &t0, &t1);
                 sp.nt += t1 - t0;
+                slots += (int64_t)(t1 - t0) * (p.wide ? rsp::kSpmvWideThreads / rsp::kSpmvThreads : 1);
             }
         };
         int64_t nnz_all = 0;
@@ -340,7 +350,7 @@
             nnz_all += A->rows > 0 ? rps[q][(size_t)A->rows] : 0;
         }
         plan_members(0, nnz_all);
-        if (spread_ok && sp.nt < R) plan_members(R, nnz_all);
+        if (spread_ok && slots < R) plan_members(R, nnz_all);
         for (int q = 0; q < sp.count; q++) {
             const TilePlan &p = plans[first + q];
             rsp_spmat_t A = mats[first + q];
@@ -418,17 +428,39 @@
                 if (p.cbase[(size_t)t] != rsp_plan::kCbaseInt32)
                     b->entries_16bit += p.blocks[(size_t)t].k1 - p.blocks[(size_t)t].k0;
             b->tiles += (int64_t)ntq;
+            put(Span::kLongRows, 0, nl * sizeof(SpmvLongRow), p.longrows.data(), nlq * sizeof(SpmvLongRow));
+            put(Span::kC16, q, 0, p.c16.data(), p.c16.size() * sizeof(uint16_t));
+            put(Span::kRuns, q, 0, p.runs.data(), p.runs.size() * sizeof(int));
+            nl += nlq;
+            if (p.wide) continue;
             put(Span::kTiles, 0, nt * sizeof(SpmvBlock), p.blocks.data() + t0, ntq * sizeof(SpmvBlock));
             put(Span::kCbases, 0, nt * sizeof(int), p.cbase.data() + t0, ntq * sizeof(int));
             put(Span::kPoffs, 0, nt * sizeof(int), p.poff.data() + t0, ntq * sizeof(int));
-            put(Span::kLongRows, 0, nl * sizeof(SpmvLongRow), p.longrows.data(), nlq * sizeof(SpmvLongRow));
-            put(Span::kC16, q, 0, p.c16.data(), p.c16.size() * sizeof(uint16_t));
-            put(Span::kRuns, q, 0, p.runs.data(), p.runs.size() * sizeof(int));
             nt += ntq;
-            nl += nlq;
         }
         a.tiles_at.begin[sp.count] = (int)nt;
         a.longs_at.begin[sp.count] = (int)nl;
+        rsp::SpmvWideTable *wt = nullptr;
+        for (int q = 0; q < sp.count; q++) {
+            const TilePlan &p = plans[sp.first + q];
+            int t0, t1;
+            tile_range(p, &t0, &t1);
+            const size_t ntq = (size_t)(t1 - t0);
+            if (!p.wide || ntq == 0) continue;
+            if (!wt || wt->count == rsp::kSpmvWideBatchMax) {
+                wt = &a.wide[a.nwide++];
+                for (int &v : wt->begin) v = INT_MAX;
+            }
+            wt->begin[wt->count] = (int)nt;
+            wt->member[wt->count] = q;
+            put(Span::kTiles, 0, nt * sizeof(SpmvBlock), p.blocks.data() + t0, ntq * sizeof(SpmvBlock));
+            put(Span::kCbases, 0, nt * sizeof(int), p.cbase.data() + t0, ntq * sizeof(int));
+            put(Span::kPoffs, 0, nt * sizeof(int), p.poff.data() + t0, ntq * sizeof(int));
+            nt += ntq;
+            wt->begin[++wt->count] = (int)nt;
+            b->tiles_wide += (int64_t)ntq;
+            for (int t = t0; t < t1; t++) b->entries_wide += p.blocks[(size_t)t].k1 - p.blocks[(size_t)t].k0;
+        }
         b->launches.push_back(a);
     }
     if (!fits) return RSP_STATUS_INTERNAL_ERROR;
@@ -650,6 +682,14 @@
     return RSP_STATUS_SUCCESS;
 }
 
+rsp_status_t rsp_spmv_plan_wide_info(rsp_spmat_t mat, int64_t *wide_tiles, int64_t *wide_entries) {
+    if (!mat || !wide_tiles || !wide_entries) return RSP_STATUS_INVALID_VALUE;
+    if (!mat->planned) return RSP_STATUS_NOT_INITIALIZED;
+    *wide_tiles = mat->wide ? mat->nblocks : 0;
+    *wide_entries = mat->wide ? mat->nnz_s : 0;
+    return RSP_STATUS_SUCCESS;
+}
+
 rsp_status_t rsp_spmv(rsp_handle_t h, rsp_operation_t op, const void *alpha, rsp_spmat_t mat,
                       const void *d_x, const void *beta, void *d_y, rsp_datatype_t compute_type,
                       void *d_buffer) {
@@ -703,6 +743,13 @@
     if (!b || !tiles || !entries_16bit) return RSP_STATUS_INVALID_VALUE;
     *tiles = b->tiles;
     *entries_16bit = b->entries_16bit;
+    return RSP_STATUS_SUCCESS;
+}
+
+rsp_status_t rsp_spmv_batch_wide_info(rsp_spmv_batch_t b, int64_t *wide_tiles, int64_t *wide_entries) {
+    if (!b || !wide_tiles || !wide_entries) return RSP_STATUS_INVALID_VALUE;
+    *wide_tiles = b->tiles_wide;
+    *wide_entries = b->entries_wide;
     return RSP_STATUS_SUCCESS;
 }
 
@@ -807,4 +854,20 @@
     });
 }
 
-}
+rsp_status_t rsp_spmv_plan_wide_stats(int m, const int *row_offsets, const int *col_ind, int64_t nnz,
+                                      rsp_datatype_t compute_type, int64_t *wide_tiles, int64_t *wide_entries,
+                                      uint64_t *digest) {
+    return guarded([&] {
+        if (m < 0 || (m > 0 && (!row_offsets || !col_ind)) || !wide_tiles || !wide_entries)
+            return RSP_STATUS_INVALID_VALUE;
+        if (compute_type != RSP_R_64F && compute_type != RSP_R_32F) return RSP_STATUS_NOT_SUPPORTED;
+        TilePlan p;
+        rsp_plan::make_tile_plan(row_offsets, col_ind, m, nnz, rsp_plan::plan_options(compute_type), p);
+        *wide_tiles = p.tiles_wide;
+        *wide_entries = p.nnz_wide;
+        if (digest) *digest = rsp_plan::digest(p);
+        return RSP_STATUS_SUCCESS;
+    });
+}
+
+}
diff --git a/respasol_amd/csrc/rsp_internal.h b/respasol_amd/csrc/rsp_internal.h
--- a/respasol_amd/csrc/rsp_internal.h
+++ b/respasol_amd/csrc/rsp_internal.h
@@ -51,6 +51,7 @@
     rsp_plan::SpmvLayout lay;
     int64_t nnz_c16;
     int64_t nnz_staged;
+    int wide;
     int64_t local_cols;
     int nint;
     unsigned long long plan_gen;
diff --git a/respasol_amd/csrc/rsp_kernels.h b/respasol_amd/csrc/rsp_kernels.h
--- a/respasol_amd/csrc/rsp_kernels.h
+++ b/respasol_amd/csrc/rsp_kernels.h
@@ -28,19 +28,31 @@
 constexpr int kSpmvLongRow = 256;
 constexpr int kSpmvHeavyMax = 128;
 constexpr int kSpmvWholeRow = -2147483647 - 1;
-template <typename T>
-struct SpmvTile {
+template <typename T, int NTH, int IT, int MAXROWS, int STAGE, int HEAVY, bool WIDE>
+struct SpmvGeom {
+    static constexpr int kThreads = NTH;
+    static constexpr int kIter = IT;
     static constexpr int kVec = 16 / sizeof(T);
-    static constexpr int kSlots = kSpmvThreads * kSpmvIter * kVec;
+    static constexpr int kSlots = NTH * IT * kVec;
     static constexpr int kMaxNnz = kSlots - (kVec - 1);
     static constexpr int kChunk = kSpmvThreads * 4 * kVec - (kVec - 1);
-    static_assert(kChunk <= kMaxNnz, "a chunk must fit one tile");
-    static constexpr int kMaxRows = sizeof(T) == 8 ? kSpmvMaxRows : 2 * kSpmvMaxRows;
-    static constexpr int kStageSlots = sizeof(T) == 8 ? 1536 : 2048;
+    static constexpr int kMaxRows = MAXROWS;
+    static constexpr int kStageSlots = STAGE;
     static constexpr bool kStageList = sizeof(T) == 8;
-};
-static_assert(SpmvTile<float>::kMaxNnz / 33 < kSpmvHeavyMax && SpmvTile<double>::kMaxNnz / 33 < kSpmvHeavyMax,
-              "every > 32-entry row of a tile fits the heavy-row list");
+    static constexpr int kHeavyMax = HEAVY;
+    static constexpr bool kWide = WIDE;
+    static_assert(kStageSlots <= kSlots, "the staged columns fit the LDS image");
+    static_assert(kMaxNnz / 33 < kHeavyMax, "every > 32-entry row of a tile fits the heavy-row list");
+    static_assert(kSlots + kVec <= 65536, "16-bit row offsets");
+};
+template <typename T>
+struct SpmvTile : SpmvGeom<T, kSpmvThreads, kSpmvIter, sizeof(T) == 8 ? kSpmvMaxRows : 2 * kSpmvMaxRows,
+                           sizeof(T) == 8 ? 1536 : 2048, kSpmvHeavyMax, false> {
+    static_assert(SpmvTile::kChunk <= SpmvTile::kMaxNnz, "a chunk must fit one tile");
+};
+constexpr int kSpmvWideThreads = 1024;
+constexpr int kSpmvWideMinTiles = 512;
+struct SpmvWideTile : SpmvGeom<double, kSpmvWideThreads, 3, 2048, 6144, 192, true> {};
 constexpr int kStageRuns = 254;
 
 struct SpmvArgs {
@@ -64,6 +76,7 @@
     int nnz;
     int vector_ok;
     int variant;
+    int wide;
 };
 
 constexpr int kSpmvBatchMax = 32;
@@ -83,6 +96,12 @@
 struct SpmvBatchTable {
     int begin[kSpmvBatchMax + 1];
 };
+constexpr int kSpmvWideBatchMax = 8;
+struct SpmvWideTable {
+    int begin[kSpmvWideBatchMax + 1];
+    int member[kSpmvWideBatchMax];
+    int count;
+};
 struct SpmvBatchArgs {
     const SpmvBatchEntry *entries;
     const SpmvBlock *tiles;
@@ -91,6 +110,8 @@
     const SpmvLongRow *longrows;
     int count;
     SpmvBatchTable tiles_at, longs_at;
+    int nwide;
+    SpmvWideTable wide[kSpmvBatchMax / kSpmvWideBatchMax];
     double alpha, beta;
     int variant;
 };
diff --git a/respasol_amd/csrc/spmv.hip b/respasol_amd/csrc/spmv.hip
--- a/respasol_amd/csrc/spmv.hip
+++ b/respasol_amd/csrc/spmv.hip
@@ -22,6 +22,10 @@
 using rsp::SpmvBlock;
 using rsp::SpmvLongRow;
 using rsp::SpmvTile;
+using rsp::SpmvWideTile;
+using rsp::kSpmvWideThreads;
+using rsp::kSpmvWideBatchMax;
+using rsp::SpmvWideTable;
 using rsp::kSpmvBatchMax;
 using rsp::SpmvBatchArgs;
 using rsp::SpmvBatchEntry;
@@ -115,16 +119,16 @@
     __builtin_amdgcn_fence(__ATOMIC_ACQUIRE, "workgroup", "local");
 }
 
-template <typename T, bool NT, int PKM, int NTH = kSpmvThreads,
-          int IT = SpmvTile<T>::kSlots / (kSpmvThreads * (16 / sizeof(T)))>
+template <typename T, bool NT, int PKM, typename G = SpmvTile<T>>
 __device__ __forceinline__ void stream_products_staged(const unsigned short *__restrict__ cidx,
                                                        const unsigned int *__restrict__ pk, int2 rd,
-                                                       int nr, const int (&lsl)[SpmvTile<T>::kStageSlots / NTH],
+                                                       int nr, const int (&lsl)[G::kStageSlots / G::kThreads],
                                                        const T *__restrict__ vals,
                                                        const T *__restrict__ x, int kb, int k1,
                                                        T *__restrict__ lds) {
     constexpr int VW = 16 / sizeof(T);
-    constexpr int SMAX = SpmvTile<T>::kStageSlots / NTH;
+    constexpr int NTH = G::kThreads, IT = G::kIter;
+    constexpr int SMAX = G::kStageSlots / NTH;
     typedef typename VecT<T, VW>::V V;
     const int tid = threadIdx.x;
     const int last = (k1 - 1) & ~(VW - 1);
@@ -163,13 +167,13 @@
     };
     T xs[SMAX];
     int U;
-    if (SpmvTile<T>::kStageList && nr == 255) {
+    if (G::kStageList && (G::kWide || nr == 255)) {
         U = rd.y;
 #pragma unroll
         for (int k = 0; k < SMAX; ++k)
             if (k * NTH < U) xs[k] = xload(rd.x + lsl[k]);
     } else {
-        int2 *tab = reinterpret_cast<int2 *>(lds + SpmvTile<T>::kSlots) - (nr + 1);
+        int2 *tab = reinterpret_cast<int2 *>(lds + G::kSlots) - (nr + 1);
         if (tid <= nr) tab[tid] = rd;
         lds_barrier();
         U = tab[nr].y;
@@ -368,7 +372,7 @@
     }
 }
 
-template <typename T, bool NT, bool BETA>
+template <typename T, bool NT, bool BETA, typename G = SpmvTile<T>>
 __device__ __forceinline__ void spmv_tile(
     const SpmvBlock blk, const int *__restrict__ rowptr, const int *__restrict__ colidx,
     const unsigned short *__restrict__ cidx, const int *__restrict__ runs, int cbase, int poff, int cmax,
@@ -376,25 +380,26 @@
     T *partials, T alpha, T beta, int beta_nonzero, int nnz, int vector_ok, T *lds,
     T *wsum, unsigned short *rp_lds, int *hl, int fuse) {
     constexpr int VW = 16 / sizeof(T);
-    constexpr int RPQ = (SpmvTile<T>::kMaxRows + kSpmvThreads) / kSpmvThreads;
-    constexpr int RPW = (SpmvTile<T>::kMaxRows / 2 + kSpmvThreads) / kSpmvThreads;
+    constexpr int NTH = G::kThreads;
+    constexpr int RPQ = (G::kMaxRows + NTH) / NTH;
+    constexpr int RPW = (G::kMaxRows / 2 + NTH) / NTH;
     static_assert(RPW <= RPQ, "the packed row words fit the row offsets' registers");
     const int tid = threadIdx.x;
     const int k0 = blk.k0, k1 = blk.k1;
     const bool staged = cbase <= -2;
-    constexpr int SMAX = SpmvTile<T>::kStageSlots / kSpmvThreads;
+    constexpr int SMAX = G::kStageSlots / NTH;
     int2 rd = make_int2(0, 0);
     int nr = 0;
     int lsl[SMAX];
     if (staged) {
         const int code = -2 - cbase;
         nr = code & 255;
-        if (SpmvTile<T>::kStageList && nr == 255) {
+        if (G::kStageList && (G::kWide || nr == 255)) {
             rd = reinterpret_cast<const int2 *>(runs)[code >> 8];
             const unsigned short *lst = reinterpret_cast<const unsigned short *>(runs + 2 * (code >> 8) + 2);
 #pragma unroll
             for (int k = 0; k < SMAX; ++k)
-                if (k * kSpmvThreads < rd.y) lsl[k] = lst[min(k * kSpmvThreads + tid, rd.y - 1)];
+                if (k * NTH < rd.y) lsl[k] = lst[min(k * NTH + tid, rd.y - 1)];
         } else if (tid <= nr) {
             rd = reinterpret_cast<const int2 *>(runs)[(code >> 8) + tid];
         }
@@ -403,18 +408,18 @@
     const int nrows_ld = nrows > 0 ? nrows : 0;
     const bool vec = vector_ok && k1 > k0 && k1 <= (nnz & ~(VW - 1));
     const int kb = vec ? (k0 & ~(VW - 1)) : k0;
-    const unsigned int *rec =
-        vec && staged && poff >= 0 ? reinterpret_cast<const unsigned int *>(runs) + (poff >> 1) : nullptr;
+    const unsigned int *rec = !G::kWide && vec && staged && poff >= 0
+                                  ? reinterpret_cast<const unsigned int *>(runs) + (poff >> 1)
+                                  : nullptr;
     const bool prow = rec && (poff & 1);
     const int nrw = (nrows_ld + 2) >> 1;
-    const int *rsrc = prow ? reinterpret_cast<const int *>(rec) +
-                                 kSpmvThreads * rsp_pack::words_per_thread(SpmvTile<T>::kSlots / kSpmvThreads)
+    const int *rsrc = prow ? reinterpret_cast<const int *>(rec) + NTH * rsp_pack::words_per_thread(G::kSlots / NTH)
                            : rowptr + blk.r0;
     const int rlim = prow ? nrw - 1 : nrows_ld;
     int rpv[RPQ];
 #pragma unroll
     for (int q = 0; q < RPQ; ++q)
-        rpv[q] = rsrc[min(tid + q * kSpmvThreads, rlim)];
+        rpv[q] = rsrc[min(tid + q * NTH, rlim)];
 #ifdef RSP_SPMV_PROBE_LOADS
     if (vec) {
         probe_tile_loads<T, NT>(colidx, vals, y, blk, kb, k1, rpv[0]);
@@ -422,34 +427,36 @@
     }
 #endif
     if (vec && cbase >= 0)
-        stream_products<T, NT, true>(colidx, cidx, cbase, cmax, vals, x, kb, k1, lds);
+        stream_products<T, NT, true, NTH, G::kIter>(colidx, cidx, cbase, cmax, vals, x, kb, k1, lds);
+    else if (vec && staged && G::kWide)
+        stream_products_staged<T, NT, 0, G>(cidx, nullptr, rd, nr, lsl, vals, x, kb, k1, lds);
     else if (vec && staged && sizeof(T) == 4)
-        stream_products_staged<T, NT, 2>(cidx, rec, rd, nr, lsl, vals, x, kb, k1, lds);
+        stream_products_staged<T, NT, 2, G>(cidx, rec, rd, nr, lsl, vals, x, kb, k1, lds);
     else if (vec && rec)
-        stream_products_staged<T, NT, 1>(cidx, rec, rd, nr, lsl, vals, x, kb, k1, lds);
+        stream_products_staged<T, NT, 1, G>(cidx, rec, rd, nr, lsl, vals, x, kb, k1, lds);
     else if (vec && staged)
-        stream_products_staged<T, NT, 0>(cidx, rec, rd, nr, lsl, vals, x, kb, k1, lds);
+        stream_products_staged<T, NT, 0, G>(cidx, rec, rd, nr, lsl, vals, x, kb, k1, lds);
     else if (vec)
-        stream_products<T, NT>(colidx, cidx, 0, 0, vals, x, kb, k1, lds);
+        stream_products<T, NT, false, NTH, G::kIter>(colidx, cidx, 0, 0, vals, x, kb, k1, lds);
     else
-        stream_products_scalar<T>(colidx, vals, x, k0, kb, k1, lds);
+        stream_products_scalar<T, NTH>(colidx, vals, x, k0, kb, k1, lds);
     if (prow) {
 #pragma unroll
         for (int q = 0; q < RPW; ++q) {
-            const int i = tid + q * kSpmvThreads;
+            const int i = tid + q * NTH;
             if (i < nrw) reinterpret_cast<unsigned int *>(rp_lds)[i] = (unsigned int)rpv[q];
         }
     } else {
 #pragma unroll
         for (int q = 0; q < RPQ; ++q) {
-            const int i = tid + q * kSpmvThreads;
+            const int i = tid + q * NTH;
             if (i <= nrows) rp_lds[i] = (unsigned short)(rpv[q] - kb);
         }
     }
     if (tid == 0) hl[0] = 0;
     lds_barrier();
 
-    if (blk.r1 < 0) {
+    if (!G::kWide && blk.r1 < 0) {
         const T t = reduce_long(lds, k0 - kb, k1 - kb, wsum);
         if (blk.r1 != rsp::kSpmvWholeRow && fuse) {
             if (tid < 64) longrow_arrive<T>(blk, rowptr, partials, y, t, alpha, beta, BETA);
@@ -466,7 +473,7 @@
     }
 
     const int r0 = blk.r0;
-    reduce_tile_rows<T>(lds, rp_lds, nrows, k1 - k0, 0, hl + 1, hl, [&](int rr, T sum) {
+    reduce_tile_rows<T, NTH>(lds, rp_lds, nrows, k1 - k0, 0, hl + 1, hl, [&](int rr, T sum) {
         T out = alpha * sum;
         if (BETA) out += beta * y[r0 + rr];
         constexpr bool kNtY = RSP_NT_Y > 0 || (RSP_NT_Y < 0 && sizeof(T) == 8);
@@ -494,6 +501,21 @@
                            fuse);
 }
 
+template <typename T, bool NT, bool BETA>
+__global__ __launch_bounds__(kSpmvWideThreads, 8) void spmv_tiles_wide(
+    const int *__restrict__ rowptr, const int *__restrict__ colidx, const T *__restrict__ vals,
+    const T *__restrict__ x, T *__restrict__ y, const SpmvBlock *__restrict__ blocks, int nblocks,
+    const int *__restrict__ cbases, const unsigned short *__restrict__ cidx, const int *__restrict__ runs,
+    int cmax, T alpha, T beta, int nnz, int vector_ok) {
+    typedef SpmvWideTile G;
+    __shared__ __attribute__((aligned(16))) T lds[G::kSlots];
+    __shared__ int hl[1 + G::kHeavyMax];
+    __shared__ __attribute__((aligned(4))) unsigned short rp_lds[G::kMaxRows + 2];
+    const int b = xcd_swizzle(blockIdx.x, nblocks);
+    spmv_tile<T, NT, BETA, G>(blocks[b], rowptr, colidx, cidx, runs, cbases[b], -1, cmax, vals, x, y, nullptr,
+                              alpha, beta, BETA, nnz, vector_ok, lds, nullptr, rp_lds, hl, 0);
+}
+
 template <typename T>
 __device__ __forceinline__ void fixup_row(const SpmvLongRow r, const T *__restrict__ partials,
                                           T *__restrict__ y, T alpha, T beta, int beta_nonzero) {
@@ -546,6 +568,45 @@
                            wsum, rp_lds, hl, fuse);
 }
 
+template <typename T, bool NT, bool BETA, bool SWZ>
+__global__ __launch_bounds__(kSpmvWideThreads, 8) void spmv_tiles_batch_wide(
+    const SpmvBatchEntry *__restrict__ entries, const SpmvBlock *__restrict__ tiles,
+    const int *__restrict__ cbases, SpmvWideTable at, T alpha, T beta) {
+    typedef SpmvWideTile G;
+    __shared__ __attribute__((aligned(16))) T lds[G::kSlots];
+    __shared__ int hl[1 + G::kHeavyMax];
+    __shared__ __attribute__((aligned(4))) unsigned short rp_lds[G::kMaxRows + 2];
+    const int b = at.begin[0] + (int)blockIdx.x;
+    int j = at.member[0], lo = at.begin[0], hi = at.begin[1];
+#pragma unroll
+    for (int q = 1; q < kSpmvWideBatchMax; ++q)
+        if (b >= at.begin[q]) {
+            j = at.member[q];
+            lo = at.begin[q];
+            hi = at.begin[q + 1];
+        }
+    const int t = lo + (SWZ ? xcd_swizzle(b - lo, hi - lo) : b - lo);
+    const SpmvBatchEntry e = entries[j];
+    spmv_tile<T, NT, BETA, G>(tiles[t], e.rowptr, e.colidx, e.cidx, e.runs, cbases[t], -1, e.cmax,
+                              (const T *)e.vals, (const T *)e.x, (T *)e.y, nullptr, alpha, beta, BETA, e.nnz,
+                              e.vector_ok, lds, nullptr, rp_lds, hl, 0);
+}
+
+template <typename T, bool NT, bool BETA>
+static hipError_t launch_spmv_batch_wide(const SpmvBatchArgs &a, T alpha, T beta, bool swz, hipStream_t s) {
+    for (int w = 0; w < a.nwide; w++) {
+        const SpmvWideTable &wt = a.wide[w];
+        const int n = wt.begin[wt.count] - wt.begin[0];
+        if (n <= 0) continue;
+        auto kern = swz ? spmv_tiles_batch_wide<T, NT, BETA, true> : spmv_tiles_batch_wide<T, NT, BETA, false>;
+        hipLaunchKernelGGL(kern, dim3(n), dim3(kSpmvWideThreads), 0, s, a.entries, a.tiles, a.cbases, wt, alpha,
+                           beta);
+        const hipError_t e = hipGetLastError();
+        if (e != hipSuccess) return e;
+    }
+    return hipSuccess;
+}
+
 template <typename T>
 __global__ __launch_bounds__(64) void spmv_longrow_fixup_batch(
     const SpmvBatchEntry *__restrict__ entries, const SpmvLongRow *__restrict__ lr,
@@ -565,6 +626,17 @@
     const int bnz = a.beta != 0.0;
     const int ntiles = a.tiles_at.begin[a.count];
     const int fuse = !(a.variant & rsp::kSpmvVariantFixup);
+    auto wide = [&]() -> hipError_t {
+        if constexpr (sizeof(T) == 8) {
+            const bool nt = !(a.variant & 1), swz = !(a.variant & 8);
+            return bnz ? (nt ? launch_spmv_batch_wide<T, true, true>(a, alpha, beta, swz, s)
+                             : launch_spmv_batch_wide<T, false, true>(a, alpha, beta, swz, s))
+                       : (nt ? launch_spmv_batch_wide<T, true, false>(a, alpha, beta, swz, s)
+                             : launch_spmv_batch_wide<T, false, false>(a, alpha, beta, swz, s));
+        } else {
+            return a.nwide > 0 ? hipErrorInvalidValue : hipSuccess;
+        }
+    };
     if (ntiles > 0) {
         const bool nt = !(a.variant & 1), swz = !(a.variant & 8);
         auto kern = bnz ? (nt ? (swz ? spmv_tiles_batch<T, true, true, true>
@@ -580,6 +652,7 @@
         const hipError_t e = hipGetLastError();
         if (e != hipSuccess) return e;
     }
+    if (const hipError_t e = wide(); e != hipSuccess) return e;
     const int nlong = a.longs_at.begin[a.count];
     if (nlong > 0 && !fuse) {
         SpmvBatchTable lt = a.longs_at;
@@ -601,6 +674,18 @@
     const T alpha = (T)a.alpha, beta = (T)a.beta;
     const int bnz = a.beta != 0.0;
     const int fuse = !(a.variant & rsp::kSpmvVariantFixup);
+    if (a.wide) {
+        if constexpr (sizeof(T) == 8) {
+            auto kern = (a.variant & 1) ? (bnz ? spmv_tiles_wide<T, false, true> : spmv_tiles_wide<T, false, false>)
+                                        : (bnz ? spmv_tiles_wide<T, true, true> : spmv_tiles_wide<T, true, false>);
+            hipLaunchKernelGGL(kern, dim3(a.nblocks), dim3(kSpmvWideThreads), 0, s, a.rowptr, a.colidx,
+                               (const T *)a.vals, (const T *)a.x, (T *)a.y, a.blocks, a.nblocks, a.cbases, a.cidx,
+                               a.runs, a.cmax, alpha, beta, a.nnz, a.vector_ok);
+            return hipGetLastError();
+        } else {
+            return hipErrorInvalidValue;
+        }
+    }
     auto kern = (a.variant & 1) ? (bnz ? spmv_tiles<T, false, true> : spmv_tiles<T, false, false>)
                                 : (bnz ? spmv_tiles<T, true, true> : spmv_tiles<T, true, false>);
     hipLaunchKernelGGL(kern, dim3(a.nblocks), dim3(kSpmvThreads), 0, s, a.rowptr, a.colidx,
diff --git a/respasol_amd/csrc/spmv_plan.cpp b/respasol_amd/csrc/spmv_plan.cpp
--- a/respasol_amd/csrc/spmv_plan.cpp
+++ b/respasol_amd/csrc/spmv_plan.cpp
@@ -20,14 +20,17 @@
     bool list;
     int vw, iw;
     int xelem;
+    bool wide;
 };
-template <typename T>
+template <typename S, typename T>
 TileGeom geom_of() {
-    using S = SpmvTile<T>;
     return {S::kMaxNnz, S::kChunk, S::kMaxRows, S::kStageSlots, S::kStageList, S::kVec,
-            rsp_pack::index_words(rsp::kSpmvThreads, rsp::kSpmvIter * S::kVec), (int)sizeof(T)};
-}
-TileGeom geom(rsp_datatype_t t) { return t == RSP_R_64F ? geom_of<double>() : geom_of<float>(); }
+            rsp_pack::index_words(S::kThreads, S::kIter * S::kVec), (int)sizeof(T), S::kWide};
+}
+TileGeom geom(rsp_datatype_t t, bool wide = false) {
+    return wide ? geom_of<rsp::SpmvWideTile, double>()
+                : t == RSP_R_64F ? geom_of<SpmvTile<double>, double>() : geom_of<SpmvTile<float>, float>();
+}
 
 SpmvBounds spmv_bounds(int64_t rows, int64_t nnz, int cap) {
     SpmvBounds b;
@@ -62,6 +65,7 @@
     o.list_cap = env_int("RSP_SPMV_LIST_CAP", o.list_cap);
     o.stage_pct = std::min(std::max(env_int("RSP_SPMV_STAGE_PCT", 80), 0), 100);
     o.pack_mode = std::min(std::max(env_int("RSP_SPMV_PACK", 2), 0), 2);
+    o.wide = std::min(std::max(env_int("RSP_SPMV_WIDE", 1), 0), 2);
     return o;
 }
 
@@ -157,8 +161,8 @@
     return o.use_stage && o.use_c16 && g.list && o.stage_list != 0;
 }
 
-void list_repack(const int *rp, const int *ci, int m, const TileGeom &g, const PlanOptions &o, RowPlan &p) {
-    int64_t band = 0, all = 0;
+bool list_repack(const int *rp, const int *ci, int m, const TileGeom &g, const PlanOptions &o, RowPlan &p) {
+    int64_t band = 0, scattered = 0, all = 0;
     std::vector<int> cols;
     const size_t step = std::max<size_t>(1, p.blocks.size() / 64);
     for (size_t t = 0; t < p.blocks.size(); t += step) {
@@ -166,10 +170,23 @@
         if (bk.r1 < 0 || bk.k1 <= bk.k0) continue;
         const int R = distinct_cols(ci, bk.k0, bk.k1, cols);
         all += bk.k1 - bk.k0;
-        if (cols.back() - cols.front() <= 65535 && R > rsp::kStageRuns && (int)cols.size() > g.ucap)
-            band += bk.k1 - bk.k0;
+        if (cols.back() - cols.front() > 65535 || R <= rsp::kStageRuns) continue;
+        scattered += bk.k1 - bk.k0;
+        if ((int)cols.size() > g.ucap) band += bk.k1 - bk.k0;
+    }
+    if (2 * scattered <= all) return false;
+    const bool short_rows =
+        std::none_of(p.blocks.begin(), p.blocks.end(), [](const SpmvBlock &b) { return b.r1 < 0; });
+    if (o.wide > 0 && o.type == RSP_R_64F && short_rows) {
+        const TileGeom w = geom(o.type, true);
+        RowPlan pw = pack_rows(rp, m, std::min(w.cap, std::min(std::max(o.list_cap, 64), w.ucap)), w, o);
+        if (o.wide >= 2 || (int64_t)pw.blocks.size() >= o.wide_min_tiles) {
+            p = std::move(pw);
+            return true;
+        }
     }
     if (2 * band > all) p = pack_rows(rp, m, std::min(g.cap, std::min(std::max(o.list_cap, 64), g.ucap)), g, o);
+    return false;
 }
 
 bool interior_tile(const SpmvBlock &b, const int *ci, int64_t local_cols) {
@@ -199,6 +216,7 @@
     const int len = bk.k1 - bk.k0;
     const int R = *R_out = distinct_cols(ci, bk.k0, bk.k1, cols);
     const int U = (int)cols.size();
+    if (g.wide) return list_tiles_ok(g, o) && U <= g.ucap ? TileKind::List : TileKind::Gather16;
     if (U <= g.ucap && R <= rsp::kStageRuns && 100LL * U <= (long long)o.stage_pct * len) return TileKind::Runs;
     if (list_tiles_ok(g, o) && U <= g.ucap && R > rsp::kStageRuns) return TileKind::List;
     return TileKind::Gather16;
@@ -301,14 +319,17 @@
 }
 
 void make_tile_plan(const int *rp, const int *ci, int m, int64_t nnz_bound, const PlanOptions &o, TilePlan &p) {
-    const TileGeom g = geom(o.type);
+    TileGeom g = geom(o.type);
     RowPlan &rows = p;
     rows = pack_rows(rp, m, g.cap, g, o);
     const size_t nb = p.blocks.size();
     if (o.spread > 0 && nb > 0 && (int64_t)nb < o.spread) respread(rp, m, nnz_bound, g, o, rows);
-    if (list_tiles_ok(g, o) && p.blocks.size() == nb && nb > 0) list_repack(rp, ci, m, g, o, rows);
+    p.wide = list_tiles_ok(g, o) && p.blocks.size() == nb && nb > 0 && list_repack(rp, ci, m, g, o, rows);
+    if (p.wide) g = geom(o.type, true);
     p.nint = o.local_cols >= 0 ? partition_interior(ci, o.local_cols, p.blocks) : 0;
     const int64_t nnz_s = m > 0 ? rp[(size_t)m] : 0;
+    p.tiles_wide = p.wide ? (int64_t)p.blocks.size() : 0;
+    p.nnz_wide = p.wide ? nnz_s : 0;
     p.cbase.assign(p.blocks.size(), kCbaseInt32);
     p.c16.clear();
     p.runs.clear();
@@ -318,7 +339,7 @@
     p.nnz_staged = 0;
     if (o.use_c16 && nnz_s > 0 && nnz_s <= nnz_bound) {
         encode_columns(ci, nnz_s, g, o, p);
-        if (o.use_stage) pack_staged_tiles(rp, g, o.pack_mode, p);
+        if (o.use_stage && !p.wide) pack_staged_tiles(rp, g, o.pack_mode, p);
     }
 }
 
@@ -368,15 +389,20 @@
 }
 
 bool plan_verify(const int *rp, const int *ci, int m, const PlanOptions &o, const TilePlan &p) {
-    const TileGeom g = geom(o.type);
+    const TileGeom g = geom(o.type, p.wide);
     const int vw = g.vw, iw = g.iw;
     const int nnz_s = m > 0 ? rp[m] : 0;
     if (p.poff.size() != p.blocks.size() || p.cbase.size() != p.blocks.size()) return false;
     if (!p.c16.empty() && p.c16.size() != (size_t)nnz_s) return false;
+    if (p.wide && (o.type != RSP_R_64F || o.wide == 0 || !list_tiles_ok(g, o) || p.blocks.empty())) return false;
+    if (p.tiles_wide != (p.wide ? (int64_t)p.blocks.size() : 0) || p.nnz_wide != (p.wide ? nnz_s : 0)) return false;
     int64_t npk = 0, epk = 0;
     for (size_t t = 0; t < p.blocks.size(); t++) {
         const SpmvBlock &b = p.blocks[t];
         const int cb = p.cbase[t], po = p.poff[t];
+        if (p.wide && (b.r1 < 0 || b.r1 - b.r0 > g.maxrows || b.k1 - b.k0 > g.cap || po != kNoPack ||
+                       (staged(cb) && !stage_decode(cb).list())))
+            return false;
         if (b.r0 < 0 || b.r0 >= m || (b.r1 >= 0 && (b.r1 < b.r0 || b.r1 > m))) return false;
         if (b.k0 < 0 || b.k1 < b.k0 || b.k1 > nnz_s) return false;
         if (cb != kCbaseInt32 && p.c16.empty() && b.k1 > b.k0) return false;
@@ -461,6 +487,8 @@
     f.vec(p.runs);
     f.vec(p.poff);
     for (const int64_t c : {p.nnz_c16, p.nnz_staged, p.tiles_packed, p.nnz_packed}) f.bytes(&c, sizeof(c));
+    if (p.wide)
+        for (const int64_t c : {p.tiles_wide, p.nnz_wide}) f.bytes(&c, sizeof(c));
     return f.h;
 }
 
diff --git a/respasol_amd/csrc/spmv_plan.h b/respasol_amd/csrc/spmv_plan.h
--- a/respasol_amd/csrc/spmv_plan.h
+++ b/respasol_amd/csrc/spmv_plan.h
@@ -55,6 +55,8 @@
     int list_cap = 1 << 30;
     int stage_pct = 80;
     int pack_mode = 2;
+    int wide = 1;
+    int64_t wide_min_tiles = rsp::kSpmvWideMinTiles;
 };
 PlanOptions plan_options(rsp_datatype_t type);
 
@@ -74,6 +76,8 @@
     int64_t nnz_c16 = 0;
     int64_t nnz_staged = 0;
     int64_t tiles_packed = 0, nnz_packed = 0;
+    bool wide = false;
+    int64_t tiles_wide = 0, nnz_wide = 0;
 };
 
 void make_tile_plan(const int *rp, const int *ci, int m, int64_t nnz_bound, const PlanOptions &o, TilePlan &p);
diff --git a/respasol_amd/sparse.py b/respasol_amd/sparse.py
--- a/respasol_amd/sparse.py
+++ b/respasol_amd/sparse.py
@@ -143,9 +143,11 @@
               "rsp_spmv_preprocess")
 
     def plan_info(self) -> dict:
-        t, e = C.c_int64(), C.c_int64()
+        t, e, wt, we = C.c_int64(), C.c_int64(), C.c_int64(), C.c_int64()
         check(rsp.rsp_spmv_plan_info(self._mat, C.byref(t), C.byref(e)), "rsp_spmv_plan_info")
-        return {"tiles": t.value, "entries_16bit": e.value}
+        if hasattr(rsp, "rsp_spmv_plan_wide_info"):
+            check(rsp.rsp_spmv_plan_wide_info(self._mat, C.byref(wt), C.byref(we)), "rsp_spmv_plan_wide_info")
+        return {"tiles": t.value, "entries_16bit": e.value, "wide_tiles": wt.value, "wide_entries": we.value}
 
     def spmv_part(self, x: torch.Tensor, y: torch.Tensor, part: int, alpha: float = 1.0) -> torch.Tensor:
         if x.dtype != self.dtype or x.numel() < self.n:
@@ -181,6 +183,18 @@
                                   int(nnz if nnz is not None else len(ci)), 1 if fp32 else 0, out),
           "rsp_spmv_plan_stats")
     return dict(zip(PLAN_STATS, (int(v) for v in out)))
+
+
+def spmv_plan_wide_stats(rowptr, colidx, fp32: bool = False, nnz: int | None = None) -> dict:
+    import numpy as np
+
+    rp = np.ascontiguousarray(rowptr, np.int32)
+    ci = np.ascontiguousarray(colidx, np.int32)
+    t, e, d = C.c_int64(), C.c_int64(), C.c_uint64()
+    check(rsp.rsp_spmv_plan_wide_stats(len(rp) - 1, rp.ctypes.data, ci.ctypes.data,
+                                       int(nnz if nnz is not None else len(ci)), 1 if fp32 else 0,
+                                       C.byref(t), C.byref(e), C.byref(d)), "rsp_spmv_plan_wide_stats")
+    return {"wide_tiles": t.value, "wide_entries": e.value, "digest": d.value}
 
 
 class SpmvBatch:
@@ -211,9 +225,11 @@
               "rsp_spmv_batch_run")
 
     def info(self) -> dict:
-        t, e = C.c_int64(), C.c_int64()
+        t, e, wt, we = C.c_int64(), C.c_int64(), C.c_int64(), C.c_int64()
         check(rsp.rsp_spmv_batch_info(self._b, C.byref(t), C.byref(e)), "rsp_spmv_batch_info")
-        return {"tiles": t.value, "entries_16bit": e.value}
+        if hasattr(rsp, "rsp_spmv_batch_wide_info"):
+            check(rsp.rsp_spmv_batch_wide_info(self._b, C.byref(wt), C.byref(we)), "rsp_spmv_batch_wide_info")
+        return {"tiles": t.value, "entries_16bit": e.value, "wide_tiles": wt.value, "wide_entries": we.value}
 
     def close(self) -> None:
         if self._b:
```

Result: no change. 1032 GFLOP/s (-0.1%).
